# qq456cvb/VoteNet

Hardware: AMD Instinct MI355X
Metric: SUN RGB-D 20k-pt scenes/sec (fwd+bwd) (higher is better)
Workload: dtype f32

## Files before the change

votenet_amd/_lib.py:

```python
import ctypes
import os
import re
import subprocess

import torch

_HERE = os.path.dirname(os.path.abspath(__file__))
_LIB_PATH = os.path.join(_HERE, "lib", "libvotenet_hip.so")
_lib = None
SIDE_LIBS = {
    "monitors": "votenet_monitors.h",
    "guard": "votenet_step_guard.h",
    "features": "votenet_point_features.h",
    "detect": "votenet_detections.h",
    "boxpts": "votenet_box_points.h",
    "aabb": "votenet_aabb_nms.h",
    "depth": "votenet_depth_scan.h",
    "votesup": "votenet_vote_supervision.h",
    "propsup": "votenet_proposal_supervision.h",
    "votesamp": "votenet_vote_sampling.h",
    "instbox": "votenet_instance_boxes.h",
}
_side = {}


class VotenetError(RuntimeError):
    """A HIP runtime / launch / workspace error reported by libvotenet_hip.so."""


class InvalidArgumentError(ValueError):
    """Mirror of tf.errors.InvalidArgumentError raised by the reference's OP_REQUIRES checks."""


def lib_path():
    return _LIB_PATH


def build(force=False):
    if force:
        import glob
        objs = [o for d in ["obj"] + [os.path.join(name, "obj") for name in SIDE_LIBS] for o in glob.glob(os.path.join(_HERE, "csrc", d, "*.o"))]
        for f in [_LIB_PATH] + [side_path(name) for name in SIDE_LIBS] + objs:
            if os.path.exists(f):
                os.remove(f)
    out = subprocess.run(["bash", os.path.join(_HERE, "csrc", "build.sh")], capture_output=True, text=True)
    if out.returncode != 0:
        raise VotenetError("libvotenet_hip.so build failed:\n" + out.stdout + out.stderr)
    return _LIB_PATH


_SCALARS = {"int": ctypes.c_int, "long": ctypes.c_long, "float": ctypes.c_float, "double": ctypes.c_double, "unsigned": ctypes.c_uint,
            "unsigned long long": ctypes.c_ulonglong, "size_t": ctypes.c_size_t}
_POINTEES = set(_SCALARS) | {"void", "char", "unsigned char", "unsigned short", "long long"}


def _declarator(text, where):
    words = text.replace("*", " * ").split()
    if not words or not words[-1].isidentifier():
        raise ValueError("%s: cannot read the declaration '%s'" % (where, " ".join(text.split())))
    return " ".join(w for w in words[:-1] if w != "const" and w != "*"), words.count("*"), words[-1]


def _ctype(base, stars, structs, where, ret=False):
    if stars == 0 and base in _SCALARS:
        return _SCALARS[base]
    if stars == 0 and ret and base == "void":
        return None
    if stars == 1 and base in structs:
        return ctypes.POINTER(structs[base])
    if stars == 1 and ret and base == "char":
        return ctypes.c_char_p
    if stars == 1 and base in _POINTEES:
        return ctypes.c_void_p
    raise ValueError("%s: no ctypes type for the C type '%s'" % (where, base + " *" * stars))


def parse_header(text, structs):
    text = re.sub(r"/\*.*?\*/|//[^\n]*", " ", text, flags=re.S)
    text = re.sub(r"#ifdef __cplusplus.*?#endif", "", text, flags=re.S)
    text = re.sub(r"^[ \t]*#.*$", "", text, flags=re.M)

    def struct(m):
        name, fields = m.group(2), []
        for line in filter(str.strip, m.group(1).split(";")):
            decls = [_declarator(d, name) for d in line.split(",")]
            fields += [(n, _ctype(decls[0][0], stars, structs, name + "." + n)) for _, stars, n in decls]
        structs[name] = type("".join(w.capitalize() for w in name.split("_")[1:]), (ctypes.Structure,),
                             {"_fields_": fields, "__doc__": "struct %s of the C ABI." % name})
        return ""
    text = re.sub(r"typedef\s+struct\s+\w+\s*\{(.*?)\}\s*(\w+)\s*;", struct, text, flags=re.S)
    funcs = {}
    for stmt in text.split(";"):
        if not stmt.strip():
            continue
        m = re.fullmatch(r"(.*?)\((.*)\)\s*", stmt, flags=re.S)
        if not m:
            raise ValueError("not a function declaration: '%s'" % " ".join(stmt.split()))
        base, stars, name = _declarator(m.group(1), "function")
        params = [] if m.group(2).strip() == "void" else m.group(2).split(",")
        funcs[name] = (_ctype(base, stars, structs, name, ret=True),
                       [_ctype(*_declarator(p, name)[:2], structs, name) for p in params])
    return funcs


_STRUCTS = ("BnRaw", "CoefTail", "MlpInput", "RowSegment", "CopySegment")
_abi_read = None


def _abi():
    global _abi_read
    if _abi_read is None:
        structs, protos = {}, []
        for h in ("votenet_hip.h", "votenet_hip_debug.h"):
            with open(os.path.join(_HERE, os.pardir, "include", h)) as f:
                protos.append(parse_header(f.read(), structs))
        globals().update({cls.__name__: cls for cls in structs.values()})
        _abi_read = tuple(protos)
    return _abi_read


def __getattr__(name):
    if name in _STRUCTS:
        _abi()
        return globals()[name]
    raise AttributeError("module %r has no attribute %r" % (__name__, name))


class _Library(ctypes.CDLL):

    def __getattr__(self, name):
        fn = super().__getattr__(name)
        for protos in _abi():
            if name in protos:
                fn.restype, fn.argtypes = protos[name]
        if "debug" in name and name not in ("votenet_debug_enable", "votenet_debug_enabled", "votenet_debug_fps_split_timeouts"):
            self.votenet_debug_enable(1)
        return fn


def lib():
    global _lib
    if _lib is None:
        if not os.path.exists(_LIB_PATH):
            raise VotenetError(
                "libvotenet_hip.so not found at %s -- run `python -c 'import __graft_entry__ as g; g.build()'` "
                "(there is no CPU fallback)" % _LIB_PATH)
        L = _Library(_LIB_PATH)
        for name in _abi()[0]:
            getattr(L, name)
        _lib = L
    return _lib


def side_path(name):
    return os.path.join(os.path.dirname(_LIB_PATH), "libvotenet_%s.so" % name)


def side_loaded(name):
    return name in _side


def side_lib(name):
    if name not in _side:
        path = side_path(name)
        if not os.path.exists(path):
            raise VotenetError("libvotenet_%s.so not found at %s -- run `python -c 'import __graft_entry__ as g; g.build()'` "
                               "(there is no CPU fallback)" % (name, path))
        with open(os.path.join(_HERE, os.pardir, "include", SIDE_LIBS[name])) as f:
            protos = parse_header(f.read(), {})
        S = ctypes.CDLL(path)
        for fname, (restype, argtypes) in protos.items():
            fn = getattr(S, fname)
            fn.restype, fn.argtypes = restype, argtypes
        last_error, = [getattr(S, fname) for fname in protos if fname.endswith("_last_error")]
        _side[name] = (S, last_error)
    return _side[name][0]


def check(rc, side=None):
    if rc == 0:
        return
    if side is None:
        msg, who = lib().votenet_last_error().decode(), "hip"
    else:
        side_lib(side)
        msg, who = _side[side][1]().decode(), side
    if rc == 1:
        raise InvalidArgumentError(msg)
    raise VotenetError("libvotenet_%s error %d: %s" % (who, rc, msg))


_raw_stream = getattr(torch._C, "_cuda_getCurrentRawStream", None)
_cur_device = getattr(torch._C, "_cuda_getDevice", None)


def stream_ptr():
    if _raw_stream is not None and _cur_device is not None:
        return _raw_stream(_cur_device())
    return torch.cuda.current_stream().cuda_stream


class _NoGuard:
    def __enter__(self):
        return None

    def __exit__(self, *a):
        return False


_NOGUARD = _NoGuard()


def device_guard(device):
    idx = device.index
    if _cur_device is not None and (idx is None or idx == _cur_device()):
        return _NOGUARD
    return torch.cuda.device(device)


def ptr(t):
    return t.data_ptr() if t is not None else None


def dev_f32(t, name, rank=None, last=None):
    if not isinstance(t, torch.Tensor):
        raise InvalidArgumentError("%s must be a torch.Tensor" % name)
    if not t.is_cuda:
        raise VotenetError("%s must live on the GPU (no CPU fallback in votenet_amd)" % name)
    if t.dtype != torch.float32:
        raise InvalidArgumentError("%s must be float32" % name)
    if rank is not None and t.dim() != rank:
        raise InvalidArgumentError("%s expects rank %d, got shape %s" % (name, rank, tuple(t.shape)))
    if last is not None and t.shape[-1] != last:
        raise InvalidArgumentError("%s expects last dimension %d, got shape %s" % (name, last, tuple(t.shape)))
    return t.contiguous()


def pitched_rows(t):
    return t.dim() == 3 and t.stride(2) == 1 and t.stride(1) >= t.shape[2] and t.stride(0) == t.shape[1] * t.stride(1)


def dev_f32_rows(t, name):
    if isinstance(t, torch.Tensor) and t.is_cuda and t.dtype == torch.float32 and pitched_rows(t):
        return t
    return dev_f32(t, name, 3)


def dev_i32(t, name, rank=None):
    if not isinstance(t, torch.Tensor):
        raise InvalidArgumentError("%s must be a torch.Tensor" % name)
    if not t.is_cuda:
        raise VotenetError("%s must live on the GPU (no CPU fallback in votenet_amd)" % name)
    if t.dtype != torch.int32:
        raise InvalidArgumentError("%s must be int32" % name)
    if rank is not None and t.dim() != rank:
        raise InvalidArgumentError("%s expects rank %d, got shape %s" % (name, rank, tuple(t.shape)))
    return t.contiguous()
```

votenet_amd/csrc/pool_bwd.hip:

```cpp
#include "mlp_types.h"
#include <mutex>
#include <set>

namespace votenet {

bool wgrad_fast_launch(int mode, const MlpIn &d, long rows, int cin, int cout, const float *dz, const BnSrc &bs, int bsrc, float *dw,
                       hipStream_t st, float *scratch);
void wgrad_reduce(int nslice, long pstride, long e0, long e1, const float *part, float *dw, hipStream_t st);

static inline int pb_grid(long total, int block, int cap)
{
    long g = (total + block - 1) / block;
    if (g > cap) g = cap;
    return (int)(g < 1 ? 1 : g);
}

__global__ __launch_bounds__(256) void bn_bwd_reduce_zsel_kernel(long groups, int c, const float *__restrict__ gout,
                                                                 const float *__restrict__ zsel, const float *__restrict__ scale,
                                                                 const float *__restrict__ shift, const float *__restrict__ mean,
                                                                 const float *__restrict__ var, float eps, int relu,
                                                                 double *__restrict__ sums, CoefTail tail)
{
    __shared__ float sh1[4][64], sh2[4][64];
    const int cx = threadIdx.x & 63, ry = threadIdx.x >> 6;
    const int col = blockIdx.y * 64 + cx;
    float s1 = 0, s2 = 0;
    if (col < c) {
        const float sc = scale[col], sf = shift[col], mu = mean[col], inv = 1.0f / sqrtf(var[col] + eps);
        const long stride = (long)gridDim.x * 4;
        long g = (long)blockIdx.x * 4 + ry;
        for (; g + 7 * stride < groups; g += 8 * stride) {
            float zz[8], gg[8];
#pragma unroll
            for (int u = 0; u < 8; u++) {
                zz[u] = zsel[(size_t)(g + u * stride) * c + col];
                gg[u] = gout[(size_t)(g + u * stride) * c + col];
            }
#pragma unroll
            for (int u = 0; u < 8; u++) {
                if (relu && !(zz[u] * sc + sf > 0.0f)) gg[u] = 0.0f;
                s1 += gg[u];
                s2 += gg[u] * ((zz[u] - mu) * inv);
            }
        }
        for (; g < groups; g += stride) {
            const float zz = zsel[(size_t)g * c + col];
            float gg = gout[(size_t)g * c + col];
            if (relu && !(zz * sc + sf > 0.0f)) gg = 0.0f;
            s1 += gg;
            s2 += gg * ((zz - mu) * inv);
        }
    }
    sh1[ry][cx] = s1;
    sh2[ry][cx] = s2;
    __syncthreads();
    if (ry == 0 && col < c) {
        const float t1 = (sh1[0][cx] + sh1[1][cx]) + (sh1[2][cx] + sh1[3][cx]);
        const float t2 = (sh2[0][cx] + sh2[1][cx]) + (sh2[2][cx] + sh2[3][cx]);
        unsafeAtomicAdd(&sums[col], (double)t1);
        unsafeAtomicAdd(&sums[c + col], (double)t2);
    }
    coef_tail(tail, gridDim.x * gridDim.y, c, sums, scale, shift, mean, var, eps);
}

template <int COUT>
__global__ __launch_bounds__(256) void pool_dgrad_prepare_kernel(int cin, const float *__restrict__ w, const float *__restrict__ bias,
                                                                 const float *__restrict__ coef, float *__restrict__ mmat,
                                                                 float *__restrict__ cvec, unsigned *__restrict__ image,
                                                                 float *__restrict__ h2_ascale = nullptr, float *__restrict__ h2_unscale = nullptr)
{
    constexpr int LD = COUT + 4;
    __shared__ __attribute__((aligned(16))) float Wj[16][LD], Wk[16][LD];
    __shared__ float Cs[COUT], Ds[COUT];
    const int tid = threadIdx.x, tx = tid & 15, ty = tid >> 4;
    const int j0 = blockIdx.y * 16, k0 = blockIdx.x * 16;
    constexpr int Q = COUT / 4;
    for (int e = tid; e < 16 * Q; e += 256) {
        const int r = e / Q, q = e % Q;
        const float4 z4 = make_float4(0.f, 0.f, 0.f, 0.f);
        *reinterpret_cast<float4 *>(&Wj[r][q * 4]) = j0 + r < cin ? *reinterpret_cast<const float4 *>(w + (size_t)(j0 + r) * COUT + q * 4) : z4;
        *reinterpret_cast<float4 *>(&Wk[r][q * 4]) = k0 + r < cin ? *reinterpret_cast<const float4 *>(w + (size_t)(k0 + r) * COUT + q * 4) : z4;
    }
    for (int c = tid; c < COUT; c += 256) {
        const float Cc = coef[2 * COUT + c];
        Cs[c] = Cc;
        Ds[c] = coef[COUT + c] + Cc * (bias ? bias[c] : 0.0f);
    }
    __syncthreads();
    float acc = 0.0f, accv = 0.0f;
#pragma unroll 8
    for (int c = 0; c < COUT; c++) {
        const float wk = Wk[tx][c];
        acc += Wj[ty][c] * Cs[c] * wk;
        accv += Ds[c] * wk;
    }
    if (j0 + ty < cin && k0 + tx < cin) mmat[(size_t)(j0 + ty) * cin + k0 + tx] = acc;
    if (blockIdx.y == 0 && ty == 0 && k0 + tx < cin) cvec[k0 + tx] = accv;
    if (image != nullptr && h2_ascale != nullptr) {
        __shared__ float nj[16], nk[16], cmax[4];
        __syncthreads();
        {
            float pj = 0.0f, pk = 0.0f;
            for (int c = tx; c < COUT; c += 16) {
                pj += Wj[ty][c] * Wj[ty][c];
                pk += Wk[ty][c] * Wk[ty][c];
            }
#pragma unroll
            for (int o = 8; o >= 1; o >>= 1) {
                pj += __shfl_xor(pj, o);
                pk += __shfl_xor(pk, o);
            }
            if (tx == 0) {
                nj[ty] = sqrtf(pj);
                nk[ty] = sqrtf(pk);
            }
            float cm = 0.0f;
            for (int c = tid; c < COUT; c += 256) cm = fmaxf(cm, fabsf(Cs[c]));
#pragma unroll
            for (int o = 32; o >= 1; o >>= 1) cm = fmaxf(cm, __shfl_xor(cm, o));
            if ((tid & 63) == 0) cmax[tid >> 6] = cm;
        }
        __syncthreads();
        auto pow2_ge = [](float v) {
            int e = 0;
            if (v > 0.0f) (void)frexpf(v, &e);
            e = e < -100 ? -100 : (e > 100 ? 100 : e);
            return ldexpf(1.0f, e);
        };
        const float S = ldexpf(1.0f, 13) / pow2_ge(fmaxf(fmaxf(cmax[0], cmax[1]), fmaxf(cmax[2], cmax[3])));
        const float rj = pow2_ge(nj[ty]), rk = pow2_ge(nk[tx]);
        if (blockIdx.y == 0 && ty == 0 && k0 + tx < cin) {
            h2_ascale[k0 + tx] = 16.0f * rk;
            h2_unscale[k0 + tx] = rk / (16.0f * S);
        }
        float(*T)[LD] = Wj;
        __syncthreads();
        T[ty][tx] = acc * (S / (rj * rk));
        __syncthreads();
        if (tid < 32) {
            const int kh = tid >> 4, c = tid & 15;
            unsigned h[4], l[4];
#pragma unroll
            for (int i = 0; i < 4; i++) split2(T[kh * 8 + 2 * i][c], T[kh * 8 + 2 * i + 1][c], h[i], l[i]);
            uint4 *dst = reinterpret_cast<uint4 *>(image) + ((size_t)(blockIdx.y * 2) * 2 + kh) * cin + k0 + c;
            dst[0] = make_uint4(h[0], h[1], h[2], h[3]);
            dst[(size_t)2 * cin] = make_uint4(l[0], l[1], l[2], l[3]);
        }
    } else if (image != nullptr) {
        __syncthreads();
        float(*T)[LD] = Wj;
        T[ty][tx] = acc;
        __syncthreads();
        if (tid < 32) {
            const int kh = tid >> 4, c = tid & 15;
            unsigned h[4], m[4], l[4];
#pragma unroll
            for (int i = 0; i < 4; i++) split3(T[kh * 8 + 2 * i][c], T[kh * 8 + 2 * i + 1][c], h[i], m[i], l[i]);
            uint4 *dst = reinterpret_cast<uint4 *>(image) + ((size_t)(blockIdx.y * 3) * 2 + kh) * cin + k0 + c;
            dst[0] = make_uint4(h[0], h[1], h[2], h[3]);
            dst[(size_t)2 * cin] = make_uint4(m[0], m[1], m[2], m[3]);
            dst[(size_t)4 * cin] = make_uint4(l[0], l[1], l[2], l[3]);
        }
    }
}

struct PoolBelow {
    const float *z, *scale, *shift, *mean, *var;
    float eps;
    int relu;
    double *sums;
    CoefTail tail;
    int reverse;
    const int *hc;
    const float *wh;
    int G;
    const int *nh_dev;
};

template <int CIN, int COUT, int K, bool RED, int NWV = 8 >
__global__ __launch_bounds__(NWV * 64) void pool_dgrad_scatter_kernel(long groups, const float *__restrict__ gout,
                                                                 const int *__restrict__ argmax, const float *__restrict__ zsel,
                                                                 const float *__restrict__ coef, int relu, const float *__restrict__ wT,
                                                                 float *__restrict__ da, PoolBelow pb)
{
    static_assert(K == 64, "one lane per row in the prefix scan");
    constexpr bool HALF = false;
    constexpr int PL = CIN / 64;
    constexpr int RW = K / NWV;
    extern __shared__ __attribute__((aligned(16))) float pds_smem[];
    float *Wl = pds_smem;
    float *sv = Wl + COUT * CIN;
    int *lst = reinterpret_cast<int *>(sv + 2 * COUT);
    int *cnt = lst + 2 * COUT;
    int *start = cnt + 2 * K;
    const int tid = threadIdx.x, lane = tid & 63, wv = tid >> 6;
    for (int e = tid; e < COUT * CIN / 4; e += NWV * 64)
        reinterpret_cast<float4 *>(Wl)[e] = reinterpret_cast<const float4 *>(wT)[e];
    float cA = 0.f, cS = 0.f, cH = 0.f;
    const bool own = tid < COUT;
    if (own) {
        cA = coef[tid];
        cS = coef[3 * COUT + tid];
        cH = coef[4 * COUT + tid];
    }
    if (tid < 2 * K) cnt[tid] = 0;
    float bS[PL], bH[PL], bM[PL], bI[PL], s1[PL], s2[PL];
#pragma unroll
    for (int q = 0; q < PL; q++) {
        s1[q] = s2[q] = 0.0f;
        if (RED) {
            const int j = lane * PL + q;
            bS[q] = pb.scale[j];
            bH[q] = pb.shift[j];
            bM[q] = pb.mean[j];
            bI[q] = 1.0f / sqrtf(pb.var[j] + pb.eps);
        }
    }
    float n_z = 0.f, n_g = 0.f, n_w = 1.0f;
    int n_a = 0;
    auto fetch = [&](long g) {
        const long ctr = HALF ? (long)pb.hc[g] : g;
        if (HALF) n_w = pb.wh[g];
        if (own) {
            n_z = zsel[(size_t)ctr * COUT + tid];
            n_g = gout[(size_t)ctr * COUT + tid];
            n_a = argmax[(size_t)ctr * COUT + tid];
            if (HALF) {
                n_a -= g >= pb.G ? 32 : 0;
                if (n_a < 0 || n_a >= 32) n_a = -1;
            }
        }
    };
    auto grp = [&](long i) { return pb.reverse ? groups - 1 - i : i; };
    if ((long)blockIdx.x < groups) fetch(grp(blockIdx.x));
    __syncthreads();
    int par = 0;
    for (long gi = blockIdx.x; gi < groups; gi += gridDim.x, par ^= 1) {
        const long g = grp(gi);
        float *svp = sv + par * COUT;
        int *lstp = lst + par * COUT, *cntp = cnt + par * K, *startp = start + par * K;
        const float zz = n_z, w31 = n_w;
        float gg = n_g;
        const int myrow = n_a;
        const bool mine = own && (!HALF || myrow >= 0);
        float pre[RW][PL], zpre[RW][PL];
#pragma unroll
        for (int ri = 0; ri < RW; ri++)
#pragma unroll
            for (int q = 0; q < PL; q++) {
                const size_t off = ((size_t)g * K + wv + NWV * ri) * CIN + lane * PL + q;
                pre[ri][q] = da[off];
                if (RED) zpre[ri][q] = pb.z[off];
            }
        const long gn = gi + gridDim.x;
        if (gn < groups) fetch(grp(gn));
        int mypos = 0;
        if (own) {
            if (relu && !(zz * cS + cH > 0.0f)) gg = 0.0f;
            svp[tid] = cA * gg;
        }
#pragma unroll
        for (int w2 = 0; w2 < COUT / 64; w2++) {
            if (wv == w2 && (!HALF || myrow >= 0)) mypos = atomicAdd(&cntp[myrow], 1);
            __syncthreads();
        }
        if (wv == 0) {
            const int c0 = lane < K ? cntp[lane] : 0;
            int x = c0;
#pragma unroll
            for (int off = 1; off < 64; off <<= 1) {
                const int t = __shfl_up(x, off);
                if (lane >= off) x += t;
            }
            if (lane < K) startp[lane] = x - c0;
        } else if (wv == 1) {
            if (lane < K) cnt[(par ^ 1) * K + lane] = 0;
        }
        __syncthreads();
        if (mine) lstp[startp[myrow] + mypos] = tid;
        __syncthreads();
#pragma unroll
        for (int ri = 0; ri < RW; ri++) {
            const int r = wv + NWV * ri;
            const int n = cntp[r], s0 = startp[r];
            const bool scaled = HALF && r == 31 && w31 != 1.0f;
            if (!RED && n == 0 && !scaled) continue;
            float acc[PL];
#pragma unroll
            for (int q = 0; q < PL; q++) acc[q] = scaled ? pre[ri][q] * w31 : pre[ri][q];
            for (int i = 0; i < n; i += 4) {
                int c[4];
                float v[4];
#pragma unroll
                for (int u = 0; u < 4; u++) {
                    const bool ok = i + u < n;
                    c[u] = lstp[s0 + (ok ? i + u : i)];
                    v[u] = ok ? svp[c[u]] : 0.0f;
                }
#pragma unroll
                for (int u = 0; u < 4; u++)
#pragma unroll
                    for (int q = 0; q < PL; q++) acc[q] += v[u] * Wl[c[u] * CIN + lane * PL + q];
            }
            if (n != 0 || scaled) {
                float *drow = da + ((size_t)g * K + r) * CIN + lane * PL;
#pragma unroll
                for (int q = 0; q < PL; q++) drow[q] = acc[q];
            }
            if (RED) {
#pragma unroll
                for (int q = 0; q < PL; q++) {
                    const float zz2 = zpre[ri][q];
                    const float gp = (pb.relu && !(zz2 * bS[q] + bH[q] > 0.0f)) ? 0.0f : acc[q];
                    s1[q] += gp;
                    s2[q] += gp * ((zz2 - bM[q]) * bI[q]);
                }
            }
        }
    }
    if (RED) {
        __syncthreads();
        float *red = Wl;
#pragma unroll
        for (int q = 0; q < PL; q++) {
            red[(wv * 2 + 0) * CIN + lane * PL + q] = s1[q];
            red[(wv * 2 + 1) * CIN + lane * PL + q] = s2[q];
        }
        __syncthreads();
        for (int e = tid; e < 2 * CIN; e += NWV * 64) {
            float t = 0.0f;
#pragma unroll
            for (int w8 = 0; w8 < NWV; w8++) t += red[w8 * 2 * CIN + e];
            unsafeAtomicAdd(&pb.sums[e], (double)t);
        }
        coef_tail(pb.tail, gridDim.x, CIN, pb.sums, pb.scale, pb.shift, pb.mean, pb.var, pb.eps);
    }
}

template <int CIN, int COUT, int K, bool RED, int NWV>
__global__ __launch_bounds__(NWV * 64) __attribute__((amdgpu_waves_per_eu(NWV == 12 ? 3 : 4))) void pool_dgrad_scatter_wave_kernel(long groups, const float *__restrict__ gout,
                                                                           const int *__restrict__ argmax, const float *__restrict__ zsel,
                                                                           const float *__restrict__ coef, int relu,
                                                                           const float *__restrict__ wT, float *__restrict__ da, PoolBelow pb)
{
    static_assert(K == 64 || K == kPiece, "one lane per row in the prefix scan");
    constexpr bool HALF = K == kPiece;
    constexpr int PL = CIN / 64;
    constexpr int NJ = COUT / 64;
    constexpr int RB = 4;
    constexpr int NB = K / RB;
    constexpr int LCAP = COUT + 3 * K;
    constexpr int WS = LCAP * 6 + K * 4;
    static_assert(WS % 16 == 0 && (LCAP * 4) % 16 == 0, "the value lists are read 16 bytes at a time");
    extern __shared__ __attribute__((aligned(16))) float pds_smem[];
    float *Wl = pds_smem;
    const int tid = threadIdx.x, lane = tid & 63;
    const int wv = __builtin_amdgcn_readfirstlane(tid >> 6);
    unsigned char *scratch = reinterpret_cast<unsigned char *>(Wl + COUT * CIN) + (size_t)wv * WS;
    float *lv = reinterpret_cast<float *>(scratch);
    unsigned short *lc = reinterpret_cast<unsigned short *>(scratch + LCAP * 4);
    int *cnt = reinterpret_cast<int *>(scratch + LCAP * 6);
    for (int e = tid; e < COUT * CIN / 4; e += NWV * 64) reinterpret_cast<float4 *>(Wl)[e] = reinterpret_cast<const float4 *>(wT)[e];
    if (lane < K) cnt[lane] = 0;
    float cA[NJ], cS[NJ], cH[NJ];
#pragma unroll
    for (int j = 0; j < NJ; j++) {
        cA[j] = coef[j * 64 + lane];
        cS[j] = coef[3 * COUT + j * 64 + lane];
        cH[j] = coef[4 * COUT + j * 64 + lane];
    }
    float bS[PL], bH[PL], bM[PL], bI[PL], s1[PL], s2[PL];
#pragma unroll
    for (int q = 0; q < PL; q++) {
        s1[q] = s2[q] = 0.0f;
        bS[q] = bH[q] = bM[q] = bI[q] = 0.0f;
        if (RED) {
            const int j = lane * PL + q;
            bS[q] = pb.scale[j];
            bH[q] = pb.shift[j];
            bM[q] = pb.mean[j];
            bI[q] = 1.0f / sqrtf(pb.var[j] + pb.eps);
        }
    }
    __syncthreads();
    if (HALF && pb.nh_dev != nullptr) groups = pb.nh_dev[0] < groups ? pb.nh_dev[0] : groups;
    const long stride = (long)gridDim.x * NWV;
    float nz[NJ], ng[NJ], nw = 1.0f;
    int na[NJ];
    auto fetch = [&](long g) {
        const int code = HALF ? pb.hc[g] : 0;
        const long ctr = HALF ? (long)(code / kBallPieces) : g;
        if (HALF) nw = pb.wh[g];
#pragma unroll
        for (int j = 0; j < NJ; j++) {
            nz[j] = zsel[(size_t)ctr * COUT + j * 64 + lane];
            ng[j] = gout[(size_t)ctr * COUT + j * 64 + lane];
            int a = argmax[(size_t)ctr * COUT + j * 64 + lane];
            if (HALF) {
                a -= (code % kBallPieces) * kPiece;
                if (a < 0 || a >= kPiece) a = -1;
            }
            na[j] = a;
        }
    };
    struct Rows {
        float d[RB][PL], z[RB][PL];
    };
    Rows R0, R1;
    auto load_rows = [&](Rows &r, long g, int rb) {
#pragma unroll
        for (int u = 0; u < RB; u++)
#pragma unroll
            for (int q = 0; q < PL; q++) {
                const size_t off = ((size_t)g * K + rb * RB + u) * CIN + lane * PL + q;
                r.d[u][q] = da[off];
                if (RED) r.z[u][q] = pb.z[off];
            }
    };
    long gi = (long)blockIdx.x * NWV + wv;
    if (gi < groups) {
        fetch(gi);
        load_rows(R0, gi, 0);
    }
    for (; gi < groups; gi += stride) {
        const long g = gi, gn = gi + stride;
        float v[NJ];
        int row[NJ], pos[NJ];
        const float w31 = nw;
#pragma unroll
        for (int j = 0; j < NJ; j++) {
            float gg = ng[j];
            if (relu && !(nz[j] * cS[j] + cH[j] > 0.0f)) gg = 0.0f;
            v[j] = cA[j] * gg;
            row[j] = v[j] != 0.0f ? na[j] : -1;
        }
        fetch(gn < groups ? gn : g);
#pragma unroll
        for (int j = 0; j < NJ; j++) pos[j] = row[j] >= 0 ? atomicAdd(&cnt[row[j]], 1) : 0;
        const int c0 = lane < K ? cnt[lane] : 0;
        const int c4 = (c0 + 3) & ~3;
        int x = c4;
#pragma unroll
        for (int off = 1; off < 64; off <<= 1) {
            const int t = __shfl_up(x, off);
            if (lane >= off) x += t;
        }
        const int start = x - c4;
        if (lane < K) {
            cnt[lane] = 0;
            for (int t = c0; t < c4; t++) {
                lc[start + t] = 0;
                lv[start + t] = 0.0f;
            }
        }
#pragma unroll
        for (int j = 0; j < NJ; j++) {
            const int st = __shfl(start, row[j] >= 0 ? row[j] : 0);
            if (row[j] >= 0) {
                lc[st + pos[j]] = (unsigned short)(j * 64 + lane);
                lv[st + pos[j]] = v[j];
            }
        }
        auto batch = [&](const Rows &r, int rb) {
#pragma unroll
            for (int u = 0; u < RB; u++) {
                const int rr = rb * RB + u;
                const int n = __builtin_amdgcn_readlane(c4, rr), s0 = __builtin_amdgcn_readlane(start, rr);
                const bool scaled = HALF && rr == 0 && w31 != 1.0f;
                float acc[PL];
#pragma unroll
                for (int q = 0; q < PL; q++) acc[q] = scaled ? r.d[u][q] * w31 : r.d[u][q];
                for (int i = 0; i < n; i += 4) {
                    const unsigned short *pc = static_cast<const unsigned short *>(__builtin_assume_aligned(&lc[s0 + i], 8));
                    const float *pv = static_cast<const float *>(__builtin_assume_aligned(&lv[s0 + i], 16));
                    const unsigned cc[4] = {pc[0], pc[1], pc[2], pc[3]};
                    const float vv[4] = {pv[0], pv[1], pv[2], pv[3]};
                    constexpr bool kPacked = PL == 2;
                    if constexpr (kPacked) {
                        f32x2 wr[4];
#pragma unroll
                        for (int t = 0; t < 4; t++) wr[t] = *reinterpret_cast<const f32x2 *>(&Wl[cc[t] * CIN + lane * PL]);
#pragma unroll
                        for (int t = 0; t < 4; t++) {
#ifdef SCATTER_PK_SRC1
                            const f32x2 a2 = __builtin_elementwise_fma(wr[t], f32x2{vv[t], vv[t]}, f32x2{acc[0], acc[1]});
#else
                            const f32x2 a2 = __builtin_elementwise_fma(f32x2{vv[t], vv[t]}, wr[t], f32x2{acc[0], acc[1]});
#endif
                            acc[0] = a2.x;
                            acc[1] = a2.y;
                        }
                    } else {
#pragma unroll
                        for (int t = 0; t < 4; t++)
#pragma unroll
                            for (int q = 0; q < PL; q++) acc[q] = __builtin_fmaf(vv[t], Wl[cc[t] * CIN + lane * PL + q], acc[q]);
                    }
                }
                if (n != 0 || scaled) {
                    float *drow = da + ((size_t)g * K + rr) * CIN + lane * PL;
#pragma unroll
                    for (int q = 0; q < PL; q++) drow[q] = acc[q];
                }
                if (RED) {
#pragma unroll
                    for (int q = 0; q < PL; q++) {
                        const float zz2 = r.z[u][q];
                        const float gp = (pb.relu && !(zz2 * bS[q] + bH[q] > 0.0f)) ? 0.0f : acc[q];
                        s1[q] += gp;
                        s2[q] += gp * ((zz2 - bM[q]) * bI[q]);
                    }
                }
            }
        };
#pragma unroll 1
        for (int rb = 0; rb < NB; rb += 2) {
            load_rows(R1, g, rb + 1);
            batch(R0, rb);
            const bool more = rb + 2 < NB;
            load_rows(R0, more ? g : (gn < groups ? gn : g), more ? rb + 2 : 0);
            batch(R1, rb + 1);
        }
    }
    if (RED) {
        __syncthreads();
        float *red = Wl;
#pragma unroll
        for (int q = 0; q < PL; q++) {
            red[(wv * 2 + 0) * CIN + lane * PL + q] = s1[q];
            red[(wv * 2 + 1) * CIN + lane * PL + q] = s2[q];
        }
        __syncthreads();
        for (int e = tid; e < 2 * CIN; e += NWV * 64) {
            float t = 0.0f;
#pragma unroll
            for (int w8 = 0; w8 < NWV; w8++) t += red[w8 * 2 * CIN + e];
            unsafeAtomicAdd(&pb.sums[e], (double)t);
        }
        coef_tail(pb.tail, gridDim.x, CIN, pb.sums, pb.scale, pb.shift, pb.mean, pb.var, pb.eps);
    }
}

template <int CIN, int K, int TEAMS>
__global__ __launch_bounds__(256 * TEAMS) void pool_wgrad_sparse_kernel(long groups, int cout, const float *__restrict__ xz,
                                                                const float *__restrict__ in_scale, const float *__restrict__ in_shift,
                                                                int in_relu, const float *__restrict__ gout,
                                                                const int *__restrict__ argmax, const float *__restrict__ zsel,
                                                                const float *__restrict__ coef, int relu, float *__restrict__ dw,
                                                                float *__restrict__ colsum, float *__restrict__ part,
                                                                const int *__restrict__ hc, const float *__restrict__ wh, int G,
                                                                const int *__restrict__ nh_dev)
{
    constexpr bool HALF = K == kPiece;
    constexpr int LD = CIN + 4;
    constexpr int NBUF = HALF ? 2 : 1;
    if (HALF && nh_dev != nullptr) groups = nh_dev[0] < groups ? nh_dev[0] : groups;
    extern __shared__ __attribute__((aligned(16))) float sparse_smem[];
    const int team = TEAMS > 1 ? __builtin_amdgcn_readfirstlane((int)(threadIdx.x >> 8)) : 0;
    const int tid = threadIdx.x & 255;
    float(*xs)[K][LD] = reinterpret_cast<float(*)[K][LD]>(sparse_smem + (size_t)team * NBUF * K * LD);
    float acc[CIN];
#pragma unroll
    for (int i = 0; i < CIN; i++) acc[i] = 0.0f;
    float csum = 0.0f;
    const bool own = tid < cout;
    const float cA = own ? coef[tid] : 0.0f, cS = own ? coef[3 * cout + tid] : 0.0f, cH = own ? coef[4 * cout + tid] : 0.0f;
    constexpr int Q = CIN / 4;
    const int q = tid % Q;
    float4 sc = make_float4(1.f, 1.f, 1.f, 1.f), sh = make_float4(0.f, 0.f, 0.f, 0.f);
    if (in_scale) {
        sc = *reinterpret_cast<const float4 *>(in_scale + q * 4);
        sh = *reinterpret_cast<const float4 *>(in_shift + q * 4);
    }
    const float fl = (in_scale && in_relu) ? 0.0f : -__builtin_inff();
    constexpr int NL = K * Q / 256;
    constexpr int D = HALF ? 4 : 1;
    float4 nxt[D][NL];
    float n_g[D], n_z[D], n_w[D];
    int n_a[D];
    auto fetch = [&](int d, long g) {
        const float4 *src = reinterpret_cast<const float4 *>(xz + (size_t)g * K * CIN);
#pragma unroll
        for (int h = 0; h < NL; h++) nxt[d][h] = src[tid + h * 256];
        const int code = HALF ? hc[g] : 0;
        const long ctr = HALF ? (long)(code / kBallPieces) : g;
        n_w[d] = HALF ? wh[g] : 1.0f;
        n_z[d] = n_g[d] = 0.0f;
        n_a[d] = 0;
        if (own) {
            n_z[d] = zsel[(size_t)ctr * cout + tid];
            n_g[d] = gout[(size_t)ctr * cout + tid];
            n_a[d] = argmax[(size_t)ctr * cout + tid];
            if (HALF) {
                n_a[d] -= (code % kBallPieces) * kPiece;
                if (n_a[d] < 0 || n_a[d] >= kPiece) {
                    n_a[d] = 0;
                    n_g[d] = 0.0f;
                }
            }
        }
    };
    const long first = (long)blockIdx.x * TEAMS + team, stride = (long)gridDim.x * TEAMS;
#pragma unroll
    for (int d = 0; d < D; d++) {
        const long g = first + (long)d * stride;
        fetch(d, g < groups ? g : groups - 1);
    }
    int buf = 0;
    for (long g0 = (long)blockIdx.x * TEAMS; g0 < groups; g0 += (long)D * stride) {
#pragma unroll
        for (int d = 0; d < D; d++) {
            if (g0 + (long)d * stride >= groups) break;
            const long g = g0 + team + (long)d * stride;
            const bool live = g < groups;
            float(*xt)[LD] = xs[HALF ? buf : 0];
#pragma unroll
            for (int h = 0; h < NL; h++) {
                float4 v = nxt[d][h];
                v.x = fmaxf(v.x * sc.x + sh.x, fl);
                v.y = fmaxf(v.y * sc.y + sh.y, fl);
                v.z = fmaxf(v.z * sc.z + sh.z, fl);
                v.w = fmaxf(v.w * sc.w + sh.w, fl);
                *reinterpret_cast<float4 *>(&xt[(tid + h * 256) / Q][q * 4]) = v;
            }
            float gg = live ? n_g[d] : 0.0f;
            const float zz = n_z[d], w31 = n_w[d];
            const int ar = n_a[d];
            const long gn = g + (long)D * stride;
            fetch(d, gn < groups ? gn : (live ? g : groups - 1));
            __syncthreads();
            if (own) {
                if (relu && !(zz * cS + cH > 0.0f)) gg = 0.0f;
                const float v = cA * gg;
                if (v != 0.0f) {
                    const float4 *row = reinterpret_cast<const float4 *>(&xt[ar][0]);
#pragma unroll
                    for (int i0 = 0; i0 < Q; i0 += 8) {
                        float4 a[8];
#pragma unroll
                        for (int i = 0; i < 8; i++) a[i] = row[i0 + i];
                        asm volatile("" ::: "memory");
#pragma unroll
                        for (int i = 0; i < 8; i++) {
                            acc[4 * (i0 + i)] += a[i].x * v;
                            acc[4 * (i0 + i) + 1] += a[i].y * v;
                            acc[4 * (i0 + i) + 2] += a[i].z * v;
                            acc[4 * (i0 + i) + 3] += a[i].w * v;
                        }
                    }
                }
            }
            if (live && tid >= 256 - CIN) {
                const int jc = tid - (256 - CIN);
#pragma unroll 8
                for (int r = (HALF ? 1 : 0); r < K; r++) csum += xt[r][jc];
                if (HALF) csum += w31 * xt[0][jc];
            }
            if (HALF) buf ^= 1;
            else __syncthreads();
        }
    }
    if (TEAMS > 1) {
        __syncthreads();
        float *comb = sparse_smem;
        if (team == 1) {
            if (own) {
#pragma unroll
                for (int i = 0; i < CIN; i++) comb[(size_t)i * cout + tid] = acc[i];
            }
            if (tid >= 256 - CIN) comb[(size_t)CIN * cout + tid - (256 - CIN)] = csum;
        }
        __syncthreads();
        if (team == 1) return;
        if (own) {
#pragma unroll
            for (int i = 0; i < CIN; i++) acc[i] += comb[(size_t)i * cout + tid];
        }
        if (tid >= 256 - CIN) csum += comb[(size_t)CIN * cout + tid - (256 - CIN)];
    }
    if (part) {
        float *__restrict__ mine = part + (size_t)blockIdx.x * (CIN + 1) * cout;
        if (own) {
#pragma unroll
            for (int i = 0; i < CIN; i++) mine[(size_t)i * cout + tid] = acc[i];
        }
        if (tid >= 256 - CIN) mine[(size_t)CIN * cout + tid - (256 - CIN)] = csum;
        return;
    }
    if (own) {
#pragma unroll
        for (int i = 0; i < CIN; i++) unsafeAtomicAdd(&dw[(size_t)i * cout + tid], acc[i]);
    }
    if (tid >= 256 - CIN) unsafeAtomicAdd(&colsum[tid - (256 - CIN)], csum);
}

template <int CIN, int TEAMS>
__global__ __launch_bounds__(256 * TEAMS) void pool_wgrad_sparse_centre_kernel(int G, long nh, int cout, const float *__restrict__ xz,
                                                                       const float *__restrict__ in_scale, const float *__restrict__ in_shift,
                                                                       int in_relu, const float *__restrict__ gout,
                                                                       const int *__restrict__ argmax, const float *__restrict__ zsel,
                                                                       const float *__restrict__ coef, int relu, float *__restrict__ dw,
                                                                       float *__restrict__ colsum, const int *__restrict__ pos,
                                                                       const float *__restrict__ wh, const int *__restrict__ nh_dev)
{
    constexpr int K = kPiece, NP = kBallPieces;
    constexpr int LD = CIN + 4;
    if (nh_dev != nullptr) nh = nh_dev[0] < nh ? nh_dev[0] : nh;
    extern __shared__ __attribute__((aligned(16))) float sparse_smem[];
    const int team = TEAMS > 1 ? __builtin_amdgcn_readfirstlane((int)(threadIdx.x >> 8)) : 0;
    const int tid = threadIdx.x & 255;
    float(*xs)[NP][K][LD] = reinterpret_cast<float(*)[NP][K][LD]>(sparse_smem + (size_t)team * 2 * NP * K * LD);
    float acc[CIN];
#pragma unroll
    for (int i = 0; i < CIN; i++) acc[i] = 0.0f;
    float csum = 0.0f;
    const bool own = tid < cout;
    const float cA = own ? coef[tid] : 0.0f, cS = own ? coef[3 * cout + tid] : 0.0f, cH = own ? coef[4 * cout + tid] : 0.0f;
    constexpr int Q = CIN / 4;
    const int q = tid % Q;
    float4 sc = make_float4(1.f, 1.f, 1.f, 1.f), sh = make_float4(0.f, 0.f, 0.f, 0.f);
    if (in_scale) {
        sc = *reinterpret_cast<const float4 *>(in_scale + q * 4);
        sh = *reinterpret_cast<const float4 *>(in_shift + q * 4);
    }
    const float fl = (in_scale && in_relu) ? 0.0f : -__builtin_inff();
    constexpr int NL = K * Q / 256;
    constexpr int D = 2;
    float4 nxt[D][NP][NL];
    long n_row[D][NP];
    float n_g[D], n_z[D], n_w[D];
    int n_a[D];
    const __amdgpu_buffer_rsrc_t xrs = __builtin_amdgcn_make_buffer_rsrc((void *)xz, 0, (int)((size_t)nh * K * CIN * 4), 0x00020000);
    const int ch = own ? tid : 0;
    auto fetch = [&](int d, long c) {
        n_row[d][0] = c * K;
#pragma unroll
        for (int j = 1; j < NP; j++) {
            const int p = pos[(size_t)c * (NP - 1) + j - 1];
            n_row[d][j] = (p >= 0 && (long)G + p < nh) ? ((long)G + p) * K : -1;
        }
#pragma unroll
        for (int j = 0; j < NP; j++) {
            const unsigned base = n_row[d][j] < 0 ? 0x80000000u : (unsigned)(n_row[d][j] * CIN * 4);
#pragma unroll
            for (int h = 0; h < NL; h++)
                nxt[d][j][h] = __builtin_bit_cast(float4, __builtin_amdgcn_raw_buffer_load_b128(xrs, base + (unsigned)(tid + h * 256) * 16u, 0, 0));
        }
        n_w[d] = wh[c];
        n_z[d] = zsel[(size_t)c * cout + ch];
        const float gv = gout[(size_t)c * cout + ch];
        n_g[d] = own ? gv : 0.0f;
        n_a[d] = argmax[(size_t)c * cout + ch];
    };
    const long first = (long)blockIdx.x * TEAMS + team, stride = (long)gridDim.x * TEAMS;
#pragma unroll
    for (int d = 0; d < D; d++) {
        const long c = first + (long)d * stride;
        fetch(d, c < G ? c : G - 1);
    }
    int buf = 0;
    for (long c0 = (long)blockIdx.x * TEAMS; c0 < G; c0 += (long)D * stride) {
#pragma unroll
        for (int d = 0; d < D; d++) {
            if (c0 + (long)d * stride >= G) break;
            const long c = c0 + team + (long)d * stride;
            const bool live = c < G;
            float(*xt)[K][LD] = xs[buf];
            bool kept[NP];
#pragma unroll
            for (int j = 0; j < NP; j++) {
                kept[j] = n_row[d][j] >= 0;
                if (!kept[j]) continue;
#pragma unroll
                for (int h = 0; h < NL; h++) {
                    float4 v = nxt[d][j][h];
                    v.x = fmaxf(v.x * sc.x + sh.x, fl);
                    v.y = fmaxf(v.y * sc.y + sh.y, fl);
                    v.z = fmaxf(v.z * sc.z + sh.z, fl);
                    v.w = fmaxf(v.w * sc.w + sh.w, fl);
                    *reinterpret_cast<float4 *>(&xt[j][(tid + h * 256) / Q][q * 4]) = v;
                }
            }
            float gg = live ? n_g[d] : 0.0f;
            const float zz = n_z[d], w31 = n_w[d];
            const int ar = n_a[d];
            const long cn = c + (long)D * stride;
            fetch(d, cn < G ? cn : (live ? c : G - 1));
            __syncthreads();
            if (own) {
                if (relu && !(zz * cS + cH > 0.0f)) gg = 0.0f;
                const float v = cA * gg;
                const int pj = ar >> 4;
                const bool there = pj == 0 ? kept[0] : pj == 1 ? kept[1] : pj == 2 ? kept[2] : kept[3];
                if (v != 0.0f && there) {
                    const float4 *row = reinterpret_cast<const float4 *>(&xt[pj][ar & (K - 1)][0]);
#pragma unroll
                    for (int i0 = 0; i0 < Q; i0 += 8) {
                        float4 a[8];
#pragma unroll
                        for (int i = 0; i < 8; i++) a[i] = row[i0 + i];
                        asm volatile("" ::: "memory");
#pragma unroll
                        for (int i = 0; i < 8; i++) {
                            acc[4 * (i0 + i)] += a[i].x * v;
                            acc[4 * (i0 + i) + 1] += a[i].y * v;
                            acc[4 * (i0 + i) + 2] += a[i].z * v;
                            acc[4 * (i0 + i) + 3] += a[i].w * v;
                        }
                    }
                }
            }
            if (live && tid >= 256 - CIN) {
                const int jc = tid - (256 - CIN);
#pragma unroll
                for (int j = 0; j < NP; j++) {
                    if (!kept[j]) continue;
#pragma unroll 8
                    for (int r = (j == 0 ? 1 : 0); r < K; r++) csum += xt[j][r][jc];
                }
                csum += w31 * xt[0][0][jc];
            }
            buf ^= 1;
        }
    }
    if (TEAMS > 1) {
        __syncthreads();
        float *comb = sparse_smem;
        if (team == 1) {
            if (own) {
#pragma unroll
                for (int i = 0; i < CIN; i++) comb[(size_t)i * cout + tid] = acc[i];
            }
            if (tid >= 256 - CIN) comb[(size_t)CIN * cout + tid - (256 - CIN)] = csum;
        }
        __syncthreads();
        if (team == 1) return;
        if (own) {
#pragma unroll
            for (int i = 0; i < CIN; i++) acc[i] += comb[(size_t)i * cout + tid];
        }
        if (tid >= 256 - CIN) csum += comb[(size_t)CIN * cout + tid - (256 - CIN)];
    }
    if (own) {
#pragma unroll
        for (int i = 0; i < CIN; i++) unsafeAtomicAdd(&dw[(size_t)i * cout + tid], acc[i]);
    }
    if (tid >= 256 - CIN) unsafeAtomicAdd(&colsum[tid - (256 - CIN)], csum);
}

__global__ __launch_bounds__(256) void pool_wgrad_finish_kernel(int cin, int cout, const float *__restrict__ gram,
                                                                const float *__restrict__ colsum, const float *__restrict__ w,
                                                                const float *__restrict__ bias, const float *__restrict__ coef,
                                                                float *__restrict__ dw)
{
    __shared__ float Gs[16][33], Ws[32][17];
    const int tx = threadIdx.x & 15, ty = threadIdx.x >> 4;
    const int j0 = blockIdx.y * 16, c0 = blockIdx.x * 16;
    float acc = 0.0f;
    for (int i0 = 0; i0 < cin; i0 += 32) {
        for (int e = threadIdx.x; e < 16 * 32; e += 256) {
            const int r = e >> 5, ii = e & 31;
            Gs[r][ii] = (j0 + r < cin && i0 + ii < cin) ? gram[(size_t)(j0 + r) * cin + i0 + ii] : 0.0f;
            const int wr = e >> 4, wc = e & 15;
            Ws[wr][wc] = (i0 + wr < cin && c0 + wc < cout) ? w[(size_t)(i0 + wr) * cout + c0 + wc] : 0.0f;
        }
        __syncthreads();
#pragma unroll 8
        for (int ii = 0; ii < 32; ii++) acc += Gs[ty][ii] * Ws[ii][tx];
        __syncthreads();
    }
    const int j = j0 + ty, c = c0 + tx;
    if (j < cin && c < cout) {
        const float Cc = coef[2 * cout + c];
        dw[(size_t)j * cout + c] += Cc * acc + colsum[j] * (coef[cout + c] + Cc * (bias ? bias[c] : 0.0f));
    }
}

}

using namespace votenet;

extern "C" int votenet_pool_backward_supported(int cin, int cout, int k)
{
    return k == 64 && ((cin == 128 && (cout == 256 || cout == 128)) || (cin == 64 && cout == 128));
}

static int g_zsel_groups = 32, g_zsel_cap = 256;
extern "C" void votenet_debug_zsel_grid(int groups_per_wg, int cap)
{
    VN_DEBUG_GATE();
    g_zsel_groups = groups_per_wg > 0 ? groups_per_wg : 32;
    g_zsel_cap = cap > 0 ? cap : 256;
}
extern "C" int votenet_bn_backward_reduce_pool(long groups, int c, const float *gout, const float *zsel, const float *scale,
                                               const float *shift, const float *mean, const float *var, float eps, int relu,
                                               double *sums, const votenet_coef_tail *tail, void *stream)
{
    VN_REQUIRE(groups > 0 && c > 0, "bn_backward_reduce_pool expects groups > 0, c > 0");
    VN_REQUIRE(gout && zsel && scale && shift && mean && var && sums, "bn_backward_reduce_pool: null buffer");
    VN_REQUIRE(!tail || (tail->ticket && tail->gamma && tail->coef && tail->rows > 0), "bn_backward_reduce_pool: incomplete coefficient tail");
    const int ny = (c + 63) / 64;
    hipLaunchKernelGGL(bn_bwd_reduce_zsel_kernel, dim3(pb_grid(groups, g_zsel_groups, g_zsel_cap / ny), ny), dim3(256), 0, as_stream(stream), groups,
                       c, gout, zsel, scale, shift, mean, var, eps, relu, sums, to_tail(tail));
    return check_launch("bn_backward_reduce_pool");
}

static int pool_dgrad_prepare_launch(int cin, int cout, const float *w, const float *bias, const float *coef, float *mmat, float *cvec,
                                     void *image, void *stream, float *h2_ascale = nullptr, float *h2_unscale = nullptr)
{
    VN_REQUIRE(cin > 0 && w && coef && mmat && cvec, "pool_dgrad_prepare: bad arguments");
    VN_REQUIRE((cout == 128 || cout == 256) && (uintptr_t)w % 16 == 0, "pool_dgrad_prepare: cout must be 128 or 256 (got %d), w 16-byte aligned", cout);
    VN_REQUIRE(image == nullptr || (cin % 16 == 0 && (uintptr_t)image % 16 == 0), "pool_dgrad_prepare_split: cin %% 16 == 0 and a 16-byte aligned image");
    const dim3 grid((cin + 15) / 16, (cin + 15) / 16);
    unsigned *img = static_cast<unsigned *>(image);
    if (cout == 256)
        hipLaunchKernelGGL(pool_dgrad_prepare_kernel<256>, grid, dim3(256), 0, as_stream(stream), cin, w, bias, coef, mmat, cvec, img, h2_ascale, h2_unscale);
    else
        hipLaunchKernelGGL(pool_dgrad_prepare_kernel<128>, grid, dim3(256), 0, as_stream(stream), cin, w, bias, coef, mmat, cvec, img, h2_ascale, h2_unscale);
    return check_launch("pool_dgrad_prepare");
}
extern "C" int votenet_pool_dgrad_prepare(int cin, int cout, const float *w, const float *bias, const float *coef, float *mmat,
                                          float *cvec, void *stream)
{
    return pool_dgrad_prepare_launch(cin, cout, w, bias, coef, mmat, cvec, nullptr, stream);
}
extern "C" int votenet_pool_dgrad_prepare_h2(int cin, int cout, const float *w, const float *bias, const float *coef, float *mmat,
                                             float *cvec, void *image, float *ascale, float *unscale, void *stream)
{
    VN_REQUIRE(image != nullptr && ascale != nullptr && unscale != nullptr, "pool_dgrad_prepare_h2: null image / scale vectors");
    return pool_dgrad_prepare_launch(cin, cout, w, bias, coef, mmat, cvec, image, stream, ascale, unscale);
}
extern "C" int votenet_pool_dgrad_prepare_split(int cin, int cout, const float *w, const float *bias, const float *coef, float *mmat,
                                                float *cvec, void *image, void *stream)
{
    VN_REQUIRE(image != nullptr, "pool_dgrad_prepare_split: null image");
    return pool_dgrad_prepare_launch(cin, cout, w, bias, coef, mmat, cvec, image, stream);
}

static int g_scatter_reverse = 0;
extern "C" void votenet_debug_scatter_reverse(int on) { VN_DEBUG_GATE(); g_scatter_reverse = on ? 1 : 0; }
static int g_scatter_nwv = 16;
extern "C" void votenet_debug_scatter_waves(int n) { VN_DEBUG_GATE(); g_scatter_nwv = n == 12 ? 12 : 16; }
static int g_scatter_wgs = 0;
extern "C" void votenet_debug_scatter_workgroups(int n) { VN_DEBUG_GATE(); g_scatter_wgs = n > 0 ? n : 0; }
static int g_scatter_form = 1;
extern "C" void votenet_debug_scatter_form(int form) { VN_DEBUG_GATE(); g_scatter_form = form ? 1 : 0; }
static int pool_dgrad_scatter_launch(long groups, int k, int cin, int cout, const float *gout, const int *argmax, const float *zsel,
                                     const float *coef, int relu, const float *wT, float *da, const float *below_z,
                                     const float *below_scale, const float *below_shift, const float *below_mean, const float *below_var,
                                     float eps, int below_relu, double *below_sums, const votenet_coef_tail *below_tail, const int *hc,
                                     const float *wh, int G, void *stream, const int *nh_dev = nullptr);
extern "C" int votenet_pool_dgrad_scatter(long groups, int k, int cin, int cout, const float *gout, const int *argmax,
                                          const float *zsel, const float *coef, int relu, const float *wT, float *da,
                                          const float *below_z, const float *below_scale, const float *below_shift,
                                          const float *below_mean, const float *below_var, float eps, int below_relu,
                                          double *below_sums, const votenet_coef_tail *below_tail, void *stream)
{
    VN_REQUIRE(!below_tail || (below_z && below_tail->ticket && below_tail->gamma && below_tail->coef && below_tail->rows > 0),
               "pool_dgrad_scatter: incomplete coefficient tail");
    VN_REQUIRE(groups > 0 && gout && argmax && zsel && coef && wT && da, "pool_dgrad_scatter: bad arguments");
    VN_REQUIRE(votenet_pool_backward_supported(cin, cout, k), "pool_dgrad_scatter: unsupported shape cin=%d cout=%d k=%d", cin, cout, k);
    VN_REQUIRE((uintptr_t)wT % 16 == 0, "pool_dgrad_scatter: wT must be 16-byte aligned");
    VN_REQUIRE(!below_z || (below_scale && below_shift && below_mean && below_var && below_sums),
               "pool_dgrad_scatter: below_z given without the layer's BatchNorm vectors / sums");
    return pool_dgrad_scatter_launch(groups, k, cin, cout, gout, argmax, zsel, coef, relu, wT, da, below_z, below_scale, below_shift, below_mean,
                                     below_var, eps, below_relu, below_sums, below_tail, nullptr, nullptr, 0, stream);
}

extern "C" int votenet_pool_dgrad_scatter_half(long nh, int G, int cin, int cout, const float *gout, const int *argmax, const float *zsel,
                                               const float *coef, int relu, const float *wT, float *da, const int *hc, const float *wh,
                                               const float *below_z, const float *below_scale, const float *below_shift,
                                               const float *below_mean, const float *below_var, float eps, int below_relu,
                                               double *below_sums, const votenet_coef_tail *below_tail, const int *nh_dev, void *stream)
{
    VN_REQUIRE(hc && wh && G > 0 && nh >= G && nh <= (long)kBallPieces * G, "pool_dgrad_scatter_half: bad piece-layout arguments");
    VN_REQUIRE(gout && argmax && zsel && coef && wT && da && (uintptr_t)wT % 16 == 0, "pool_dgrad_scatter_half: null / unaligned buffer");
    VN_REQUIRE(votenet_pool_backward_supported(cin, cout, 64), "pool_dgrad_scatter_half: unsupported shape cin=%d cout=%d", cin, cout);
    VN_REQUIRE(!below_z || (below_scale && below_shift && below_mean && below_var && below_sums),
               "pool_dgrad_scatter_half: below_z given without the layer's BatchNorm vectors / sums");
    VN_REQUIRE(!below_tail || (below_z && below_tail->ticket && below_tail->gamma && below_tail->coef && below_tail->rows > 0),
               "pool_dgrad_scatter_half: incomplete coefficient tail");
    return pool_dgrad_scatter_launch(nh, 64, cin, cout, gout, argmax, zsel, coef, relu, wT, da, below_z, below_scale, below_shift, below_mean,
                                     below_var, eps, below_relu, below_sums, below_tail, hc, wh, G, stream, nh_dev);
}

static int pool_dgrad_scatter_launch(long groups, int k, int cin, int cout, const float *gout, const int *argmax, const float *zsel,
                                     const float *coef, int relu, const float *wT, float *da, const float *below_z,
                                     const float *below_scale, const float *below_shift, const float *below_mean, const float *below_var,
                                     float eps, int below_relu, double *below_sums, const votenet_coef_tail *below_tail, const int *hc,
                                     const float *wh, int G, void *stream, const int *nh_dev)
{
    hipStream_t st = as_stream(stream);
    const PoolBelow pb = {below_z, below_scale, below_shift, below_mean, below_var, eps, below_relu, below_sums, to_tail(below_tail), g_scatter_reverse, hc, wh, G, nh_dev};
    auto go = [&](auto kern, int ci, int co, int threads = 512) {
        const size_t smem = ((size_t)co * ci + 4 * co + 4 * k) * 4;
        const int per_cu = smem > 80 * 1024 ? 1 : (smem > 40 * 1024 ? 2 : 4);
        static std::set<const void *> raised;
        static std::mutex raised_mu;
        bool fresh;
        {
            std::lock_guard<std::mutex> lock(raised_mu);
            fresh = raised.insert(reinterpret_cast<const void *>(kern)).second;
        }
        if (fresh)
            (void)hipFuncSetAttribute(reinterpret_cast<const void *>(kern), hipFuncAttributeMaxDynamicSharedMemorySize, (int)smem);
        hipLaunchKernelGGL(kern, dim3(pb_grid(groups, 2, 256 * per_cu)), dim3(threads), smem, st, groups, gout, argmax, zsel, coef, relu,
                           wT, da, pb);
    };
    auto gow = [&](auto kern, int ci, int co, int kk, int nwv) {
        const size_t smem = (size_t)co * ci * 4 + (size_t)nwv * ((co + 3 * kk) * 6 + kk * 4);
        const int per_cu = smem > 80 * 1024 ? 1 : (smem > 40 * 1024 ? 2 : 4);
        static std::set<const void *> raised_w;
        static std::mutex raised_w_mu;
        bool fresh;
        {
            std::lock_guard<std::mutex> lock(raised_w_mu);
            fresh = raised_w.insert(reinterpret_cast<const void *>(kern)).second;
        }
        if (fresh)
            (void)hipFuncSetAttribute(reinterpret_cast<const void *>(kern), hipFuncAttributeMaxDynamicSharedMemorySize, (int)smem);
        hipLaunchKernelGGL(kern, dim3(pb_grid(groups, nwv, g_scatter_wgs > 0 ? g_scatter_wgs : 256 * per_cu)), dim3(nwv * 64), smem, st, groups, gout,
                           argmax, zsel, coef, relu, wT, da, pb);
    };
    if (g_scatter_form == 1 || hc) {
#define VN_SCATTER_WAVE(CI, CO, KK, NW)                                                            \
    do {                                                                                           \
        if (below_z) gow(pool_dgrad_scatter_wave_kernel<CI, CO, KK, true, NW>, CI, CO, KK, NW);   \
        else gow(pool_dgrad_scatter_wave_kernel<CI, CO, KK, false, NW>, CI, CO, KK, NW);          \
    } while (0)
        if (hc) {
            if (cin == 64) VN_SCATTER_WAVE(64, 128, kPiece, 8);
            else if (cout == 256) {
                if (g_scatter_nwv == 12) VN_SCATTER_WAVE(128, 256, kPiece, 12);
                else VN_SCATTER_WAVE(128, 256, kPiece, 16);
            }
            else VN_SCATTER_WAVE(128, 128, kPiece, 8);
        } else {
            if (cin == 64) VN_SCATTER_WAVE(64, 128, 64, 8);
            else if (cout == 256) VN_SCATTER_WAVE(128, 256, 64, 8);
            else VN_SCATTER_WAVE(128, 128, 64, 8);
        }
#undef VN_SCATTER_WAVE
        return check_launch("pool_dgrad_scatter");
    }
    if (below_z) {
        if (cin == 128 && cout == 256)
            go(pool_dgrad_scatter_kernel<128, 256, 64, true, 16>, 128, 256, 1024);
        else if (cin == 128)
            go(pool_dgrad_scatter_kernel<128, 128, 64, true>, 128, 128);
        else
            go(pool_dgrad_scatter_kernel<64, 128, 64, true>, 64, 128);
    } else {
        if (cin == 128 && cout == 256)
            go(pool_dgrad_scatter_kernel<128, 256, 64, false, 16>, 128, 256, 1024);
        else if (cin == 128)
            go(pool_dgrad_scatter_kernel<128, 128, 64, false>, 128, 128);
        else
            go(pool_dgrad_scatter_kernel<64, 128, 64, false>, 64, 128);
    }
    return check_launch("pool_dgrad_scatter");
}

#ifndef GRAM_ABL
#define GRAM_ABL 0
#endif
template <int C, int NP = 3>
__global__ __launch_bounds__(256) void gram_bf3_kernel(long rows, const float *__restrict__ x, const float *__restrict__ scale_shift,
                                                       int relu, float *__restrict__ gram, long rows_per_block,
                                                       const float *__restrict__ wh ,
                                                       const int *__restrict__ nh_dev )
{
    if (nh_dev != nullptr) {
        const long lim = (long)nh_dev[0] * kPiece;
        rows = lim < rows ? lim : rows;
    }
    constexpr int KPT = C / 16;
    constexpr int T = C / 64;
    constexpr int PL = C * 4 + 16;
    static_assert(NP == 2 || NP == 3, "pieces per operand");
    constexpr float kA = NP == 2 ? 16.0f : 1.0f, kUn = NP == 2 ? 1.0f / 256.0f : 1.0f;
    __shared__ __attribute__((aligned(16))) unsigned Ts[2][NP][2][PL];
    const int tid = threadIdx.x, lane = tid & 63;
    const int wv = __builtin_amdgcn_readfirstlane(tid >> 6);
    const int wi = wv >> 1, wj = wv & 1;
    const long r_begin = (long)blockIdx.x * rows_per_block;
    if (r_begin >= rows) return;
    const int nrow = (int)((r_begin + rows_per_block < rows ? r_begin + rows_per_block : rows) - r_begin);
    const int nslab = (nrow + 15) / 16;
    const int c = tid % C, rg = tid / C;
    const int kh_w = (C == 128) ? rg : (rg >> 1), d_w = (C == 128) ? 0 : (rg & 1) * 2;
    const float sc = scale_shift[c] * kA, sh = scale_shift[C + c] * kA;
    const float floor_ = relu ? 0.0f : -__builtin_inff();
    const float *xb = x + (size_t)r_begin * C + c;
    float R[2][KPT];
    static_assert(kPiece == 16, "one slab = one piece");
    const bool first_rg = rg == 0;
    const float *whb = wh ? wh + r_begin / kPiece : nullptr;
    const float *whp = whb ? whb : scale_shift;
    float Wq[2] = {1.0f, 1.0f};
    bool abl_prologue = true;
    auto load = [&](float (&r)[KPT], int s, float &wq) {
        if ((GRAM_ABL & 4) && !abl_prologue) return;
#pragma unroll
        for (int i = 0; i < KPT; i++) {
            int lr = s * 16 + rg * KPT + i;
            lr = lr < nrow ? lr : nrow - 1;
            r[i] = xb[(size_t)lr * C];
        }
        const int sw = (whb != nullptr && s * 16 < nrow) ? s : 0;
        wq = whp[sw];
    };
    auto store = [&](int buf, const float (&r)[KPT], int s, float wq) {
        if ((GRAM_ABL & 8) && !abl_prologue) return;
        float v[KPT];
#pragma unroll
        for (int i = 0; i < KPT; i++) {
            v[i] = fmaxf(r[i] * sc + sh, floor_);
            if (s * 16 + rg * KPT + i >= nrow) v[i] = 0.0f;
        }
        if (whb != nullptr && first_rg && s * 16 < nrow) v[0] *= sqrtf(wq);
        if constexpr (NP == 2) {
            unsigned h[KPT / 2], l[KPT / 2];
#pragma unroll
            for (int i = 0; i < KPT / 2; i++) split2(v[2 * i], v[2 * i + 1], h[i], l[i]);
            if constexpr (C == 128) {
                *reinterpret_cast<uint4 *>(&Ts[buf][0][kh_w][c * 4]) = make_uint4(h[0], h[1], h[2], h[3]);
                *reinterpret_cast<uint4 *>(&Ts[buf][1][kh_w][c * 4]) = make_uint4(l[0], l[1], l[2], l[3]);
            } else {
                *reinterpret_cast<uint2 *>(&Ts[buf][0][kh_w][c * 4 + d_w]) = make_uint2(h[0], h[1]);
                *reinterpret_cast<uint2 *>(&Ts[buf][1][kh_w][c * 4 + d_w]) = make_uint2(l[0], l[1]);
            }
            return;
        }
        unsigned h[KPT / 2], m[KPT / 2], l[KPT / 2];
#pragma unroll
        for (int i = 0; i < KPT / 2; i++) split3(v[2 * i], v[2 * i + 1], h[i], m[i], l[i]);
        if constexpr (C == 128) {
            *reinterpret_cast<uint4 *>(&Ts[buf][0][kh_w][c * 4]) = make_uint4(h[0], h[1], h[2], h[3]);
            *reinterpret_cast<uint4 *>(&Ts[buf][1][kh_w][c * 4]) = make_uint4(m[0], m[1], m[2], m[3]);
            *reinterpret_cast<uint4 *>(&Ts[buf][NP - 1][kh_w][c * 4]) = make_uint4(l[0], l[1], l[2], l[3]);
        } else {
            *reinterpret_cast<uint2 *>(&Ts[buf][0][kh_w][c * 4 + d_w]) = make_uint2(h[0], h[1]);
            *reinterpret_cast<uint2 *>(&Ts[buf][1][kh_w][c * 4 + d_w]) = make_uint2(m[0], m[1]);
            *reinterpret_cast<uint2 *>(&Ts[buf][NP - 1][kh_w][c * 4 + d_w]) = make_uint2(l[0], l[1]);
        }
    };
    f32x16 acc[T][T];
#pragma unroll
    for (int a = 0; a < T; a++)
#pragma unroll
        for (int b = 0; b < T; b++)
#pragma unroll
            for (int e = 0; e < 16; e++) acc[a][b][e] = 0.0f;
    load(R[0], 0, Wq[0]);
    store(0, R[0], 0, Wq[0]);
    load(R[1], 1, Wq[1]);
    __builtin_amdgcn_sched_barrier(0);
    load(R[0], 2, Wq[0]);
    __syncthreads();
    const int kh = lane >> 5, l31 = lane & 31;
    int buf = 0;
    abl_prologue = false;
    const int nslab2 = (nslab + 1) & ~1;
    for (int s = 0; s < nslab2; s += 2) {
#pragma unroll
        for (int par = 0; par < 2; par++) {
            uint4 fa[NP][T], fb[NP][T];
#pragma unroll
            for (int p = 0; p < NP; p++) {
#pragma unroll
                for (int t = 0; t < T; t++) {
                    fa[p][t] = *reinterpret_cast<const uint4 *>(&Ts[buf][p][kh][((wi * T + t) * 32 + l31) * 4]);
                    fb[p][t] = *reinterpret_cast<const uint4 *>(&Ts[buf][p][kh][((wj * T + t) * 32 + l31) * 4]);
                }
            }
            auto mm = [&](int pa, int pb) {
                if (GRAM_ABL & 1) {
                    acc[0][0][0] += __uint_as_float(fa[pa][0].x ^ fb[pb][0].y);
                    return;
                }
#pragma unroll
                for (int a = 0; a < T; a++)
#pragma unroll
                    for (int b = 0; b < T; b++) {
                        if constexpr (NP == 2)
                            acc[a][b] = __builtin_amdgcn_mfma_f32_32x32x16_f16(__builtin_bit_cast(f16x8, fa[pa][a]),
                                                                               __builtin_bit_cast(f16x8, fb[pb][b]), acc[a][b], 0, 0, 0);
                        else
                            acc[a][b] = __builtin_amdgcn_mfma_f32_32x32x16_bf16(__builtin_bit_cast(bf16x8, fa[pa][a]),
                                                                                __builtin_bit_cast(bf16x8, fb[pb][b]), acc[a][b], 0, 0, 0);
                    }
            };
            if constexpr (NP == 2) {
                mm(1, 0);
                mm(0, 1);
                store(buf ^ 1, R[par ^ 1], s + par + 1, Wq[par ^ 1]);
                load(R[par ^ 1], s + par + 3, Wq[par ^ 1]);
                mm(0, 0);
            } else {
                mm(2, 0);
                mm(0, 2);
                mm(1, 1);
                store(buf ^ 1, R[par ^ 1], s + par + 1, Wq[par ^ 1]);
                load(R[par ^ 1], s + par + 3, Wq[par ^ 1]);
                mm(1, 0);
                mm(0, 1);
                mm(0, 0);
            }
            lds_barrier();
            buf ^= 1;
        }
    }
    if (GRAM_ABL & 2) {
        float t_ = 0.0f;
#pragma unroll
        for (int a = 0; a < T; a++)
#pragma unroll
            for (int b = 0; b < T; b++)
#pragma unroll
                for (int e = 0; e < 16; e++) t_ += acc[a][b][e];
        if (t_ == 12345.678f) gram[0] = t_;
        return;
    }
#pragma unroll
    for (int a = 0; a < T; a++)
#pragma unroll
        for (int b = 0; b < T; b++) {
            const int j = (wj * T + b) * 32 + l31;
#pragma unroll
            for (int e = 0; e < 16; e++) {
                const int i = (wi * T + a) * 32 + (e & 3) + 8 * (e >> 2) + 4 * kh;
                unsafeAtomicAdd(&gram[(size_t)i * C + j], acc[a][b][e] * kUn);
            }
        }
}

int g_gram_bf3 = 1;
static int g_gram_wgs = 384;
template <int C>
static void gram_bf3_launch(long rows, const float *z, const float *scale_shift, int relu, float *gram, hipStream_t st, const float *wh = nullptr,
                            const int *nh_dev = nullptr)
{
    long rpb = (rows + g_gram_wgs - 1) / g_gram_wgs;
    rpb = (rpb + 31) / 32 * 32;
    if (rpb < 128) rpb = 128;
    const unsigned gx = (unsigned)((rows + rpb - 1) / rpb);
    if (g_gram_bf3 != 3) hipLaunchKernelGGL((gram_bf3_kernel<C, 2>), dim3(gx), dim3(256), 0, st, rows, z, scale_shift, relu, gram, rpb, wh, nh_dev);
    else hipLaunchKernelGGL((gram_bf3_kernel<C, 3>), dim3(gx), dim3(256), 0, st, rows, z, scale_shift, relu, gram, rpb, wh, nh_dev);
}
extern "C" void votenet_debug_gram_bf3(int on) { VN_DEBUG_GATE(); g_gram_bf3 = on; }
extern "C" void votenet_debug_gram_workgroups(int n) { VN_DEBUG_GATE(); g_gram_wgs = n > 0 ? n : 384; }

extern "C" int votenet_mlp_gram(long rows, int c, const float *z, const float *scale_shift, int relu, float *gram, float *scratch,
                                void *stream)
{
    if (g_gram_bf3 && scratch == nullptr && (c == 64 || c == 128) && rows > 0 && rows < (1L << 31) / c && z && scale_shift && gram &&
        (uintptr_t)z % 16 == 0) {
        if (c == 128) gram_bf3_launch<128>(rows, z, scale_shift, relu, gram, as_stream(stream));
        else gram_bf3_launch<64>(rows, z, scale_shift, relu, gram, as_stream(stream));
        return check_launch("mlp_gram");
    }
    VN_REQUIRE(rows > 0 && c > 0 && z && scale_shift && gram, "mlp_gram: bad arguments");
    MlpIn d = {};
    d.x = z;
    d.in_scale = scale_shift;
    d.in_shift = scale_shift + c;
    d.in_relu = relu;
    BnSrc bs = {};
    bs.z = z;
    bs.coef = scale_shift;
    bs.relu = relu;
    VN_REQUIRE(wgrad_fast_launch(0, d, rows, c, c, nullptr, bs, 3, gram, as_stream(stream), scratch),
               "mlp_gram: shape not served (c %% 64 == 0, 16-byte aligned operands), got c = %d", c);
    return check_launch("mlp_gram");
}

static int g_sparse_wgs = 384, g_sparse_wgs2 = 256, g_sparse_teams = 2;
extern "C" void votenet_debug_sparse_workgroups(int n) { VN_DEBUG_GATE(); g_sparse_wgs = n > 0 ? n : 384; }
extern "C" void votenet_debug_sparse_teams(int teams, int wgs)
{
    VN_DEBUG_GATE();
    g_sparse_teams = teams == 1 ? 1 : 2;
    if (wgs > 0) g_sparse_wgs2 = wgs;
}
static int pool_wgrad_sparse_launch(long groups, int cin, int cout, const float *xz, const float *in_scale, const float *in_shift, int in_relu,
                                    const float *gout, const int *argmax, const float *zsel, const float *coef, int relu, float *dw,
                                    float *colsum, float *scratch, const int *hc, const float *wh, int G, void *stream, const int *nh_dev = nullptr);
extern "C" int votenet_pool_wgrad_sparse(long groups, int k, int cin, int cout, const float *xz, const float *in_scale,
                                         const float *in_shift, int in_relu, const float *gout, const int *argmax, const float *zsel,
                                         const float *coef, int relu, float *dw, float *colsum, float *scratch, void *stream)
{
    VN_REQUIRE(groups > 0 && xz && gout && argmax && zsel && coef && dw && colsum, "pool_wgrad_sparse: bad arguments");
    VN_REQUIRE(cin <= cout, "pool_wgrad_sparse expects cin <= cout");
    VN_REQUIRE(votenet_pool_backward_supported(cin, cout, k), "pool_wgrad_sparse: unsupported shape cin=%d cout=%d k=%d", cin, cout, k);
    VN_REQUIRE((in_scale == nullptr) == (in_shift == nullptr), "pool_wgrad_sparse: in_scale and in_shift go together");
    VN_REQUIRE((uintptr_t)xz % 16 == 0 && (!in_scale || ((uintptr_t)in_scale % 16 == 0 && (uintptr_t)in_shift % 16 == 0)),
               "pool_wgrad_sparse: operands must be 16-byte aligned");
    return pool_wgrad_sparse_launch(groups, cin, cout, xz, in_scale, in_shift, in_relu, gout, argmax, zsel, coef, relu, dw, colsum, scratch,
                                    nullptr, nullptr, 0, stream);
}

extern "C" int votenet_mlp_gram_half(long rows, int c, const float *z, const float *scale_shift, int relu, const float *wh, float *gram,
                                     const int *nh_dev, void *stream)
{
    VN_REQUIRE(rows > 0 && rows % kPiece == 0 && rows < (1L << 31) / c && (c == 128 || c == 64), "mlp_gram_half expects rows %% 16 == 0 and c in {64, 128}");
    VN_REQUIRE(z && scale_shift && wh && gram && (uintptr_t)z % 16 == 0, "mlp_gram_half: null / unaligned buffer");
    if (c == 128) gram_bf3_launch<128>(rows, z, scale_shift, relu, gram, as_stream(stream), wh, nh_dev);
    else gram_bf3_launch<64>(rows, z, scale_shift, relu, gram, as_stream(stream), wh, nh_dev);
    return check_launch("mlp_gram_half");
}

extern "C" int votenet_pool_wgrad_sparse_half(long nh, int G, int cin, int cout, const float *xz, const float *in_scale, const float *in_shift,
                                              int in_relu, const float *gout, const int *argmax, const float *zsel, const float *coef, int relu,
                                              float *dw, float *colsum, const int *hc, const float *wh, const int *nh_dev, void *stream)
{
    VN_REQUIRE(nh > 0 && G > 0 && nh >= G && nh <= (long)kBallPieces * G && hc && wh, "pool_wgrad_sparse_half: bad piece-layout arguments");
    VN_REQUIRE(xz && gout && argmax && zsel && coef && dw && colsum, "pool_wgrad_sparse_half: bad arguments");
    VN_REQUIRE(votenet_pool_backward_supported(cin, cout, 64), "pool_wgrad_sparse_half: unsupported shape cin=%d cout=%d", cin, cout);
    VN_REQUIRE((in_scale == nullptr) == (in_shift == nullptr), "pool_wgrad_sparse_half: in_scale and in_shift go together");
    VN_REQUIRE((uintptr_t)xz % 16 == 0 && (!in_scale || ((uintptr_t)in_scale % 16 == 0 && (uintptr_t)in_shift % 16 == 0)),
               "pool_wgrad_sparse_half: operands must be 16-byte aligned");
    return pool_wgrad_sparse_launch(nh, cin, cout, xz, in_scale, in_shift, in_relu, gout, argmax, zsel, coef, relu, dw, colsum, nullptr, hc, wh,
                                    G, stream, nh_dev);
}

static int g_sparse_centre_wgs = 192, g_sparse_centre_teams = 2;
extern "C" void votenet_debug_sparse_centre_workgroups(int n) { VN_DEBUG_GATE(); g_sparse_centre_wgs = n > 0 ? n : 192; }
extern "C" void votenet_debug_sparse_centre_teams(int t) { VN_DEBUG_GATE(); g_sparse_centre_teams = t == 1 ? 1 : 2; }
extern "C" int votenet_pool_wgrad_sparse_half_centres(long nh, int G, int cin, int cout, const float *xz, const float *in_scale,
                                                      const float *in_shift, int in_relu, const float *gout, const int *argmax,
                                                      const float *zsel, const float *coef, int relu, float *dw, float *colsum,
                                                      const int *pos, const float *wh, const int *nh_dev, void *stream)
{
    VN_REQUIRE(nh > 0 && G > 0 && nh >= G && nh <= (long)kBallPieces * G && pos && wh, "pool_wgrad_sparse_half_centres: bad piece-layout arguments");
    VN_REQUIRE(xz && gout && argmax && zsel && coef && dw && colsum, "pool_wgrad_sparse_half_centres: bad arguments");
    VN_REQUIRE(votenet_pool_backward_supported(cin, cout, 64), "pool_wgrad_sparse_half_centres: unsupported shape cin=%d cout=%d", cin, cout);
    VN_REQUIRE((in_scale == nullptr) == (in_shift == nullptr), "pool_wgrad_sparse_half_centres: in_scale and in_shift go together");
    VN_REQUIRE((size_t)nh * kPiece * (size_t)cin * 4 < ((size_t)1 << 31),
               "pool_wgrad_sparse_half_centres: nh*16*cin*4 = %zu bytes exceeds the 2 GiB the centre-walking kernel addresses; "
               "use votenet_pool_wgrad_sparse_half", (size_t)nh * kPiece * (size_t)cin * 4);
    VN_REQUIRE((uintptr_t)xz % 16 == 0 && (!in_scale || ((uintptr_t)in_scale % 16 == 0 && (uintptr_t)in_shift % 16 == 0)),
               "pool_wgrad_sparse_half_centres: operands must be 16-byte aligned");
    hipStream_t st = as_stream(stream);
    const int teams = g_sparse_centre_teams;
    auto go = [&](auto kern, int ci) {
        const size_t tiles = (size_t)teams * 2 * kBallPieces * kPiece * (ci + 4) * 4;
        const size_t comb = teams > 1 ? (size_t)(ci + 1) * cout * 4 : 0;
        const size_t smem = tiles > comb ? tiles : comb;
        static std::set<const void *> raised_c;
        static std::mutex raised_c_mu;
        bool fresh;
        {
            std::lock_guard<std::mutex> lock(raised_c_mu);
            fresh = raised_c.insert(reinterpret_cast<const void *>(kern)).second;
        }
        if (fresh) (void)hipFuncSetAttribute(reinterpret_cast<const void *>(kern), hipFuncAttributeMaxDynamicSharedMemorySize, (int)smem);
        const int grid = pb_grid(G, 8 * teams, g_sparse_centre_wgs * 2 / teams);
        hipLaunchKernelGGL(kern, dim3(grid), dim3(256 * teams), smem, st, G, nh, cout, xz, in_scale, in_shift, in_relu, gout, argmax, zsel, coef, relu, dw,
                           colsum, pos, wh, nh_dev);
    };
    if (teams == 1) {
        if (cin == 64) go(pool_wgrad_sparse_centre_kernel<64, 1>, 64);
        else go(pool_wgrad_sparse_centre_kernel<128, 1>, 128);
    } else if (cin == 64) go(pool_wgrad_sparse_centre_kernel<64, 2>, 64);
    else go(pool_wgrad_sparse_centre_kernel<128, 2>, 128);
    return check_launch("pool_wgrad_sparse_half_centres");
}

static int pool_wgrad_sparse_launch(long groups, int cin, int cout, const float *xz, const float *in_scale, const float *in_shift, int in_relu,
                                    const float *gout, const int *argmax, const float *zsel, const float *coef, int relu, float *dw,
                                    float *colsum, float *scratch, const int *hc, const float *wh, int G, void *stream, const int *nh_dev)
{
    hipStream_t st = as_stream(stream);
    int grid;
    auto go = [&](auto kern, int ci, int kk, int teams, int cap) {
        const size_t tiles = (size_t)teams * (kk == kPiece ? 2 : 1) * kk * (ci + 4) * 4;
        const size_t comb = teams > 1 ? (size_t)(ci + 1) * cout * 4 : 0;
        const size_t smem = tiles > comb ? tiles : comb;
        static std::set<const void *> raised_s;
        static std::mutex raised_s_mu;
        bool fresh;
        {
            std::lock_guard<std::mutex> lock(raised_s_mu);
            fresh = raised_s.insert(reinterpret_cast<const void *>(kern)).second;
        }
        if (fresh) (void)hipFuncSetAttribute(reinterpret_cast<const void *>(kern), hipFuncAttributeMaxDynamicSharedMemorySize, (int)smem);
        grid = pb_grid(groups, (kk == kPiece ? 32 : 8) * teams, cap);
        hipLaunchKernelGGL(kern, dim3(grid), dim3(256 * teams), smem, st, groups, cout, xz, in_scale, in_shift, in_relu, gout, argmax, zsel, coef,
                           relu, dw, colsum, scratch, hc, wh, G, nh_dev);
    };
    if (hc && g_sparse_teams == 2 && !scratch) {
        if (cin == 64) go(pool_wgrad_sparse_kernel<64, kPiece, 2>, 64, kPiece, 2, g_sparse_wgs2);
        else go(pool_wgrad_sparse_kernel<128, kPiece, 2>, 128, kPiece, 2, g_sparse_wgs2);
    } else if (hc) {
        if (cin == 64) go(pool_wgrad_sparse_kernel<64, kPiece, 1>, 64, kPiece, 1, g_sparse_wgs);
        else go(pool_wgrad_sparse_kernel<128, kPiece, 1>, 128, kPiece, 1, g_sparse_wgs);
    } else if (cin == 128) {
        go(pool_wgrad_sparse_kernel<128, 64, 1>, 128, 64, 1, g_sparse_wgs);
    } else {
        go(pool_wgrad_sparse_kernel<64, 64, 1>, 64, 64, 1, g_sparse_wgs);
    }
    if (scratch) {
        const long ps = (long)(cin + 1) * cout;
        wgrad_reduce(grid, ps, 0, (long)cin * cout, scratch, dw, st);
        wgrad_reduce(grid, ps, (long)cin * cout, (long)cin * cout + cin, scratch, colsum - (long)cin * cout, st);
    }
    return check_launch("pool_wgrad_sparse");
}

extern "C" size_t votenet_pool_wgrad_scratch_floats(long groups, int cin, int cout)
{
    if (groups <= 0) return 0;
    return (size_t)pb_grid(groups, 8, g_sparse_wgs) * (size_t)(cin + 1) * cout;
}

extern "C" int votenet_pool_wgrad_finish(int cin, int cout, const float *gram, const float *colsum, const float *w, const float *bias,
                                         const float *coef, float *dw, void *stream)
{
    VN_REQUIRE(cin > 0 && cout > 0 && gram && colsum && w && coef && dw, "pool_wgrad_finish: bad arguments");
    hipLaunchKernelGGL(pool_wgrad_finish_kernel, dim3((cout + 15) / 16, (cin + 15) / 16), dim3(256), 0, as_stream(stream), cin, cout,
                       gram, colsum, w, bias, coef, dw);
    return check_launch("pool_wgrad_finish");
}
```

votenet_amd/mlp.py:

```python
import ctypes

import torch

from . import _lib as L

PROFILE_EVENTS = None
PROFILE_SHAPES = None


class _Timed:
    def __init__(self, kind, flops, shape=None, limit=None):
        self.kind, self.flops, self.shape = kind, flops, shape
        if limit is not None and getattr(limit, "nh_limit", None) is not None:
            self.flops = (flops, limit.nh_dev, BALL_PIECES * limit.G)

    def __enter__(self):
        if PROFILE_EVENTS is not None:
            self.e0, self.e1 = torch.cuda.Event(enable_timing=True), torch.cuda.Event(enable_timing=True)
            self.e0.record()

    def __exit__(self, *a):
        if PROFILE_EVENTS is not None:
            self.e1.record()
            PROFILE_EVENTS.append((self.e0, self.e1, self.kind, self.flops) if PROFILE_SHAPES is None else (self.e0, self.e1, self.kind, self.flops, self.shape))


def resolve_event(ev):
    if isinstance(ev[3], tuple):
        fl, nh, bound = ev[3]
        ev = ev[:3] + (fl * float(nh.item()) / bound,) + tuple(ev[4:])
    return ev


class _StatsArena:
    buf = None
    nd = 0
    off = 0
    cap32 = 0
    off32 = 0
    want32 = 0
    zeroed32 = 0
    depth = 0
    active = False
    whole_step = False


def arena_begin(device, ndoubles=1 << 17, whole_step=False):
    a = _StatsArena
    if a.active and a.buf is not None and a.buf.device == device:
        a.depth += 1
        return
    need32 = (a.want32 + 1023) // 1024 * 1024
    if a.buf is None or a.buf.device != device or a.nd < ndoubles or a.cap32 < need32:
        a.nd, a.cap32 = ndoubles, max(need32, a.cap32)
        a.buf = torch.empty(a.nd + a.cap32 // 2, dtype=torch.float64, device=device)
    used32 = min(a.cap32, need32)
    a.buf[:a.nd + used32 // 2].zero_()
    a.zeroed32 = used32
    a.off = a.off32 = a.want32 = 0
    a.depth = 1
    a.active = True
    a.whole_step = bool(whole_step)


def arena_end():
    a = _StatsArena
    a.depth -= 1
    if a.depth <= 0:
        a.active = False
        a.depth = 0
        a.whole_step = False


def _zeros_f64(n, device):
    a = _StatsArena
    if a.active and a.buf.device == device and a.off + n <= a.nd:
        v = a.buf[a.off:a.off + n]
        a.off += (n + 1) & ~1
        return v
    return torch.zeros(n, dtype=torch.float64, device=device)


def _zeros_i64(shape, device):
    n = 1
    for d in shape:
        n *= int(d)
    a = _StatsArena
    if a.active and a.buf.device == device and a.off + n <= a.nd:
        v = a.buf[a.off:a.off + n].view(torch.int64).view(shape)
        a.off += (n + 1) & ~1
        return v
    return torch.zeros(shape, dtype=torch.int64, device=device)


def _zeros_f32(shape, device):
    n = 1
    for d in shape:
        n *= int(d)
    a = _StatsArena
    if a.active and a.buf.device == device:
        n4 = (n + 3) & ~3
        a.want32 += n4
        if a.off32 + n4 <= a.zeroed32:
            v = a.buf[a.nd:].view(torch.float32)[a.off32:a.off32 + n].view(shape)
            a.off32 += n4
            return v
    return torch.zeros(shape, dtype=torch.float32, device=device)


DETERMINISTIC = False
CONFIG_EPOCH = 0


def debug_switch(name, *args):
    global CONFIG_EPOCH
    CONFIG_EPOCH += 1
    return getattr(L.lib(), "votenet_debug_" + name)(*args)


def set_deterministic(on=True):
    global DETERMINISTIC
    prev, DETERMINISTIC = DETERMINISTIC, bool(on)
    return prev


COEF_TAIL = True
_tickets = {}


def _coef_tail(tail, c, device):
    if tail is None or not COEF_TAIL:
        return None, None
    rows, gamma, dgamma, dbeta = tail
    tk = _tickets.get(device)
    if tk is None:
        tk = _tickets[device] = [torch.zeros(64, dtype=torch.int32, device=device), 0]
    tk[1] = (tk[1] + 1) % 64
    coef = torch.empty(5 * c, dtype=torch.float32, device=device)
    t = L.CoefTail()
    t.ticket = tk[0].data_ptr() + 4 * tk[1]
    t.rows = rows
    t.gamma, t.coef = gamma.data_ptr(), coef.data_ptr()
    t.dgamma = dgamma.data_ptr() if dgamma is not None else None
    t.dbeta = dbeta.data_ptr() if dbeta is not None else None
    return t, coef


def _coef_after(tail, bn, sums, eps):
    rows, gamma, dgamma, dbeta = tail
    return bn_backward_coef(rows, bn[0], bn[1], bn[2], bn[3], gamma, sums, dgamma, dbeta, eps)


def _wgrad_scratch(desc, rows, cin, cout, device):
    if not DETERMINISTIC:
        return None
    nf = L.lib().votenet_mlp_wgrad_scratch_floats(ctypes.byref(desc) if desc is not None else None, rows, cin, cout)
    return torch.empty(nf, dtype=torch.float32, device=device) if nf else None


def inverse_index(idx, n):
    b = idx.shape[0]
    slots = idx.numel()
    if idx.is_cuda and idx.dtype == torch.int32 and idx.is_contiguous() and 0 < n <= 8192 and b > 0 and slots // b <= 8 * n:
        order = torch.empty(slots, dtype=torch.int32, device=idx.device)
        offsets = torch.empty(b * n + 1, dtype=torch.int32, device=idx.device)
        with L.device_guard(idx.device):
            L.check(L.lib().votenet_inverse_index(b, slots // b, n, L.ptr(idx), L.ptr(order), L.ptr(offsets), L.stream_ptr()))
        return order, offsets
    flat = (idx.reshape(b, -1).to(torch.int64) + (torch.arange(b, device=idx.device, dtype=torch.int64) * n)[:, None]).reshape(-1)
    keys, _ = torch.sort(flat * slots + torch.arange(slots, device=idx.device, dtype=torch.int64))
    pts = torch.div(keys, slots, rounding_mode="floor")
    order = (keys - pts * slots).to(torch.int32)
    offsets = torch.searchsorted(pts, torch.arange(b * n + 1, device=idx.device, dtype=torch.int64)).to(torch.int32)
    return order, offsets


def attach_inverse(idx, n, always=False):
    if (DETERMINISTIC or always) and getattr(idx, "_inv", None) is None:
        idx._inv = inverse_index(idx, n)
    return idx


def _inverse_of(idx, n):
    inv = getattr(idx, "_inv", None)
    if inv is None or inv[1].numel() != idx.shape[0] * n + 1:
        inv = inverse_index(idx, n)
        idx._inv = inv
    return inv


def csr_gather_sum(src2d, inv, npts, weight=None, div=1):
    c = src2d.shape[1]
    out = torch.empty((npts, c), dtype=torch.float32, device=src2d.device)
    with L.device_guard(src2d.device):
        if src2d.is_contiguous():
            L.check(L.lib().votenet_csr_gather_sum(npts, c, L.ptr(src2d), L.ptr(inv[0]), L.ptr(inv[1]), L.ptr(weight), div, L.ptr(out),
                                                   L.stream_ptr()))
        else:
            if src2d.stride(1) != 1 or src2d.stride(0) < c:
                raise L.InvalidArgumentError("csr_gather_sum expects rows with unit column stride")
            L.check(L.lib().votenet_csr_gather_sum_pitched(npts, c, L.ptr(src2d), src2d.stride(0), L.ptr(inv[0]), L.ptr(inv[1]), L.ptr(weight),
                                                           div, L.ptr(out), L.stream_ptr()))
    return out


BN_EPS = 1e-5


class PendingBN:

    def __init__(self, stats, gamma, beta, rows, eps=None, out=None):
        self.stats, self.gamma, self.beta, self.rows = stats, gamma, beta, rows
        self.eps = BN_EPS if eps is None else eps
        self.out = out if out is not None else torch.empty((4, gamma.shape[0]), dtype=torch.float32, device=gamma.device)
        self.done = False

    scale = property(lambda self: self.out[0])
    shift = property(lambda self: self.out[1])
    mean = property(lambda self: self.out[2])
    var = property(lambda self: self.out[3])

    def raw(self):
        r = L.BnRaw()
        r.stats, r.gamma, r.beta = self.stats.data_ptr(), self.gamma.data_ptr(), self.beta.data_ptr()
        r.rows, r.eps, r.out = self.rows, self.eps, self.out.data_ptr()
        self.done = True
        return r

    def finalize(self):
        if not self.done:
            c = self.gamma.shape[0]
            with L.device_guard(self.gamma.device):
                L.check(L.lib().votenet_bn_finalize(self.rows, c, L.ptr(self.stats), L.ptr(self.gamma), L.ptr(self.beta), float(self.eps),
                                                    L.ptr(self.out[0]), L.ptr(self.out[1]), L.ptr(self.out[2]), L.ptr(self.out[3]),
                                                    L.stream_ptr()))
            self.done = True
        return self.out[0], self.out[1]


class FrozenBN:
    done = True

    def __init__(self, out):
        self.out = out

    scale = property(lambda self: self.out[0])
    shift = property(lambda self: self.out[1])

    def finalize(self):
        return self.out[0], self.out[1]


def _desc_dense(x, scale=None, shift=None, relu=True, in_bn=None):
    d = L.MlpInput()
    if in_bn is not None:
        if in_bn.done:
            scale, shift = in_bn.scale, in_bn.shift
        else:
            d._raw = in_bn.raw()
            d.in_bn = ctypes.pointer(d._raw)
    d.x = x.data_ptr()
    d.in_scale = scale.data_ptr() if scale is not None else None
    d.in_shift = shift.data_ptr() if shift is not None else None
    d.in_relu = 1 if (relu and (scale is not None or bool(d.in_bn))) else 0
    return d


def _desc_gather(xyz, new_xyz, feat, idx):
    d = L.MlpInput()
    d.x = None
    d.xyz = xyz.data_ptr()
    d.new_xyz = new_xyz.data_ptr()
    d.feat = feat.data_ptr() if feat is not None else None
    d.idx = idx.data_ptr()
    d.b, d.n = xyz.shape[0], xyz.shape[1]
    d.m, d.nsample = idx.shape[1], idx.shape[2]
    d.c = feat.shape[2] if feat is not None else 0
    return d


SPLIT_ADHOC = False
SPLIT_ADHOC_ROWS = 65536
ADHOC_H2 = True


def split_eligible(cin, cout):
    return cin % 32 == 0 and cin <= 512 and cout % 64 == 0


class SplitImages:

    def __init__(self, mats, pieces=3):
        mats = [w for w in mats if w.dim() == 2 and w.is_contiguous() and split_eligible(*w.shape)]
        self.mats = mats
        self.nseg = len(mats)
        self.pieces = int(pieces)
        assert self.pieces in (2, 3)
        if not mats:
            return
        dev = mats[0].device
        total, offs = 0, []
        for w in mats:
            offs.append(total)
            total += w.shape[0] * w.shape[1] * 2 * self.pieces
            total = (total + 15) // 16 * 16
        self.buf = torch.empty(total, dtype=torch.uint8, device=dev)
        base = self.buf.data_ptr()
        table = []
        for w, o in zip(mats, offs):
            table += [w.data_ptr(), base + o, w.shape[0], w.shape[1]]
        self.table = torch.tensor(table, dtype=torch.int64, device=dev)
        self._reg = [(w.data_ptr(), w.shape[0], w.shape[1], base + o) for w, o in zip(mats, offs)]
        for wp, cin, cout, ip in self._reg:
            L.check(L.lib().votenet_register_split_weights_pieces(ctypes.c_void_p(wp), cin, cout, ctypes.c_void_p(ip), self.pieces))

    def refresh(self):
        if self.nseg:
            with L.device_guard(self.buf.device):
                fn = L.lib().votenet_split_weights_h2 if self.pieces == 2 else L.lib().votenet_split_weights
                L.check(fn(self.nseg, L.ptr(self.table), L.stream_ptr()))

    def close(self):
        for wp, cin, cout, _ in getattr(self, "_reg", []):
            L.lib().votenet_register_split_weights(ctypes.c_void_p(wp), cin, cout, None)
        self._reg = []

    def __del__(self):
        try:
            self.close()
        except Exception:
            pass


FORWARD_H2 = True
SPLIT_K = False
_SK_TICKETS = {}


class _SplitK:
    __slots__ = ("ws",)

    def __init__(self, rows, cin, cout, device):
        self.ws = None
        if not SPLIT_K or rows <= 0 or rows > 16384:
            return
        if device not in _SK_TICKETS:
            if torch.cuda.is_current_stream_capturing():
                return
            t = torch.zeros(1 << 16, dtype=torch.int32, device=device)
            torch.cuda.current_stream(device).synchronize()
            L.check(L.lib().votenet_mlp_split_k_tickets(L.ptr(t), t.numel()))
            _SK_TICKETS[device] = t
        n = L.lib().votenet_mlp_split_k_floats(rows, cin, cout)
        if n > 0:
            self.ws = torch.empty(n, dtype=torch.float32, device=device)

    def __enter__(self):
        if self.ws is not None:
            L.lib().votenet_mlp_split_k_arm(L.ptr(self.ws), self.ws.numel())
        return self

    def __exit__(self, *exc):
        if self.ws is not None:
            L.lib().votenet_mlp_split_k_arm(None, 0)
        return False


def linear_dense(x, w, bias=None, in_scale=None, in_shift=None, in_relu=True, want_stats=True, in_bn=None):
    x = L.dev_f32(x, "mlp_linear x", 2)
    w = L.dev_f32(w, "mlp_linear w", 2)
    rows, cin = x.shape
    if w.shape[0] != cin:
        raise L.InvalidArgumentError("mlp_linear: w has %d rows, input has %d channels" % (w.shape[0], cin))
    cout = w.shape[1]
    z = torch.empty((rows, cout), dtype=torch.float32, device=x.device)
    stats = _zeros_f64(2 * cout, x.device) if want_stats else None
    d = _desc_dense(x, in_scale, in_shift, in_relu, in_bn)
    with L.device_guard(x.device), _SplitK(rows, cin, cout, x.device), \
            _Timed("linear_dense", 2.0 * rows * cin * cout, (rows, cin, cout, "fwd" + ("+bn" if (in_scale is not None or in_bn is not None) else ""))):
        L.check(L.lib().votenet_mlp_linear(ctypes.byref(d), rows, cin, cout, L.ptr(w), L.ptr(bias), L.ptr(z), L.ptr(stats),
                                           L.stream_ptr()))
    return z, stats


def linear_gather(xyz, new_xyz, feat, idx, w, bias=None, want_stats=True):
    xyz = L.dev_f32(xyz, "mlp_linear xyz", 3, 3)
    new_xyz = L.dev_f32(new_xyz, "mlp_linear new_xyz", 3, 3)
    idx = L.dev_i32(idx, "mlp_linear idx", 3)
    feat = L.dev_f32(feat, "mlp_linear feat", 3) if feat is not None else None
    w = L.dev_f32(w, "mlp_linear w", 2)
    b, m, k = idx.shape
    c = feat.shape[2] if feat is not None else 0
    cin, cout = 3 + c, w.shape[1]
    if w.shape[0] != cin:
        raise L.InvalidArgumentError("mlp_linear: w has %d rows, grouped input has %d channels" % (w.shape[0], cin))
    rows = b * m * k
    z = torch.empty((rows, cout), dtype=torch.float32, device=xyz.device)
    stats = _zeros_f64(2 * cout, xyz.device) if want_stats else None
    d = _desc_gather(xyz, new_xyz, feat, idx)
    with L.device_guard(xyz.device), _Timed("linear_gather", 2.0 * rows * cin * cout, (rows, cin, cout, "gather")):
        L.check(L.lib().votenet_mlp_linear(ctypes.byref(d), rows, cin, cout, L.ptr(w), L.ptr(bias), L.ptr(z), L.ptr(stats),
                                           L.stream_ptr()))
    return z, stats


def assembled_supported(rows, c0, c1):
    return rows > 0 and rows % 128 == 0 and rows < 2 ** 31 and c0 % 64 == 0 and c0 <= 512 and c1 % 64 == 0


def assemble_rows(xyz, new_xyz, idx, want_sums=True, pts_cnt=None, in_pass=False):
    b, m, k = idx.shape
    n = xyz.shape[1]
    geo = torch.empty((b * m * k, 4), dtype=torch.float32, device=xyz.device)
    cntv = (_zeros_i64((b * n, 4), xyz.device) if in_pass else torch.zeros((b * n, 4), dtype=torch.int64, device=xyz.device)) if want_sums else None
    mom = (_zeros_f64(10, xyz.device)[:9] if in_pass else torch.zeros(9, dtype=torch.float64, device=xyz.device)) if want_sums else None
    with L.device_guard(xyz.device):
        L.check(L.lib().votenet_assemble_rows(b, n, m, k, L.ptr(xyz), L.ptr(new_xyz), L.ptr(idx), L.ptr(pts_cnt), L.ptr(geo), L.ptr(cntv), L.ptr(mom),
                                              L.stream_ptr()))
    return geo, cntv, mom


PIECE = 16
BALL_PIECES = 64 // PIECE
_nh_ring = None
_nh_turn = 0


_slot_source = None


class layout_slots:

    def __init__(self, pinned):
        self.pinned, self.turn = pinned, 0

    def _next(self):
        if self.turn >= self.pinned.numel():
            raise L.VotenetError("layout_slots: more piece layouts than slots (%d)" % self.pinned.numel())
        self.turn += 1
        return self.pinned[self.turn - 1:self.turn]

    def __enter__(self):
        global _slot_source
        self._saved, _slot_source = _slot_source, self._next
        return self

    def __exit__(self, *exc):
        global _slot_source
        _slot_source = self._saved


class HalfLayout:

    @staticmethod
    def host_slot():
        global _nh_ring, _nh_turn
        if _slot_source is not None:
            return _slot_source()
        if _nh_ring is None:
            if L.lib().votenet_half_piece_rows() != PIECE:
                raise L.VotenetError("libvotenet_hip.so was built for pieces of %d rows, the host code for %d" % (L.lib().votenet_half_piece_rows(), PIECE))
            _nh_ring = torch.zeros(256, dtype=torch.int32).pin_memory()
        slot = _nh_ring[_nh_turn:_nh_turn + 1]
        _nh_turn = (_nh_turn + 1) % 256
        return slot

    def __init__(self, G, pos, hc, wh, nh_dev, device_count=False, slot=None):
        global _nh_ring, _nh_turn
        self.G, self.pos, self._hc, self._wh, self.nh_dev = G, pos, hc, wh, nh_dev
        self._geo = self._u8 = None
        self._order = None
        self.nh_limit = nh_dev if device_count else None
        if device_count:
            self.nh = None
            self._ev = None
            return
        self._slot = slot
        if torch.cuda.is_current_stream_capturing():
            self._ev = None
        else:
            self._ev = torch.cuda.Event()
            self._ev.record()
        self.nh = None

    def rearm(self, ev):
        self.nh = None
        self._ev = ev

    def tensors(self):
        return [t for t in (self.pos, self._hc, self._wh, self.nh_dev, self._geo, self._u8, self._order) if t is not None]

    def resolve(self):
        if self.nh is None and self.nh_limit is not None:
            self.nh = BALL_PIECES * self.G
            self.hc, self.wh, self.geo, self.u8, self.order = self._hc, self._wh, self._geo, self._u8, self._order
        if self.nh is None:
            self._ev.synchronize()
            self.nh = int(self._slot.item())
            if not (self.G <= self.nh <= BALL_PIECES * self.G and self.nh % (128 // PIECE) == 0):
                raise L.VotenetError("piece layout: bad count %d for %d centres" % (self.nh, self.G))
            self.hc, self.wh = self._hc[:self.nh], self._wh[:self.nh]
            self.geo = self._geo[:self.nh * PIECE] if self._geo is not None else None
            self.u8 = self._u8[:self.nh * PIECE] if self._u8 is not None else None
            self.order = self._order[:self.nh * PIECE] if self._order is not None else None
        return self

    @property
    def rows(self):
        return self.resolve().nh * PIECE

    def true_count(self):
        return int(self.nh_dev.item()) if self.nh_limit is not None else self.resolve().nh

    def full_index(self):
        self.resolve()
        G, dev = self.G, self.pos.device
        c = torch.arange(G, device=dev)[:, None]
        s = torch.arange(64, device=dev)[None, :]
        j = s // PIECE
        posx = torch.cat([torch.zeros(G, 1, dtype=torch.long, device=dev), self.pos.view(G, BALL_PIECES - 1).long()], 1)
        p = torch.gather(posx, 1, j.expand(G, 64))
        src = torch.where(j == 0, c * PIECE + s, torch.where(p >= 0, (G + p) * PIECE + s % PIECE, c * PIECE))
        return src.reshape(-1)

    def full_rows(self, t):
        return t[self.full_index()]

    def row_weights(self):
        self.resolve()
        w = torch.ones(self.nh, PIECE, device=self.wh.device)
        w[:, 0] = self.wh
        return w.reshape(-1)


def half_groups(pts_cnt, device_count=False):
    G = pts_cnt.numel()
    dev = pts_cnt.device
    ints = torch.empty((BALL_PIECES - 1) * G + BALL_PIECES * G + 1, dtype=torch.int32, device=dev)
    pos, hc, nh = ints[:(BALL_PIECES - 1) * G], ints[(BALL_PIECES - 1) * G:-1], ints[-1:]
    wh = torch.empty(BALL_PIECES * G, dtype=torch.float32, device=dev)
    slot = None if device_count else HalfLayout.host_slot()
    with L.device_guard(dev):
        L.check(L.lib().votenet_half_groups(G, L.ptr(pts_cnt), L.ptr(pos), L.ptr(hc), L.ptr(wh), L.ptr(nh), L.ptr(slot), L.stream_ptr()))
        return HalfLayout(G, pos, hc, wh, nh, device_count, slot)


def assemble_rows_half(xyz, new_xyz, idx, pts_cnt, half):
    b, m, k = idx.shape
    n = xyz.shape[1]
    if k != 64:
        raise L.InvalidArgumentError("assemble_rows_half expects nsample == 64")
    geo = torch.empty((b * m * 64, 4), dtype=torch.float32, device=xyz.device)
    npts = b * n
    nz = npts * 4 + 16 + (npts + 1) // 2
    if half.nh_limit is not None and _StatsArena.active and _StatsArena.whole_step:
        zero = _zeros_i64((nz,), xyz.device)
    else:
        zero = torch.zeros(nz, dtype=torch.int64, device=xyz.device)
    cntv = zero[:npts * 4].view(npts, 4)
    mom = zero[npts * 4:npts * 4 + 9].view(torch.float64)
    work = zero[npts * 4 + 16:].view(torch.int32)[:npts]
    with L.device_guard(xyz.device):
        L.check(L.lib().votenet_assemble_rows_half(b, n, m, L.ptr(half.nh_dev), L.ptr(xyz), L.ptr(new_xyz), L.ptr(idx), L.ptr(pts_cnt),
                                                   L.ptr(half._hc), L.ptr(geo), L.ptr(cntv), L.ptr(mom), L.ptr(work), L.stream_ptr()))
    half._geo, half._work = geo, work
    return geo, cntv, mom


def narrow_rows_half(xyz, new_xyz, feat, idx, pts_cnt, half):
    b, m, k = idx.shape
    n = xyz.shape[1]
    c = feat.shape[2] if feat is not None else 0
    if k != 64:
        raise L.InvalidArgumentError("narrow_rows_half expects nsample == 64")
    u8 = torch.empty((b * m * 64, 8), dtype=torch.float32, device=xyz.device)
    mom = torch.zeros(72, dtype=torch.float64, device=xyz.device)
    with L.device_guard(xyz.device):
        L.check(L.lib().votenet_narrow_rows_half(b, n, m, c, L.ptr(half.nh_dev), L.ptr(xyz), L.ptr(new_xyz), L.ptr(feat), L.ptr(idx),
                                                 L.ptr(pts_cnt), L.ptr(half._hc), L.ptr(u8), L.ptr(mom), L.stream_ptr()))
    half._u8 = u8
    return u8, mom


def half_sort_rows(half, npts):
    dev = half._geo.device
    work, half._work = getattr(half, "_work", None), None
    counted = work is not None
    if not counted:
        work = torch.empty(npts, dtype=torch.int32, device=dev)
    order = torch.empty(half.G * 64, dtype=torch.int32, device=dev)
    with L.device_guard(dev):
        L.check(L.lib().votenet_half_sort_rows(npts, half.G, L.ptr(half.nh_dev), L.ptr(half._geo), L.ptr(work), 1 if counted else 0, L.ptr(order),
                                               L.stream_ptr()))
    half._order = order
    if half.nh is not None:
        half.order = order[:half.nh * PIECE]
    return order


def group_linear_backward_half(half, b, n, P, wx, da, coef, relu, dw_xyz):
    cout = P.shape[1]
    if getattr(half, "order", None) is None:
        half_sort_rows(half, b * n)
    S = _zeros_f32((b, n, cout), P.device)
    with L.device_guard(P.device):
        L.check(L.lib().votenet_group_linear_backward_sorted(half.nh, cout, L.ptr(half.order), L.ptr(half.geo), L.ptr(half.wh), L.ptr(P),
                                                             L.ptr(wx), L.ptr(da), L.ptr(coef), 1 if relu else 0, L.ptr(S), L.ptr(dw_xyz),
                                                             L.ptr(half.nh_limit), L.stream_ptr()))
    return S


_masked_slots = None


def dgrad_bn_half(z, coef, relu, wT, da, half):
    rows, c = z.shape
    cout = wT.shape[1]
    out = torch.empty((rows, cout), dtype=torch.float32, device=z.device)
    with L.device_guard(z.device), _Timed("linear_dense", 2.0 * rows * c * cout, (rows, c, cout, "dgrad_bn half"), limit=half):
        L.check(L.lib().votenet_mlp_dgrad_bn_half(rows, c, cout, L.ptr(da), L.ptr(z), L.ptr(coef), 1 if relu else 0, L.ptr(wT), L.ptr(out),
                                                  L.ptr(half.wh), L.ptr(half.nh_limit), L.stream_ptr()))
    return out


def group_linear_backward_decomposed(half, b, n, P, wx, da, bn, relu, tail, cntv, mom, dw_xyz, eps=BN_EPS, defer=None):
    cout = P.shape[1]
    dev = P.device
    if getattr(half, "order", None) is None:
        half_sort_rows(half, b * n)
    sc, sh, me, va = bn
    global _masked_slots, COEF_TAIL
    if _masked_slots is None:
        _masked_slots = int(L.lib().votenet_group_linear_backward_masked_slots())
    nparts = _masked_slots
    S = _zeros_f32((b, n, cout), dev)
    small = _zeros_f32((3 + 3 * nparts, cout), dev)
    ug, vp = small[:3], small[3:]
    zeros = _zeros_f64(2 * cout + _masked_slots * 5 * cout, dev)
    sums, part = zeros[:2 * cout], zeros[2 * cout:]
    prev_ct, COEF_TAIL = COEF_TAIL, True
    try:
        t, coef = _coef_tail(tail, cout, dev)
    finally:
        COEF_TAIL = prev_ct
    with L.device_guard(dev):
        L.check(L.lib().votenet_group_linear_backward_masked(half.nh, cout, L.ptr(half.order), L.ptr(half.geo), L.ptr(P), L.ptr(wx), L.ptr(da),
                                                             L.ptr(sc), L.ptr(sh), L.ptr(me), L.ptr(va), eps, 1 if relu else 0, L.ptr(S),
                                                             L.ptr(ug), L.ptr(sums), L.ptr(part), ctypes.byref(t), L.ptr(half.nh_limit),
                                                             L.stream_ptr()))
        L.check(L.lib().votenet_assembled_point_grad(b * n, cout, L.ptr(P), L.ptr(cntv), L.ptr(wx), L.ptr(coef), L.ptr(S), L.ptr(vp),
                                                     L.stream_ptr()))

    def finish():
        with L.device_guard(dev):
            L.check(L.lib().votenet_assembled_wx_finish(cout, L.ptr(coef), L.ptr(ug), L.ptr(vp), nparts, L.ptr(mom), L.ptr(wx), L.ptr(dw_xyz),
                                                        L.stream_ptr()))
    if defer is not None:
        defer(finish, coef, small, mom)
    else:
        finish()
    return S, coef


def half_centre_sums(half, P, wx, da, coef, relu):
    cout = P.shape[1]
    T = torch.empty((half.G, cout), dtype=torch.float32, device=P.device)
    with L.device_guard(P.device):
        L.check(L.lib().votenet_half_centre_sums(half.G, cout, L.ptr(half.pos), L.ptr(half.geo), L.ptr(half.wh), L.ptr(P), L.ptr(wx), L.ptr(da),
                                                 L.ptr(coef), 1 if relu else 0, L.ptr(T), L.stream_ptr()))
    return T


def assemble_stats(P, cntv, wx, mom):
    npts, c0 = P.shape
    stats = _zeros_f64(2 * c0, P.device)
    with L.device_guard(P.device):
        L.check(L.lib().votenet_assemble_stats(npts, c0, L.ptr(P), L.ptr(cntv), L.ptr(wx), L.ptr(mom), L.ptr(stats), L.stream_ptr()))
    return stats


def assemble_z0(geo, P, wx):
    z0 = torch.empty((geo.shape[0], P.shape[1]), dtype=torch.float32, device=P.device)
    with L.device_guard(P.device):
        L.check(L.lib().votenet_assemble_z0(geo.shape[0], P.shape[1], L.ptr(geo), L.ptr(P), L.ptr(wx), L.ptr(z0), L.stream_ptr()))
    return z0


def assembled_linear(geo, P, wx, w, bias, in_bn, in_relu=True, want_stats=True, half=None):
    rows, c0, cout = geo.shape[0], P.shape[1], w.shape[1]
    z = torch.empty((rows, cout), dtype=torch.float32, device=P.device)
    stats = _zeros_f64(2 * cout, P.device) if want_stats else None
    scale = shift = raw = None
    if in_bn.done:
        scale, shift = in_bn.scale, in_bn.shift
    else:
        raw = in_bn.raw()
    if half is not None:
        with L.device_guard(P.device), _Timed("linear_dense", 2.0 * rows * c0 * cout, (rows, c0, cout, "fwd+bn assembled half"), limit=half):
            L.check(L.lib().votenet_assembled_linear_half(rows, c0, cout, L.ptr(geo), L.ptr(P), L.ptr(wx), L.ptr(scale), L.ptr(shift),
                                                          ctypes.byref(raw) if raw is not None else None, 1 if in_relu else 0, L.ptr(w),
                                                          L.ptr(bias), L.ptr(z), L.ptr(stats), L.ptr(half.wh), L.ptr(half.nh_limit), L.stream_ptr()))
        return z, stats
    with L.device_guard(P.device), _Timed("linear_dense", 2.0 * rows * c0 * cout, (rows, c0, cout, "fwd+bn assembled")):
        L.check(L.lib().votenet_assembled_linear(rows, c0, cout, L.ptr(geo), L.ptr(P), L.ptr(wx), L.ptr(scale), L.ptr(shift),
                                                 ctypes.byref(raw) if raw is not None else None, 1 if in_relu else 0, L.ptr(w),
                                                 L.ptr(bias), L.ptr(z), L.ptr(stats), L.stream_ptr()))
    return z, stats


def assembled_wgrad_bn(geo, P, wx, in_scale, in_shift, in_relu, z, coef, relu, da, dw, half=None):
    rows, c0, cout = geo.shape[0], P.shape[1], z.shape[1]
    if half is not None:
        with L.device_guard(P.device), _Timed("wgrad_dense", 2.0 * rows * c0 * cout, (rows, c0, cout, "wgrad_bn assembled half"), limit=half):
            L.check(L.lib().votenet_assembled_wgrad_bn_half(rows, c0, cout, L.ptr(geo), L.ptr(P), L.ptr(wx), L.ptr(in_scale), L.ptr(in_shift),
                                                            1 if in_relu else 0, L.ptr(da), L.ptr(z), L.ptr(coef), 1 if relu else 0,
                                                            L.ptr(half.wh), L.ptr(dw), L.ptr(half.nh_limit), L.stream_ptr()))
        return
    scr = _wgrad_scratch(None, rows, c0, cout, P.device)
    with L.device_guard(P.device), _Timed("wgrad_dense", 2.0 * rows * c0 * cout, (rows, c0, cout, "wgrad_bn assembled")):
        L.check(L.lib().votenet_assembled_wgrad_bn(rows, c0, cout, L.ptr(geo), L.ptr(P), L.ptr(wx), L.ptr(in_scale), L.ptr(in_shift),
                                                   1 if in_relu else 0, L.ptr(da), L.ptr(z), L.ptr(coef), 1 if relu else 0, L.ptr(dw),
                                                   L.ptr(scr), L.stream_ptr()))


def assembled_dgrad_bn_reduce(z, coef, relu, wT, da, geo, P, wx, below, eps=BN_EPS, below_tail=None, half=None):
    rows, c = z.shape
    cout = wT.shape[1]
    bsc, bsh, bme, bva, brelu = below
    out = torch.empty((rows, cout), dtype=torch.float32, device=z.device)
    sums = _zeros_f64(2 * cout, z.device)
    t, coef_b = _coef_tail(below_tail, cout, z.device)
    if half is not None:
        with L.device_guard(z.device), _Timed("linear_dense", 2.0 * rows * c * cout, (rows, c, cout, "dgrad_bn_reduce assembled half"), limit=half):
            L.check(L.lib().votenet_assembled_dgrad_bn_reduce_half(rows, c, cout, L.ptr(da), L.ptr(z), L.ptr(coef), 1 if relu else 0, L.ptr(wT),
                                                                   L.ptr(out), L.ptr(geo), L.ptr(P), L.ptr(wx), L.ptr(bsc), L.ptr(bsh),
                                                                   L.ptr(bme), L.ptr(bva), eps, 1 if brelu else 0, L.ptr(sums),
                                                                   ctypes.byref(t) if t is not None else None, L.ptr(half.wh), L.ptr(half.nh_limit),
                                                                   L.stream_ptr()))
    else:
        with L.device_guard(z.device), _Timed("linear_dense", 2.0 * rows * c * cout, (rows, c, cout, "dgrad_bn_reduce assembled")):
            L.check(L.lib().votenet_assembled_dgrad_bn_reduce(rows, c, cout, L.ptr(da), L.ptr(z), L.ptr(coef), 1 if relu else 0, L.ptr(wT),
                                                              L.ptr(out), L.ptr(geo), L.ptr(P), L.ptr(wx), L.ptr(bsc), L.ptr(bsh), L.ptr(bme),
                                                              L.ptr(bva), eps, 1 if brelu else 0, L.ptr(sums),
                                                              ctypes.byref(t) if t is not None else None, L.stream_ptr()))
    if below_tail is None:
        return out, sums
    return out, (coef_b if coef_b is not None else _coef_after(below_tail, (bsc, bsh, bme, bva), sums, eps))


def group_linear_backward_assembled(xyz, new_xyz, idx, pts_cnt, P, wx, da, coef, relu, dw_xyz, want_dz=False):
    b, m, k = idx.shape
    n, cout = xyz.shape[1], P.shape[1]
    dz = torch.empty((b * m * k, cout), dtype=torch.float32, device=P.device) if want_dz else None
    S = _zeros_f32((b, n, cout), P.device)
    with L.device_guard(P.device):
        L.check(L.lib().votenet_group_linear_backward_assembled(b, n, m, k, cout, L.ptr(xyz), L.ptr(new_xyz), L.ptr(idx), L.ptr(pts_cnt),
                                                                L.ptr(P), L.ptr(wx), L.ptr(da), L.ptr(coef), 1 if relu else 0, L.ptr(S),
                                                                L.ptr(dw_xyz), L.ptr(dz), L.stream_ptr()))
    return S, dz


def narrow_supported(rows, k0, c0, c1):
    return 3 <= k0 <= 8 and rows > 0 and rows % 128 == 0 and rows < 2 ** 31 and c0 % 64 == 0 and c0 <= 128 and (c1 % 64 == 0)


def narrow_rows(xyz, new_xyz, feat, idx, want_moments=True):
    b, m, k = idx.shape
    n = xyz.shape[1]
    c = feat.shape[2] if feat is not None else 0
    u8 = torch.empty((b * m * k, 8), dtype=torch.float32, device=xyz.device)
    mom = torch.zeros(72, dtype=torch.float64, device=xyz.device) if want_moments else None
    with L.device_guard(xyz.device):
        L.check(L.lib().votenet_narrow_rows(b, n, m, k, c, L.ptr(xyz), L.ptr(new_xyz), L.ptr(feat), L.ptr(idx), L.ptr(u8), L.ptr(mom),
                                            L.stream_ptr()))
    return u8, mom


def narrow_z0(u8, w0, b0):
    k0, c0 = w0.shape
    z0 = torch.empty((u8.shape[0], c0), dtype=torch.float32, device=u8.device)
    with L.device_guard(u8.device):
        L.check(L.lib().votenet_narrow_z0(u8.shape[0], k0, c0, L.ptr(u8), L.ptr(w0), L.ptr(b0), L.ptr(z0), L.stream_ptr()))
    return z0


def narrow_stats(rows, mom, w0, b0):
    k0, c0 = w0.shape
    stats = torch.empty(2 * c0, dtype=torch.float64, device=w0.device)
    with L.device_guard(w0.device):
        L.check(L.lib().votenet_narrow_stats(rows, k0, c0, L.ptr(mom), L.ptr(w0), L.ptr(b0), L.ptr(stats), L.stream_ptr()))
    return stats


NARROW_MASK = True


def narrow_mask_supported(rows, c0):
    return rows % 128 == 0 and c0 % 64 == 0


def narrow_linear(u8, w0, b0, w, bias, in_bn, in_relu=True, want_stats=True, half=None, want_mask=False):
    rows = u8.shape[0]
    k0, c0 = w0.shape
    cout = w.shape[1]
    z = torch.empty((rows, cout), dtype=torch.float32, device=u8.device)
    stats = _zeros_f64(2 * cout, u8.device) if want_stats else None
    scale = shift = raw = None
    if in_bn.done:
        scale, shift = in_bn.scale, in_bn.shift
    else:
        raw = in_bn.raw()
    if want_mask:
        if not narrow_mask_supported(rows, c0):
            raise L.InvalidArgumentError("narrow_linear: the mask needs rows %% 128 == 0 and c0 %% 64 == 0")
        mask = torch.empty((rows, c0 // 16), dtype=torch.int16, device=u8.device)
        with L.device_guard(u8.device), _Timed("linear_dense", 2.0 * rows * c0 * cout, (rows, c0, cout, "fwd+bn narrow" + (" half" if half else ""))):
            L.check(L.lib().votenet_narrow_linear_masked(rows, k0, c0, cout, L.ptr(u8), L.ptr(w0), L.ptr(b0), L.ptr(scale), L.ptr(shift),
                                                         ctypes.byref(raw) if raw is not None else None, 1 if in_relu else 0, L.ptr(w),
                                                         L.ptr(bias), L.ptr(z), L.ptr(stats), L.ptr(half.wh) if half is not None else None,
                                                         L.ptr(mask), L.stream_ptr()))
        return z, stats, mask
    if half is not None:
        with L.device_guard(u8.device), _Timed("linear_dense", 2.0 * rows * c0 * cout, (rows, c0, cout, "fwd+bn narrow half")):
            L.check(L.lib().votenet_narrow_linear_half(rows, k0, c0, cout, L.ptr(u8), L.ptr(w0), L.ptr(b0), L.ptr(scale), L.ptr(shift),
                                                       ctypes.byref(raw) if raw is not None else None, 1 if in_relu else 0, L.ptr(w),
                                                       L.ptr(bias), L.ptr(z), L.ptr(stats), L.ptr(half.wh), L.stream_ptr()))
        return z, stats
    with L.device_guard(u8.device), _Timed("linear_dense", 2.0 * rows * c0 * cout, (rows, c0, cout, "fwd+bn narrow")):
        L.check(L.lib().votenet_narrow_linear(rows, k0, c0, cout, L.ptr(u8), L.ptr(w0), L.ptr(b0), L.ptr(scale), L.ptr(shift),
                                              ctypes.byref(raw) if raw is not None else None, 1 if in_relu else 0, L.ptr(w),
                                              L.ptr(bias), L.ptr(z), L.ptr(stats), L.stream_ptr()))
    return z, stats


def narrow_wgrad_bn(u8, w0, b0, in_scale, in_shift, in_relu, z, coef, relu, da, dw, half=None):
    rows = u8.shape[0]
    k0, c0 = w0.shape
    cout = z.shape[1]
    if half is not None:
        with L.device_guard(u8.device), _Timed("wgrad_dense", 2.0 * rows * c0 * cout, (rows, c0, cout, "wgrad_bn narrow half")):
            L.check(L.lib().votenet_narrow_wgrad_bn_half(rows, k0, c0, cout, L.ptr(u8), L.ptr(w0), L.ptr(b0), L.ptr(in_scale), L.ptr(in_shift),
                                                         1 if in_relu else 0, L.ptr(da), L.ptr(z), L.ptr(coef), 1 if relu else 0,
                                                         L.ptr(half.wh), L.ptr(dw), L.stream_ptr()))
        return
    scr = _wgrad_scratch(None, rows, c0, cout, u8.device)
    with L.device_guard(u8.device), _Timed("wgrad_dense", 2.0 * rows * c0 * cout, (rows, c0, cout, "wgrad_bn narrow")):
        L.check(L.lib().votenet_narrow_wgrad_bn(rows, k0, c0, cout, L.ptr(u8), L.ptr(w0), L.ptr(b0), L.ptr(in_scale), L.ptr(in_shift),
                                                1 if in_relu else 0, L.ptr(da), L.ptr(z), L.ptr(coef), 1 if relu else 0, L.ptr(dw),
                                                L.ptr(scr), L.stream_ptr()))


def narrow_dgrad_bn_reduce(z, coef, relu, wT, da, u8, w0, b0, below, eps=BN_EPS, tail=None, half=None, mask=None):
    rows, c = z.shape
    k0, c0 = w0.shape
    bsc, bsh, bme, bva, brelu = below
    out = _zeros_f64(10 * c0, z.device)
    sums, ug = out[:2 * c0], out[2 * c0:]
    t, coef0 = _coef_tail(tail, c0, z.device)
    if mask is not None and t is not None and half is not None:
        with L.device_guard(z.device), _Timed("linear_dense", 2.0 * rows * c * c0, (rows, c, c0, "dgrad_bn_reduce narrow half")):
            L.check(L.lib().votenet_narrow_dgrad_bn_reduce_masked(rows, c, c0, k0, L.ptr(da), L.ptr(z), L.ptr(coef), 1 if relu else 0, L.ptr(wT),
                                                                  L.ptr(u8), L.ptr(w0), L.ptr(b0), L.ptr(bsc), L.ptr(bsh), L.ptr(bme), L.ptr(bva),
                                                                  eps, 1 if brelu else 0, L.ptr(sums), L.ptr(ug), ctypes.byref(t), L.ptr(half.wh),
                                                                  L.ptr(mask), L.stream_ptr()))
        return coef0, ug.view(8, c0)
    with L.device_guard(z.device), _Timed("linear_dense", 2.0 * rows * c * c0, (rows, c, c0, "dgrad_bn_reduce narrow" + (" half" if half else ""))):
        args = (rows, c, c0, k0, L.ptr(da), L.ptr(z), L.ptr(coef), 1 if relu else 0, L.ptr(wT), L.ptr(u8), L.ptr(w0), L.ptr(b0), L.ptr(bsc),
                L.ptr(bsh), L.ptr(bme), L.ptr(bva), eps, 1 if brelu else 0, L.ptr(sums), L.ptr(ug), ctypes.byref(t) if t is not None else None)
        if half is not None:
            L.check(L.lib().votenet_narrow_dgrad_bn_reduce_half(*args, L.ptr(half.wh), L.stream_ptr()))
        else:
            L.check(L.lib().votenet_narrow_dgrad_bn_reduce(*args, L.stream_ptr()))
    if tail is None:
        return sums, ug.view(8, c0)
    return (coef0 if coef0 is not None else _coef_after(tail, (bsc, bsh, bme, bva), sums, eps)), ug.view(8, c0)


def narrow_wgrad_first(mom, ug, coef, w0, b0, dw0):
    k0, c0 = w0.shape
    with L.device_guard(w0.device):
        L.check(L.lib().votenet_narrow_wgrad_first(k0, c0, L.ptr(mom), L.ptr(ug), L.ptr(coef), L.ptr(w0), L.ptr(b0), L.ptr(dw0),
                                                   L.stream_ptr()))


def linear_pool_supported(rows, cin, cout, k):
    return k == 64 and rows > 0 and rows % 128 == 0 and cin % 32 == 0 and cin <= 512 and cout % 128 == 0


def linear_dense_pool(x, w, k, bias=None, in_scale=None, in_shift=None, in_relu=True, keep_z=True, in_bn=None, half=None, gamma=None):
    rows, cin = x.shape
    cout = w.shape[1]
    z = torch.empty((rows, cout), dtype=torch.float32, device=x.device) if keep_z else None
    stats = _zeros_f64(2 * cout, x.device)
    d = _desc_dense(x, in_scale, in_shift, in_relu, in_bn)
    if half is not None:
        if gamma is None:
            raise L.InvalidArgumentError("linear_dense_pool(half=...): the layer's gamma decides which extreme a piece keeps")
        zbest = torch.empty((half.nh, cout), dtype=torch.float32, device=x.device)
        abest = torch.empty((half.nh, cout), dtype=torch.int32, device=x.device)
        with L.device_guard(x.device), _Timed("linear_dense", 2.0 * rows * cin * cout, (rows, cin, cout, "fwd+pool half"), limit=half):
            L.check(L.lib().votenet_mlp_linear_pool_half(ctypes.byref(d), rows, cin, cout, L.ptr(w), L.ptr(bias), L.ptr(z), L.ptr(stats),
                                                         L.ptr(half.wh), L.ptr(gamma), L.ptr(zbest), L.ptr(abest), L.ptr(half.nh_limit), L.stream_ptr()))
        return z, stats, (zbest, abest)
    g = rows // k
    vals = torch.empty((2, g, cout), dtype=torch.float32, device=x.device)
    args = torch.empty((2, g, cout), dtype=torch.int32, device=x.device)
    with L.device_guard(x.device), _Timed("linear_dense", 2.0 * rows * cin * cout, (rows, cin, cout, "fwd+pool")):
        L.check(L.lib().votenet_mlp_linear_pool(ctypes.byref(d), rows, cin, cout, L.ptr(w), L.ptr(bias), L.ptr(z), L.ptr(stats), k,
                                                L.ptr(vals[0]), L.ptr(vals[1]), L.ptr(args[0]), L.ptr(args[1]), L.stream_ptr()))
    return z, stats, (vals[0], vals[1], args[0], args[1])


def bn_pool_finalize(pool, scale, shift, relu=True, want_argmax=False, bn=None, want_zsel=False, half=None):
    zmax = pool[0]
    raw = None
    if bn is not None:
        if bn.done:
            scale, shift = bn.scale, bn.shift
        else:
            raw = bn.raw()
    g, c = zmax.shape
    if half is not None:
        g = half.G
    out = torch.empty((g, c), dtype=torch.float32, device=zmax.device)
    arg = torch.empty((g, c), dtype=torch.int32, device=zmax.device) if want_argmax else None
    zsel = torch.empty((g, c), dtype=torch.float32, device=zmax.device) if want_zsel else None
    if half is not None:
        with L.device_guard(zmax.device):
            L.check(L.lib().votenet_bn_pool_finalize_half(g, c, L.ptr(pool[0]), L.ptr(pool[1]), L.ptr(half.pos), L.ptr(scale), L.ptr(shift),
                                                          ctypes.byref(raw) if raw is not None else None, 1 if relu else 0, L.ptr(out),
                                                          L.ptr(arg), L.ptr(zsel), L.stream_ptr()))
        return (out, arg, zsel) if want_zsel else (out, arg)
    zmax, zmin, amax, amin = pool
    with L.device_guard(zmax.device):
        L.check(L.lib().votenet_bn_pool_finalize(g, c, L.ptr(zmax), L.ptr(zmin), L.ptr(amax), L.ptr(amin), L.ptr(scale), L.ptr(shift),
                                                 ctypes.byref(raw) if raw is not None else None, 1 if relu else 0, L.ptr(out),
                                                 L.ptr(arg), L.ptr(zsel), L.stream_ptr()))
    return (out, arg, zsel) if want_zsel else (out, arg)


def pool_backward_supported(cin, cout, k):
    return bool(L.lib().votenet_pool_backward_supported(cin, cout, k))


def bn_backward_reduce_pool(gout, zsel, scale, shift, mean, var, relu, eps=BN_EPS, tail=None):
    g, c = gout.shape
    sums = _zeros_f64(2 * c, gout.device)
    t, coef = _coef_tail(tail, c, gout.device)
    with L.device_guard(gout.device):
        L.check(L.lib().votenet_bn_backward_reduce_pool(g, c, L.ptr(gout), L.ptr(zsel), L.ptr(scale), L.ptr(shift), L.ptr(mean),
                                                        L.ptr(var), float(eps), 1 if relu else 0, L.ptr(sums),
                                                        ctypes.byref(t) if t is not None else None, L.stream_ptr()))
    if tail is None:
        return sums
    return coef if coef is not None else _coef_after(tail, (scale, shift, mean, var), sums, eps)


def pool_dgrad_prepare(w, bias, coef, rows=None):
    cin, cout = w.shape
    mm = torch.empty((cin + 1, cin), dtype=torch.float32, device=w.device)
    want_img = SPLIT_ADHOC and split_eligible(cin, cin) and (rows is None or rows >= SPLIT_ADHOC_ROWS)
    with L.device_guard(w.device):
        if ADHOC_H2 and FORWARD_H2 and split_eligible(cin, cin):
            img = torch.empty(cin * cin * 4, dtype=torch.uint8, device=w.device)
            sv = torch.empty((2, cin), dtype=torch.float32, device=w.device)
            L.check(L.lib().votenet_pool_dgrad_prepare_h2(cin, cout, L.ptr(w), L.ptr(bias), L.ptr(coef), L.ptr(mm), L.ptr(mm[cin]),
                                                          L.ptr(img), L.ptr(sv[0]), L.ptr(sv[1]), L.stream_ptr()))
            mm._img, mm._h2 = img, sv
        elif want_img:
            img = torch.empty(cin * cin * 6, dtype=torch.uint8, device=w.device)
            L.check(L.lib().votenet_pool_dgrad_prepare_split(cin, cout, L.ptr(w), L.ptr(bias), L.ptr(coef), L.ptr(mm), L.ptr(mm[cin]),
                                                             L.ptr(img), L.stream_ptr()))
            mm._img = img
        else:
            L.check(L.lib().votenet_pool_dgrad_prepare(cin, cout, L.ptr(w), L.ptr(bias), L.ptr(coef), L.ptr(mm), L.ptr(mm[cin]), L.stream_ptr()))
    return mm


def pool_dgrad(xz, in_scale, in_shift, in_relu, w, bias, wT, coef, relu, gout, argmax, zsel, k, below=None, eps=BN_EPS, mm=None,
               below_tail=None, half=None):
    rows, cin = xz.shape
    cout = w.shape[1]
    if mm is None:
        mm = pool_dgrad_prepare(w, bias, coef, rows)
    img = getattr(mm, "_img", None)
    h2 = getattr(mm, "_h2", None)

    def register():
        if h2 is not None:
            L.check(L.lib().votenet_register_split_weights_scaled(L.ptr(mm), cin, cin, L.ptr(img), L.ptr(h2[0]), L.ptr(h2[1])))
        else:
            L.check(L.lib().votenet_register_split_weights(L.ptr(mm), cin, cin, L.ptr(img)))
    if half is not None and half.nh_limit is not None:
        da = torch.empty((rows, cin), dtype=torch.float32, device=xz.device)
        if h2 is not None:
            register()
        try:
            with L.device_guard(xz.device), _Timed("linear_dense", 2.0 * rows * cin * cin, (rows, cin, cin, "gram-form dense dgrad half"), limit=half):
                L.check(L.lib().votenet_mlp_linear_half(L.ptr(xz), L.ptr(in_scale), L.ptr(in_shift), 1 if in_relu else 0, rows, cin, cin, L.ptr(mm),
                                                        L.ptr(mm[cin]), L.ptr(da), L.ptr(half.nh_limit), L.stream_ptr()))
        finally:
            if h2 is not None:
                L.lib().votenet_register_split_weights(L.ptr(mm), cin, cin, None)
    elif img is not None:
        register()
        try:
            da, _ = linear_dense(xz, mm[:cin], mm[cin], in_scale, in_shift, in_relu, want_stats=False)
        finally:
            L.lib().votenet_register_split_weights(L.ptr(mm), cin, cin, None)
    else:
        da, _ = linear_dense(xz, mm[:cin], mm[cin], in_scale, in_shift, in_relu, want_stats=False)
    sums = _zeros_f64(2 * cin, xz.device) if below is not None else None
    bsc, bsh, bme, bva, brelu = below if below is not None else (None, None, None, None, False)
    t, coef_b = _coef_tail(below_tail if below is not None else None, cin, xz.device)
    if half is not None:
        with L.device_guard(xz.device):
            L.check(L.lib().votenet_pool_dgrad_scatter_half(half.nh, half.G, cin, cout, L.ptr(gout), L.ptr(argmax), L.ptr(zsel), L.ptr(coef),
                                                            1 if relu else 0, L.ptr(wT), L.ptr(da), L.ptr(half.hc), L.ptr(half.wh),
                                                            L.ptr(xz if below is not None else None), L.ptr(bsc), L.ptr(bsh), L.ptr(bme),
                                                            L.ptr(bva), float(eps), 1 if brelu else 0, L.ptr(sums),
                                                            ctypes.byref(t) if t is not None else None, L.ptr(half.nh_limit), L.stream_ptr()))
    else:
        with L.device_guard(xz.device):
            L.check(L.lib().votenet_pool_dgrad_scatter(rows // k, k, cin, cout, L.ptr(gout), L.ptr(argmax), L.ptr(zsel), L.ptr(coef),
                                                       1 if relu else 0, L.ptr(wT), L.ptr(da), L.ptr(xz if below is not None else None),
                                                       L.ptr(bsc), L.ptr(bsh), L.ptr(bme), L.ptr(bva), float(eps), 1 if brelu else 0,
                                                       L.ptr(sums), ctypes.byref(t) if t is not None else None, L.stream_ptr()))
    if below is None:
        return da
    if below_tail is None:
        return da, sums
    return da, (coef_b if coef_b is not None else _coef_after(below_tail, (bsc, bsh, bme, bva), sums, eps))


def gram(xz, scale_shift, relu, half=None):
    rows, c = xz.shape
    g = _zeros_f32((c + 1, c), xz.device)
    if half is not None:
        with L.device_guard(xz.device), _Timed("wgrad_dense", 2.0 * rows * c * c, (rows, c, c, "gram half"), limit=half):
            L.check(L.lib().votenet_mlp_gram_half(rows, c, L.ptr(xz), L.ptr(scale_shift), 1 if relu else 0, L.ptr(half.wh), L.ptr(g),
                                                  L.ptr(half.nh_limit), L.stream_ptr()))
        return g
    scr = _wgrad_scratch(None, rows, c, c, xz.device)
    with L.device_guard(xz.device), _Timed("wgrad_dense", 2.0 * rows * c * c, (rows, c, c, "gram")):
        L.check(L.lib().votenet_mlp_gram(rows, c, L.ptr(xz), L.ptr(scale_shift), 1 if relu else 0, L.ptr(g), L.ptr(scr), L.stream_ptr()))
    return g


POOL_WGRAD_CENTRES = True


def pool_wgrad(xz, in_scale, in_shift, in_relu, gram_buf, w, bias, coef, relu, gout, argmax, zsel, k, dw, half=None):
    rows, cin = xz.shape
    cout = w.shape[1]
    if half is not None and POOL_WGRAD_CENTRES and half.nh * 16 * cin * 4 < 2 ** 31:
        with L.device_guard(xz.device):
            L.check(L.lib().votenet_pool_wgrad_sparse_half_centres(half.nh, half.G, cin, cout, L.ptr(xz), L.ptr(in_scale), L.ptr(in_shift),
                                                                   1 if in_relu else 0, L.ptr(gout), L.ptr(argmax), L.ptr(zsel), L.ptr(coef),
                                                                   1 if relu else 0, L.ptr(dw), L.ptr(gram_buf[cin]), L.ptr(half.pos), L.ptr(half.wh),
                                                                   L.ptr(half.nh_limit), L.stream_ptr()))
            L.check(L.lib().votenet_pool_wgrad_finish(cin, cout, L.ptr(gram_buf), L.ptr(gram_buf[cin]), L.ptr(w), L.ptr(bias), L.ptr(coef),
                                                      L.ptr(dw), L.stream_ptr()))
        return
    if half is not None:
        with L.device_guard(xz.device):
            L.check(L.lib().votenet_pool_wgrad_sparse_half(half.nh, half.G, cin, cout, L.ptr(xz), L.ptr(in_scale), L.ptr(in_shift),
                                                           1 if in_relu else 0, L.ptr(gout), L.ptr(argmax), L.ptr(zsel), L.ptr(coef),
                                                           1 if relu else 0, L.ptr(dw), L.ptr(gram_buf[cin]), L.ptr(half.hc), L.ptr(half.wh),
                                                           L.ptr(half.nh_limit), L.stream_ptr()))
            L.check(L.lib().votenet_pool_wgrad_finish(cin, cout, L.ptr(gram_buf), L.ptr(gram_buf[cin]), L.ptr(w), L.ptr(bias), L.ptr(coef),
                                                      L.ptr(dw), L.stream_ptr()))
        return
    scr = None
    if DETERMINISTIC:
        scr = torch.empty(L.lib().votenet_pool_wgrad_scratch_floats(rows // k, cin, cout), dtype=torch.float32, device=xz.device)
    with L.device_guard(xz.device):
        L.check(L.lib().votenet_pool_wgrad_sparse(rows // k, k, cin, cout, L.ptr(xz), L.ptr(in_scale), L.ptr(in_shift), 1 if in_relu else 0,
                                                  L.ptr(gout), L.ptr(argmax), L.ptr(zsel), L.ptr(coef), 1 if relu else 0, L.ptr(dw),
                                                  L.ptr(gram_buf[cin]), L.ptr(scr), L.stream_ptr()))
        L.check(L.lib().votenet_pool_wgrad_finish(cin, cout, L.ptr(gram_buf), L.ptr(gram_buf[cin]), L.ptr(w), L.ptr(bias), L.ptr(coef),
                                                  L.ptr(dw), L.stream_ptr()))


def group_linear(xyz, new_xyz, idx, P, w_xyz, bias=None, want_stats=True):
    b, m, k = idx.shape
    n, cout = xyz.shape[1], w_xyz.shape[1]
    rows = b * m * k
    z = torch.empty((rows, cout), dtype=torch.float32, device=xyz.device)
    stats = _zeros_f64(2 * cout, xyz.device) if want_stats else None
    with L.device_guard(xyz.device):
        L.check(L.lib().votenet_group_linear(b, n, m, k, cout, L.ptr(xyz), L.ptr(new_xyz), L.ptr(idx), L.ptr(P), L.ptr(w_xyz),
                                             L.ptr(bias), L.ptr(z), L.ptr(stats), L.stream_ptr()))
    return z, stats


def group_linear_backward_supported(cout, nsample):
    return cout in (32, 64, 128, 256) and nsample <= 128


def group_linear_backward(xyz, new_xyz, idx, pts_cnt, z, da, coef, relu, dw_xyz, want_dz=False):
    b, m, k = idx.shape
    n, cout = xyz.shape[1], z.shape[1]
    dz = torch.empty_like(z) if want_dz else None
    if DETERMINISTIC:
        inv = _inverse_of(idx, n)
        S = torch.empty((b, n, cout), dtype=torch.float32, device=z.device)
        scr = torch.empty(L.lib().votenet_group_linear_backward_scratch_floats(b, n, cout), dtype=torch.float32, device=z.device)
        with L.device_guard(z.device):
            L.check(L.lib().votenet_group_linear_backward_csr(b, n, m, k, cout, L.ptr(xyz), L.ptr(new_xyz), L.ptr(inv[0]), L.ptr(inv[1]),
                                                              L.ptr(inv[2]) if len(inv) > 2 else None, L.ptr(z), L.ptr(da), L.ptr(coef), 1 if relu else 0, L.ptr(S), L.ptr(dw_xyz),
                                                              L.ptr(dz), L.ptr(scr), L.stream_ptr()))
        return S, dz
    S = _zeros_f32((b, n, cout), z.device)
    with L.device_guard(z.device):
        L.check(L.lib().votenet_group_linear_backward(b, n, m, k, cout, L.ptr(xyz), L.ptr(new_xyz), L.ptr(idx), L.ptr(pts_cnt),
                                                      L.ptr(z), L.ptr(da), L.ptr(coef), 1 if relu else 0, L.ptr(S), L.ptr(dw_xyz),
                                                      L.ptr(dz), L.stream_ptr()))
    return S, dz


def bn_finalize(rows, stats, gamma, beta, eps=BN_EPS):
    c = gamma.shape[0]
    out = torch.empty((4, c), dtype=torch.float32, device=gamma.device)
    with L.device_guard(gamma.device):
        L.check(L.lib().votenet_bn_finalize(rows, c, L.ptr(stats), L.ptr(gamma), L.ptr(beta), float(eps), L.ptr(out[0]),
                                            L.ptr(out[1]), L.ptr(out[2]), L.ptr(out[3]), L.stream_ptr()))
    return out[0], out[1], out[2], out[3]


def bn_relu_max(z, k, scale, shift, relu=True, want_argmax=False):
    rows, c = z.shape
    groups = rows // k
    out = torch.empty((groups, c), dtype=torch.float32, device=z.device)
    arg = torch.empty((groups, c), dtype=torch.int32, device=z.device) if want_argmax else None
    with L.device_guard(z.device):
        L.check(L.lib().votenet_bn_relu_max(groups, k, c, L.ptr(z), L.ptr(scale), L.ptr(shift), 1 if relu else 0, L.ptr(out),
                                            L.ptr(arg), L.stream_ptr()))
    return out, arg


POOL_MODES = {"max": 0, "avg": 1, "weighted_avg": 2, "max_and_avg": 3}


def bn_relu_pool(z, k, scale, shift, relu=True, mode="max", w=None, want_argmax=False):
    rows, c = z.shape
    groups = rows // k
    m = POOL_MODES[mode]
    out = torch.empty((groups, 2 * c if mode == "max_and_avg" else c), dtype=torch.float32, device=z.device)
    arg = torch.empty((groups, c), dtype=torch.int32, device=z.device) if want_argmax and mode in ("max", "max_and_avg") else None
    nwork = L.lib().votenet_bn_relu_pool_workspace_floats(groups, k, c)
    work = torch.empty(nwork, dtype=torch.float32, device=z.device) if nwork else None
    with L.device_guard(z.device):
        L.check(L.lib().votenet_bn_relu_pool(groups, k, c, L.ptr(z), L.ptr(scale), L.ptr(shift), 1 if relu else 0, m, L.ptr(w),
                                             L.ptr(out), L.ptr(arg), L.ptr(work), L.stream_ptr()))
    return out, arg


def sa_pool_weights(xyz, new_xyz=None, idx=None):
    b, n = xyz.shape[:2]
    m, k = (idx.shape[1], idx.shape[2]) if idx is not None else (1, n)
    w = torch.empty(b * m * k, dtype=torch.float32, device=xyz.device)
    with L.device_guard(xyz.device):
        L.check(L.lib().votenet_sa_pool_weights(b, n, m, k, L.ptr(xyz), L.ptr(new_xyz), L.ptr(idx), L.ptr(w), L.stream_ptr()))
    return w


def sa_pool_grad(gout, k, c, mode, w=None, argmax=None):
    groups = gout.shape[0]
    da = torch.empty((groups * k, c), dtype=torch.float32, device=gout.device)
    with L.device_guard(gout.device):
        L.check(L.lib().votenet_sa_pool_grad(groups, k, c, POOL_MODES[mode], L.ptr(gout), L.ptr(w), L.ptr(argmax), L.ptr(da),
                                             L.stream_ptr()))
    return da


def sa_pool_weights_grad(xyz, new_xyz, idx, z, scale, shift, relu, gout, w):
    b, n = xyz.shape[:2]
    m, k = (idx.shape[1], idx.shape[2]) if idx is not None else (1, n)
    c = z.shape[1]
    gw = torch.empty(b * m * k, dtype=torch.float32, device=z.device)
    dv = torch.empty((b * m * k, 3), dtype=torch.float32, device=z.device)
    with L.device_guard(z.device):
        L.check(L.lib().votenet_sa_pool_weights_grad(b, n, m, k, c, L.ptr(xyz), L.ptr(new_xyz), L.ptr(idx), L.ptr(z), L.ptr(scale),
                                                     L.ptr(shift), 1 if relu else 0, L.ptr(gout), L.ptr(w), L.ptr(gw), L.ptr(dv),
                                                     L.stream_ptr()))
    return dv


def bn_relu(z, scale, shift, relu=True, bn=None):
    rows, c = z.shape
    y = torch.empty_like(z)
    raw = None
    if bn is not None:
        if bn.done:
            scale, shift = bn.scale, bn.shift
        else:
            raw = bn.raw()
    with L.device_guard(z.device):
        L.check(L.lib().votenet_bn_relu(rows, c, L.ptr(z), L.ptr(scale), L.ptr(shift), ctypes.byref(raw) if raw is not None else None,
                                        1 if relu else 0, L.ptr(y), L.stream_ptr()))
    return y


def bn_backward(z, scale, shift, mean, var, gamma, relu, da, dgamma, dbeta, argmax=None, k=0, eps=BN_EPS):
    sums = bn_backward_reduce(z, scale, shift, mean, var, relu, da, argmax, k, eps)
    coef = bn_backward_coef(z.shape[0], scale, shift, mean, var, gamma, sums, dgamma, dbeta, eps)
    return bn_backward_apply(z, coef, relu, da, argmax, k)


def bn_backward_apply(z, coef, relu, da, argmax=None, k=0):
    rows, c = z.shape
    dz = torch.empty_like(z)
    with L.device_guard(z.device):
        L.check(L.lib().votenet_bn_backward_apply(rows, c, k, L.ptr(da), L.ptr(argmax), L.ptr(z), L.ptr(coef), 1 if relu else 0,
                                                  L.ptr(dz), L.stream_ptr()))
    return dz


def bn_backward_reduce(z, scale, shift, mean, var, relu, da, argmax=None, k=0, eps=BN_EPS, tail=None):
    rows, c = z.shape
    sums = _zeros_f64(2 * c, z.device)
    t, coef = _coef_tail(tail, c, z.device)
    with L.device_guard(z.device):
        L.check(L.lib().votenet_bn_backward_reduce(rows, c, k, L.ptr(da), L.ptr(argmax), L.ptr(z), L.ptr(scale), L.ptr(shift),
                                                   L.ptr(mean), L.ptr(var), float(eps), 1 if relu else 0, L.ptr(sums),
                                                   ctypes.byref(t) if t is not None else None, L.stream_ptr()))
    if tail is None:
        return sums
    return coef if coef is not None else _coef_after(tail, (scale, shift, mean, var), sums, eps)


def bn_backward_coef(rows, scale, shift, mean, var, gamma, sums, dgamma, dbeta, eps=BN_EPS):
    c = gamma.shape[0]
    coef = torch.empty(5 * c, dtype=torch.float32, device=gamma.device)
    with L.device_guard(gamma.device):
        L.check(L.lib().votenet_bn_backward_coef(rows, c, L.ptr(scale), L.ptr(shift), L.ptr(mean), L.ptr(var), float(eps),
                                                 L.ptr(gamma), L.ptr(sums), L.ptr(coef), L.ptr(dgamma), L.ptr(dbeta),
                                                 L.stream_ptr()))
    return coef


def dgrad_bn_supported(rows, c, cout):
    return rows > 0 and rows % 128 == 0 and c % 32 == 0 and c <= 512 and cout % 64 == 0


def wgrad_dense_bn(x, z, coef, relu, dw, da=None, gout=None, argmax=None, k=0, in_scale=None, in_shift=None, in_relu=True):
    rows, cin = x.shape
    cout = z.shape[1]
    d = _desc_dense(x, in_scale, in_shift, in_relu)
    scr = _wgrad_scratch(d, rows, cin, cout, x.device)
    with L.device_guard(x.device), _Timed("wgrad_dense", 2.0 * rows * cin * cout, (rows, cin, cout, "wgrad_bn")):
        L.check(L.lib().votenet_mlp_wgrad_bn(ctypes.byref(d), rows, cin, cout, L.ptr(da), L.ptr(gout), L.ptr(argmax), k, L.ptr(z),
                                             L.ptr(coef), 1 if relu else 0, L.ptr(dw), L.ptr(scr), L.stream_ptr()))


def dgrad_bn(z, coef, relu, wT, da=None, gout=None, argmax=None, k=0, below=None, eps=BN_EPS, below_tail=None):
    rows, c = z.shape
    cout = wT.shape[1]
    out = torch.empty((rows, cout), dtype=torch.float32, device=z.device)
    if below is not None:
        zp, bsc, bsh, bme, bva, brelu = below
        sums = _zeros_f64(2 * cout, z.device)
        t, coef_b = _coef_tail(below_tail, cout, z.device)
        with L.device_guard(z.device), _SplitK(rows, c, cout, z.device), _Timed("linear_dense", 2.0 * rows * c * cout, (rows, c, cout, "dgrad_bn_reduce")):
            L.check(L.lib().votenet_mlp_dgrad_bn_reduce(rows, c, cout, L.ptr(da), L.ptr(z), L.ptr(coef), 1 if relu else 0, L.ptr(wT),
                                                        L.ptr(out), L.ptr(zp), L.ptr(bsc), L.ptr(bsh), L.ptr(bme), L.ptr(bva), eps,
                                                        1 if brelu else 0, L.ptr(sums), ctypes.byref(t) if t is not None else None,
                                                        L.stream_ptr()))
        if below_tail is None:
            return out, sums
        return out, (coef_b if coef_b is not None else _coef_after(below_tail, (bsc, bsh, bme, bva), sums, eps))
    with L.device_guard(z.device), _SplitK(rows if da is not None else 0, c, cout, z.device), _Timed("linear_dense", 2.0 * rows * c * cout, (rows, c, cout, "dgrad_bn")):
        L.check(L.lib().votenet_mlp_dgrad_bn(rows, c, cout, L.ptr(da), L.ptr(gout), L.ptr(argmax), k, L.ptr(z), L.ptr(coef),
                                             1 if relu else 0, L.ptr(wT), L.ptr(out), L.stream_ptr()))
    return out


def bias_grad(dz, dbias):
    rows, c = dz.shape
    pitch = dz.stride(0) if rows > 1 else c
    if dz.stride(1) != 1:
        dz, pitch = dz.contiguous(), c
    with L.device_guard(dz.device):
        L.check(L.lib().votenet_bias_grad_strided(rows, c, L.ptr(dz), pitch, L.ptr(_zeros_f64(c, dz.device)), L.ptr(dbias), L.stream_ptr()))


def wgrad_dense(x, dz, dw, in_scale=None, in_shift=None, in_relu=True):
    rows, cin = x.shape
    cout = dz.shape[1]
    d = _desc_dense(x, in_scale, in_shift, in_relu)
    scr = _wgrad_scratch(d, rows, cin, cout, x.device)
    with L.device_guard(x.device), _Timed("wgrad_dense", 2.0 * rows * cin * cout, (rows, cin, cout, "wgrad")):
        L.check(L.lib().votenet_mlp_wgrad(ctypes.byref(d), rows, cin, cout, L.ptr(dz), L.ptr(dw), L.ptr(scr), L.stream_ptr()))


def wgrad_gather(xyz, new_xyz, feat, idx, dz, dw):
    b, m, k = idx.shape
    c = feat.shape[2] if feat is not None else 0
    d = _desc_gather(xyz, new_xyz, feat, idx)
    scr = _wgrad_scratch(d, b * m * k, 3 + c, dz.shape[1], xyz.device)
    with L.device_guard(xyz.device), _Timed("wgrad_gather", 2.0 * b * m * k * (3 + c) * dz.shape[1], (b * m * k, 3 + c, dz.shape[1], "wgrad_gather")):
        L.check(L.lib().votenet_mlp_wgrad(ctypes.byref(d), b * m * k, 3 + c, dz.shape[1], L.ptr(dz), L.ptr(dw), L.ptr(scr), L.stream_ptr()))


def rows_dot3(dz, w3):
    rows, c = dz.shape
    out = torch.empty((rows, 3), dtype=torch.float32, device=dz.device)
    with L.device_guard(dz.device):
        L.check(L.lib().votenet_rows_dot3(rows, c, L.ptr(dz), L.ptr(w3), L.ptr(out), L.stream_ptr()))
    return out


def group_concat_grad(d_rows_feat, d_rows_xyz, idx, pts_cnt, n, c):
    b, m, k = idx.shape
    dev = idx.device
    if DETERMINISTIC and (d_rows_feat is None or d_rows_feat.shape[1] <= 256):
        inv = _inverse_of(idx, n)
        d_feat = csr_gather_sum(d_rows_feat, inv, b * n).view(b, n, c) if d_rows_feat is not None else None
        d_xyz = d_new = None
        if d_rows_xyz is not None:
            d_xyz = csr_gather_sum(d_rows_xyz, inv, b * n).view(b, n, 3)
            d_new = -d_rows_xyz.view(b, m, k, 3).sum(2)
        return d_feat, d_xyz, d_new
    d_feat = _zeros_f32((b, n, c), dev) if d_rows_feat is not None else None
    d_xyz = _zeros_f32((b, n, 3), dev) if d_rows_xyz is not None else None
    d_new = _zeros_f32((b, m, 3), dev) if d_rows_xyz is not None else None
    with L.device_guard(dev):
        L.check(L.lib().votenet_group_concat_grad(b, n, c, m, k, L.ptr(d_rows_feat), L.ptr(d_rows_xyz), L.ptr(idx), L.ptr(pts_cnt),
                                                  L.ptr(d_feat), L.ptr(d_xyz), L.ptr(d_new), L.stream_ptr()))
    return d_feat, d_xyz, d_new


def _rows2d(t):
    if t.dim() != 2 or (t.shape[1] > 1 and t.stride(1) != 1):
        raise L.InvalidArgumentError("row_segments: operands are 2-D row-major views with unit column stride")
    return t, (t.stride(0) if t.shape[0] > 1 else max(t.shape[1], t.stride(0)))


def row_segments(rows, segs):
    arr = (L.RowSegment * len(segs))()
    dev = None
    for i, (dst, a, b) in enumerate(segs):
        d, dp = _rows2d(dst)
        dev = d.device
        w = d.shape[1]
        arr[i].dst, arr[i].dst_pitch, arr[i].dst_off, arr[i].width = d.data_ptr(), dp, 0, w
        for name, t in (("a", a), ("b", b)):
            if t is None:
                setattr(arr[i], name, None)
                setattr(arr[i], name + "_pitch", w)
                setattr(arr[i], name + "_off", 0)
                continue
            tt, tp = _rows2d(t)
            if tt.shape[0] != rows or tt.shape[1] != w or d.shape[0] != rows:
                raise L.InvalidArgumentError("row_segments: segment %d: shapes %s / %s do not match (%d rows)" % (i, tuple(d.shape), tuple(tt.shape), rows))
            setattr(arr[i], name, tt.data_ptr())
            setattr(arr[i], name + "_pitch", tp)
            setattr(arr[i], name + "_off", 0)
    with L.device_guard(dev):
        L.check(L.lib().votenet_row_segments(rows, len(segs), arr, L.stream_ptr()))


def copy_segments(pairs):
    arr = (L.CopySegment * len(pairs))()
    dev = None
    for i, (dst, src) in enumerate(pairs):
        nb = dst.numel() * dst.element_size()
        if not (dst.is_contiguous() and src.is_contiguous() and nb == src.numel() * src.element_size() and dst.device == src.device):
            raise L.InvalidArgumentError("copy_segments: pair %d: tensors must be contiguous, on one device and of equal byte size (%s <- %s)"
                                         % (i, tuple(dst.shape), tuple(src.shape)))
        arr[i].dst, arr[i].src, arr[i].bytes = dst.data_ptr(), src.data_ptr(), nb
        dev = dst.device
    if not pairs:
        return
    with L.device_guard(dev):
        L.check(L.lib().votenet_copy_segments(len(pairs), arr, L.stream_ptr()))


SUMSQ_SLICES = 32


def clip_adam(seg, sumsq, p, g, m, v, lr, step, grad_scale=1.0, clip=0.5, beta1=0.9, beta2=0.999, eps=1e-8):
    if sumsq.numel() < SUMSQ_SLICES * (seg.numel() // 2):
        raise L.InvalidArgumentError("clip_adam: the scratch holds %d floats, %d tensors need %d" % (sumsq.numel(), seg.numel() // 2, SUMSQ_SLICES * (seg.numel() // 2)))
    with L.device_guard(p.device):
        L.check(L.lib().votenet_clip_adam(seg.numel() // 2, L.ptr(seg), L.ptr(sumsq), L.ptr(p), L.ptr(g), L.ptr(m), L.ptr(v),
                                          float(lr), float(beta1), float(beta2), float(eps), int(step), float(grad_scale),
                                          float(clip), L.stream_ptr()))


def clip_adam_guarded(seg, sumsq, p, g, m, v, lr, step, guard_state, ema=None, ema_snapshot=None, grad_scale=1.0, clip=0.5, beta1=0.9,
                      beta2=0.999, eps=1e-8):
    nt = seg.numel() // 2
    if sumsq.numel() < SUMSQ_SLICES * nt:
        raise L.InvalidArgumentError("clip_adam_guarded: the scratch holds %d floats, %d tensors need %d" % (sumsq.numel(), nt, SUMSQ_SLICES * nt))
    G = L.side_lib("guard")
    want = G.votenet_step_guard_state_ints()
    if guard_state.dtype != torch.int32 or guard_state.numel() != want or not guard_state.is_contiguous():
        raise L.InvalidArgumentError("clip_adam_guarded: guard_state must be %d contiguous int32, got %d %s"
                                     % (want, guard_state.numel(), guard_state.dtype))
    if (ema is None) != (ema_snapshot is None):
        raise L.InvalidArgumentError("clip_adam_guarded: ema and ema_snapshot go together")
    n_ema = 0
    if ema is not None:
        n_ema = ema.numel()
        if ema_snapshot.numel() != n_ema or ema.dtype != torch.float32 or ema_snapshot.dtype != torch.float32 \
                or not (ema.is_contiguous() and ema_snapshot.is_contiguous()):
            raise L.InvalidArgumentError("clip_adam_guarded: ema and ema_snapshot must be contiguous float32 of one size (%d, %d)"
                                         % (n_ema, ema_snapshot.numel()))
    if not p.is_cuda:
        raise L.VotenetError("clip_adam_guarded: the buffers must live on the GPU (no CPU fallback in votenet_amd)")
    with L.device_guard(p.device):
        L.check(G.votenet_clip_adam_guarded(nt, L.ptr(seg), L.ptr(sumsq), L.ptr(p), L.ptr(g), L.ptr(m), L.ptr(v), float(lr),
                                            float(beta1), float(beta2), float(eps), int(step), float(grad_scale), float(clip),
                                            L.ptr(ema) if n_ema else None, L.ptr(ema_snapshot) if n_ema else None, n_ema,
                                            L.ptr(guard_state), L.stream_ptr()), side="guard")
```

Baseline: 2298.

## Fuse column sums into half-gram kernel and compute only upper-triangle gram tiles

The half-precision gram kernel now also accumulates per-column sums and computes only the upper-triangular (diagonal and off-diagonal) MFMA tiles. The finish kernel mirrors the missing lower half from the upper half as it reads it. The sparse pool wgrad kernels get a CSUM=false variant that skips their column-sum accumulation, because the colsum now comes from the gram pass. This is meant to cut redundant MFMA work and the colsum reduction inside the sparse pass. It adds a new side library, and the finish step now writes the lower half of the gram buffer.

```diff
diff --git a/include/votenet_pool_once.h b/include/votenet_pool_once.h
--- /dev/null
+++ b/include/votenet_pool_once.h
@@ -0,0 +1,22 @@
+#ifndef VOTENET_POOL_ONCE_H
+#define VOTENET_POOL_ONCE_H
+
+#ifdef __cplusplus
+extern "C" {
+#endif
+
+const char *votenet_pool_once_last_error(void);
+
+int votenet_mlp_gram_colsum_half(long rows, int c, const float *z, const float *scale_shift, int relu, const float *wh, float *gram,
+                                 float *colsum, const int *nh_dev, void *stream);
+
+int votenet_pool_wgrad_finish_upper(int cin, int cout, float *gram, const float *colsum, const float *w, const float *bias,
+                                    const float *coef, float *dw, void *stream);
+
+int votenet_pool_once_pieces(int pieces);
+
+#ifdef __cplusplus
+}
+#endif
+
+#endif
diff --git a/votenet_amd/_lib.py b/votenet_amd/_lib.py
--- a/votenet_amd/_lib.py
+++ b/votenet_amd/_lib.py
@@ -20,6 +20,7 @@
     "propsup": "votenet_proposal_supervision.h",
     "votesamp": "votenet_vote_sampling.h",
     "instbox": "votenet_instance_boxes.h",
+    "poolonce": "votenet_pool_once.h",
 }
 _side = {}
 
diff --git a/votenet_amd/csrc/gram_bf3.h b/votenet_amd/csrc/gram_bf3.h
--- /dev/null
+++ b/votenet_amd/csrc/gram_bf3.h
@@ -0,0 +1,274 @@
+#pragma once
+#include "mlp_types.h"
+#include <type_traits>
+
+namespace votenet {
+
+template <bool UPPER>
+__global__ __launch_bounds__(256) void pool_wgrad_finish_kernel(int cin, int cout, float *gram,
+                                                                const float *__restrict__ colsum, const float *__restrict__ w,
+                                                                const float *__restrict__ bias, const float *__restrict__ coef,
+                                                                float *__restrict__ dw)
+{
+    __shared__ float Gs[16][33], Ws[32][17];
+    const int tx = threadIdx.x & 15, ty = threadIdx.x >> 4;
+    const int j0 = blockIdx.y * 16, c0 = blockIdx.x * 16;
+    float acc = 0.0f;
+    for (int i0 = 0; i0 < cin; i0 += 32) {
+        for (int e = threadIdx.x; e < 16 * 32; e += 256) {
+            const int r = e >> 5, ii = e & 31;
+            const int gj = j0 + r, gi = i0 + ii;
+            const bool in = gj < cin && gi < cin, low = UPPER && gj > gi;
+            const float gv = in ? gram[low ? (size_t)gi * cin + gj : (size_t)gj * cin + gi] : 0.0f;
+            Gs[r][ii] = gv;
+            if (UPPER && blockIdx.x == 0 && in && low) gram[(size_t)gj * cin + gi] = gv;
+            const int wr = e >> 4, wc = e & 15;
+            Ws[wr][wc] = (i0 + wr < cin && c0 + wc < cout) ? w[(size_t)(i0 + wr) * cout + c0 + wc] : 0.0f;
+        }
+        __syncthreads();
+#pragma unroll 8
+        for (int ii = 0; ii < 32; ii++) acc += Gs[ty][ii] * Ws[ii][tx];
+        __syncthreads();
+    }
+    const int j = j0 + ty, c = c0 + tx;
+    if (j < cin && c < cout) {
+        const float Cc = coef[2 * cout + c];
+        dw[(size_t)j * cout + c] += Cc * acc + colsum[j] * (coef[cout + c] + Cc * (bias ? bias[c] : 0.0f));
+    }
+}
+
+
+#ifndef GRAM_ABL
+#define GRAM_ABL 0
+#endif
+enum { kGramFull, kGramDiag, kGramOff, kGramNone };
+__host__ __device__ constexpr int gram_px(int form, int T, int t) { return form == kGramFull ? t / T : form == kGramDiag ? (t == 2 ? 1 : 0) : 0; }
+__host__ __device__ constexpr int gram_py(int form, int T, int t) { return form == kGramFull ? T + t % T : form == kGramDiag ? (t == 0 ? 0 : 1) : 1 + t; }
+template <int C, int NP = 3, bool CS = false, bool UP = false>
+__global__ __launch_bounds__(256) void gram_bf3_kernel(long rows, const float *__restrict__ x, const float *__restrict__ scale_shift,
+                                                       int relu, float *__restrict__ gram, long rows_per_block,
+                                                       const float *__restrict__ wh ,
+                                                       const int *__restrict__ nh_dev ,
+                                                       float *__restrict__ colsum = nullptr )
+{
+    if (nh_dev != nullptr) {
+        const long lim = (long)nh_dev[0] * kPiece;
+        rows = lim < rows ? lim : rows;
+    }
+    constexpr int KPT = 8;
+    constexpr int KS = 128 / C;
+    constexpr int RS = 16 * KS;
+    constexpr int T = C / 64;
+    constexpr int PL = C * 4 + 16;
+    static_assert(NP == 2 || NP == 3, "pieces per operand");
+    constexpr float kA = NP == 2 ? 16.0f : 1.0f, kUn = NP == 2 ? 1.0f / 256.0f : 1.0f;
+    __shared__ __attribute__((aligned(16))) unsigned Ts[2][NP][KS][2][PL];
+    const int tid = threadIdx.x, lane = tid & 63;
+    const int wv = __builtin_amdgcn_readfirstlane(tid >> 6);
+    const int wi = wv >> 1, wj = wv & 1;
+    const long r_begin = (long)blockIdx.x * rows_per_block;
+    if (r_begin >= rows) return;
+    const int nrow = (int)((r_begin + rows_per_block < rows ? r_begin + rows_per_block : rows) - r_begin);
+    const int nslab = (nrow + RS - 1) / RS;
+    const int c = tid % C, rg = tid / C;
+    const int ks_w = rg >> 1, kh_w = rg & 1;
+    const int row_w = ks_w * 16 + kh_w * KPT;
+    const float sc = scale_shift[c] * kA, sh = scale_shift[C + c] * kA;
+    const float floor_ = relu ? 0.0f : -__builtin_inff();
+    const float *xb = x + (size_t)r_begin * C + c;
+    float R[2][KPT];
+    static_assert(kPiece == 16, "one k-step = one piece");
+    const bool first_rg = kh_w == 0;
+    const float *whb = wh ? wh + r_begin / kPiece : nullptr;
+    const float *whp = whb ? whb : scale_shift;
+    float Wq[2] = {1.0f, 1.0f};
+    bool abl_prologue = true;
+    float csum = 0.0f;
+    auto load = [&](float (&r)[KPT], int s, float &wq) {
+        if ((GRAM_ABL & 4) && !abl_prologue) return;
+#pragma unroll
+        for (int i = 0; i < KPT; i++) {
+            int lr = s * RS + row_w + i;
+            lr = lr < nrow ? lr : nrow - 1;
+            r[i] = xb[(size_t)lr * C];
+        }
+        const int sw = (whb != nullptr && s * RS + ks_w * 16 < nrow) ? s * KS + ks_w : 0;
+        wq = whp[sw];
+    };
+    auto store = [&](int buf, const float (&r)[KPT], int s, float wq) {
+        if ((GRAM_ABL & 8) && !abl_prologue) return;
+        float v[KPT];
+#pragma unroll
+        for (int i = 0; i < KPT; i++) {
+            v[i] = fmaxf(r[i] * sc + sh, floor_);
+            if (s * RS + row_w + i >= nrow) v[i] = 0.0f;
+        }
+        const bool head = whb != nullptr && first_rg && s * RS + ks_w * 16 < nrow;
+        if constexpr (CS) {
+            float t[KPT];
+            t[0] = head ? v[0] * wq : v[0];
+#pragma unroll
+            for (int i = 1; i < KPT; i++) t[i] = v[i];
+#pragma unroll
+            for (int w2 = 1; w2 < KPT; w2 *= 2)
+#pragma unroll
+                for (int i = 0; i < KPT; i += 2 * w2) t[i] += t[i + w2];
+            csum += t[0];
+        }
+        if (head) v[0] *= sqrtf(wq);
+        if constexpr (NP == 2) {
+            unsigned h[KPT / 2], l[KPT / 2];
+#pragma unroll
+            for (int i = 0; i < KPT / 2; i++) split2(v[2 * i], v[2 * i + 1], h[i], l[i]);
+            *reinterpret_cast<uint4 *>(&Ts[buf][0][ks_w][kh_w][c * 4]) = make_uint4(h[0], h[1], h[2], h[3]);
+            *reinterpret_cast<uint4 *>(&Ts[buf][1][ks_w][kh_w][c * 4]) = make_uint4(l[0], l[1], l[2], l[3]);
+            return;
+        }
+        unsigned h[KPT / 2], m[KPT / 2], l[KPT / 2];
+#pragma unroll
+        for (int i = 0; i < KPT / 2; i++) split3(v[2 * i], v[2 * i + 1], h[i], m[i], l[i]);
+        *reinterpret_cast<uint4 *>(&Ts[buf][0][ks_w][kh_w][c * 4]) = make_uint4(h[0], h[1], h[2], h[3]);
+        *reinterpret_cast<uint4 *>(&Ts[buf][1][ks_w][kh_w][c * 4]) = make_uint4(m[0], m[1], m[2], m[3]);
+        *reinterpret_cast<uint4 *>(&Ts[buf][NP - 1][ks_w][kh_w][c * 4]) = make_uint4(l[0], l[1], l[2], l[3]);
+    };
+    load(R[0], 0, Wq[0]);
+    store(0, R[0], 0, Wq[0]);
+    load(R[1], 1, Wq[1]);
+    __builtin_amdgcn_sched_barrier(0);
+    load(R[0], 2, Wq[0]);
+    __syncthreads();
+    const int kh = lane >> 5, l31 = lane & 31;
+    auto run = [&](auto form_c) {
+        constexpr int FORM = decltype(form_c)::value;
+        constexpr int NF = FORM == kGramFull ? 2 * T : FORM == kGramDiag ? 2 : FORM == kGramOff ? 3 : 1;
+        constexpr int NT = FORM == kGramFull ? T * T : FORM == kGramDiag ? 3 : FORM == kGramOff ? 2 : 0;
+        auto blk = [&](int f) {
+            if constexpr (FORM == kGramFull) return f < T ? wi * T + f : wj * T + (f - T);
+            else if constexpr (FORM == kGramDiag) return 2 * wv + f;
+            else return f == 0 ? wv - 2 : f + 1;
+        };
+        f32x16 acc[NT > 0 ? NT : 1];
+#pragma unroll
+        for (int t = 0; t < (NT > 0 ? NT : 1); t++)
+#pragma unroll
+            for (int e = 0; e < 16; e++) acc[t][e] = 0.0f;
+        int buf = 0;
+        abl_prologue = false;
+        const int nslab2 = (nslab + 1) & ~1;
+        for (int s = 0; s < nslab2; s += 2) {
+#pragma unroll
+            for (int par = 0; par < 2; par++) {
+                uint4 fr[KS][NP][NF];
+                if constexpr (NT > 0) {
+#pragma unroll
+                    for (int k = 0; k < KS; k++)
+#pragma unroll
+                        for (int p = 0; p < NP; p++)
+#pragma unroll
+                            for (int f = 0; f < NF; f++) fr[k][p][f] = *reinterpret_cast<const uint4 *>(&Ts[buf][p][k][kh][(blk(f) * 32 + l31) * 4]);
+                }
+                auto mmk = [&](int k, int pa, int pb) {
+                    if constexpr (NT > 0) {
+                        if (GRAM_ABL & 1) {
+                            acc[0][0] += __uint_as_float(fr[k][pa][0].x ^ fr[k][pb][NF - 1].y);
+                            return;
+                        }
+#pragma unroll
+                        for (int t = 0; t < NT; t++) {
+                            const uint4 fa = fr[k][pa][gram_px(FORM, T, t)], fb = fr[k][pb][gram_py(FORM, T, t)];
+                            if constexpr (NP == 2)
+                                acc[t] = __builtin_amdgcn_mfma_f32_32x32x16_f16(__builtin_bit_cast(f16x8, fa), __builtin_bit_cast(f16x8, fb), acc[t], 0, 0, 0);
+                            else
+                                acc[t] = __builtin_amdgcn_mfma_f32_32x32x16_bf16(__builtin_bit_cast(bf16x8, fa), __builtin_bit_cast(bf16x8, fb), acc[t], 0, 0, 0);
+                        }
+                    }
+                };
+                auto mm = [&](int pa, int pb) { mmk(0, pa, pb); };
+                auto rest = [&]() {
+#pragma unroll
+                    for (int k = 1; k < KS; k++) {
+                        if constexpr (NP == 3) {
+                            mmk(k, 2, 0);
+                            mmk(k, 0, 2);
+                            mmk(k, 1, 1);
+                        }
+                        mmk(k, 1, 0);
+                        mmk(k, 0, 1);
+                        mmk(k, 0, 0);
+                    }
+                };
+                if constexpr (NP == 2) {
+                    mm(1, 0);
+                    mm(0, 1);
+                    store(buf ^ 1, R[par ^ 1], s + par + 1, Wq[par ^ 1]);
+                    load(R[par ^ 1], s + par + 3, Wq[par ^ 1]);
+                    mm(0, 0);
+                } else {
+                    mm(2, 0);
+                    mm(0, 2);
+                    mm(1, 1);
+                    store(buf ^ 1, R[par ^ 1], s + par + 1, Wq[par ^ 1]);
+                    load(R[par ^ 1], s + par + 3, Wq[par ^ 1]);
+                    mm(1, 0);
+                    mm(0, 1);
+                    mm(0, 0);
+                }
+                rest();
+                lds_barrier();
+                buf ^= 1;
+            }
+        }
+        if (GRAM_ABL & 2) {
+            float t_ = 0.0f;
+#pragma unroll
+            for (int t = 0; t < NT; t++)
+#pragma unroll
+                for (int e = 0; e < 16; e++) t_ += acc[t][e];
+            if (t_ == 12345.678f) gram[0] = t_;
+            return;
+        }
+#pragma unroll
+        for (int t = 0; t < NT; t++) {
+            const int i0 = blk(gram_px(FORM, T, t)) * 32 + 4 * kh, j = blk(gram_py(FORM, T, t)) * 32 + l31;
+#pragma unroll
+            for (int e = 0; e < 16; e++) unsafeAtomicAdd(&gram[(size_t)(i0 + (e & 3) + 8 * (e >> 2)) * C + j], acc[t][e] * kUn);
+        }
+    };
+    if constexpr (!UP) run(std::integral_constant<int, kGramFull>{});
+    else if constexpr (C == 128) {
+        if (wv < 2) run(std::integral_constant<int, kGramDiag>{});
+        else run(std::integral_constant<int, kGramOff>{});
+    } else {
+        if (wv == 2) run(std::integral_constant<int, kGramNone>{});
+        else run(std::integral_constant<int, kGramFull>{});
+    }
+    if constexpr (CS) {
+        float *cl = reinterpret_cast<float *>(&Ts[0][0][0][0][0]);
+        cl[tid] = csum;
+        __syncthreads();
+        if (tid < C) {
+            float t = cl[tid] + cl[C + tid];
+            if constexpr (C == 64) t = t + (cl[2 * C + tid] + cl[3 * C + tid]);
+            unsafeAtomicAdd(&colsum[tid], t * (1.0f / kA));
+        }
+    }
+}
+
+template <int C, bool ONCE = false>
+static void gram_bf3_launch(int pieces , int wgs, long rows, const float *z, const float *scale_shift, int relu, float *gram, hipStream_t st, const float *wh = nullptr,
+                            const int *nh_dev = nullptr, float *colsum = nullptr)
+{
+    long rpb = (rows + wgs - 1) / wgs;
+    rpb = (rpb + 31) / 32 * 32;
+    if (rpb < 128) rpb = 128;
+    const unsigned gx = (unsigned)((rows + rpb - 1) / rpb);
+    if constexpr (ONCE) {
+        if (pieces != 3) hipLaunchKernelGGL((gram_bf3_kernel<C, 2, true, true>), dim3(gx), dim3(256), 0, st, rows, z, scale_shift, relu, gram, rpb, wh, nh_dev, colsum);
+        else hipLaunchKernelGGL((gram_bf3_kernel<C, 3, true, true>), dim3(gx), dim3(256), 0, st, rows, z, scale_shift, relu, gram, rpb, wh, nh_dev, colsum);
+        return;
+    }
+    if (pieces != 3) hipLaunchKernelGGL((gram_bf3_kernel<C, 2>), dim3(gx), dim3(256), 0, st, rows, z, scale_shift, relu, gram, rpb, wh, nh_dev, colsum);
+    else hipLaunchKernelGGL((gram_bf3_kernel<C, 3>), dim3(gx), dim3(256), 0, st, rows, z, scale_shift, relu, gram, rpb, wh, nh_dev, colsum);
+}
+
+}
diff --git a/votenet_amd/csrc/pool_bwd.hip b/votenet_amd/csrc/pool_bwd.hip
--- a/votenet_amd/csrc/pool_bwd.hip
+++ b/votenet_amd/csrc/pool_bwd.hip
@@ -1,4 +1,5 @@
 #include "mlp_types.h"
+#include "gram_bf3.h"
 #include <mutex>
 #include <set>
 
@@ -541,7 +542,7 @@
     }
 }
 
-template <int CIN, int K, int TEAMS>
+template <int CIN, int K, int TEAMS, bool CSUM = true>
 __global__ __launch_bounds__(256 * TEAMS) void pool_wgrad_sparse_kernel(long groups, int cout, const float *__restrict__ xz,
                                                                 const float *__restrict__ in_scale, const float *__restrict__ in_shift,
                                                                 int in_relu, const float *__restrict__ gout,
@@ -650,7 +651,7 @@
                     }
                 }
             }
-            if (live && tid >= 256 - CIN) {
+            if (CSUM && live && tid >= 256 - CIN) {
                 const int jc = tid - (256 - CIN);
 #pragma unroll 8
                 for (int r = (HALF ? 1 : 0); r < K; r++) csum += xt[r][jc];
@@ -668,7 +669,7 @@
 #pragma unroll
                 for (int i = 0; i < CIN; i++) comb[(size_t)i * cout + tid] = acc[i];
             }
-            if (tid >= 256 - CIN) comb[(size_t)CIN * cout + tid - (256 - CIN)] = csum;
+            if (CSUM && tid >= 256 - CIN) comb[(size_t)CIN * cout + tid - (256 - CIN)] = csum;
         }
         __syncthreads();
         if (team == 1) return;
@@ -676,7 +677,7 @@
 #pragma unroll
             for (int i = 0; i < CIN; i++) acc[i] += comb[(size_t)i * cout + tid];
         }
-        if (tid >= 256 - CIN) csum += comb[(size_t)CIN * cout + tid - (256 - CIN)];
+        if (CSUM && tid >= 256 - CIN) csum += comb[(size_t)CIN * cout + tid - (256 - CIN)];
     }
     if (part) {
         float *__restrict__ mine = part + (size_t)blockIdx.x * (CIN + 1) * cout;
@@ -684,17 +685,17 @@
 #pragma unroll
             for (int i = 0; i < CIN; i++) mine[(size_t)i * cout + tid] = acc[i];
         }
-        if (tid >= 256 - CIN) mine[(size_t)CIN * cout + tid - (256 - CIN)] = csum;
+        if (CSUM && tid >= 256 - CIN) mine[(size_t)CIN * cout + tid - (256 - CIN)] = csum;
         return;
     }
     if (own) {
 #pragma unroll
         for (int i = 0; i < CIN; i++) unsafeAtomicAdd(&dw[(size_t)i * cout + tid], acc[i]);
     }
-    if (tid >= 256 - CIN) unsafeAtomicAdd(&colsum[tid - (256 - CIN)], csum);
-}
-
-template <int CIN, int TEAMS>
+    if (CSUM && tid >= 256 - CIN) unsafeAtomicAdd(&colsum[tid - (256 - CIN)], csum);
+}
+
+template <int CIN, int TEAMS, bool CSUM = true>
 __global__ __launch_bounds__(256 * TEAMS) void pool_wgrad_sparse_centre_kernel(int G, long nh, int cout, const float *__restrict__ xz,
                                                                        const float *__restrict__ in_scale, const float *__restrict__ in_shift,
                                                                        int in_relu, const float *__restrict__ gout,
@@ -810,7 +811,7 @@
                     }
                 }
             }
-            if (live && tid >= 256 - CIN) {
+            if (CSUM && live && tid >= 256 - CIN) {
                 const int jc = tid - (256 - CIN);
 #pragma unroll
                 for (int j = 0; j < NP; j++) {
@@ -831,7 +832,7 @@
 #pragma unroll
                 for (int i = 0; i < CIN; i++) comb[(size_t)i * cout + tid] = acc[i];
             }
-            if (tid >= 256 - CIN) comb[(size_t)CIN * cout + tid - (256 - CIN)] = csum;
+            if (CSUM && tid >= 256 - CIN) comb[(size_t)CIN * cout + tid - (256 - CIN)] = csum;
         }
         __syncthreads();
         if (team == 1) return;
@@ -839,41 +840,13 @@
 #pragma unroll
             for (int i = 0; i < CIN; i++) acc[i] += comb[(size_t)i * cout + tid];
         }
-        if (tid >= 256 - CIN) csum += comb[(size_t)CIN * cout + tid - (256 - CIN)];
+        if (CSUM && tid >= 256 - CIN) csum += comb[(size_t)CIN * cout + tid - (256 - CIN)];
     }
     if (own) {
 #pragma unroll
         for (int i = 0; i < CIN; i++) unsafeAtomicAdd(&dw[(size_t)i * cout + tid], acc[i]);
     }
-    if (tid >= 256 - CIN) unsafeAtomicAdd(&colsum[tid - (256 - CIN)], csum);
-}
-
-__global__ __launch_bounds__(256) void pool_wgrad_finish_kernel(int cin, int cout, const float *__restrict__ gram,
-                                                                const float *__restrict__ colsum, const float *__restrict__ w,
-                                                                const float *__restrict__ bias, const float *__restrict__ coef,
-                                                                float *__restrict__ dw)
-{
-    __shared__ float Gs[16][33], Ws[32][17];
-    const int tx = threadIdx.x & 15, ty = threadIdx.x >> 4;
-    const int j0 = blockIdx.y * 16, c0 = blockIdx.x * 16;
-    float acc = 0.0f;
-    for (int i0 = 0; i0 < cin; i0 += 32) {
-        for (int e = threadIdx.x; e < 16 * 32; e += 256) {
-            const int r = e >> 5, ii = e & 31;
-            Gs[r][ii] = (j0 + r < cin && i0 + ii < cin) ? gram[(size_t)(j0 + r) * cin + i0 + ii] : 0.0f;
-            const int wr = e >> 4, wc = e & 15;
-            Ws[wr][wc] = (i0 + wr < cin && c0 + wc < cout) ? w[(size_t)(i0 + wr) * cout + c0 + wc] : 0.0f;
-        }
-        __syncthreads();
-#pragma unroll 8
-        for (int ii = 0; ii < 32; ii++) acc += Gs[ty][ii] * Ws[ii][tx];
-        __syncthreads();
-    }
-    const int j = j0 + ty, c = c0 + tx;
-    if (j < cin && c < cout) {
-        const float Cc = coef[2 * cout + c];
-        dw[(size_t)j * cout + c] += Cc * acc + colsum[j] * (coef[cout + c] + Cc * (bias ? bias[c] : 0.0f));
-    }
+    if (CSUM && tid >= 256 - CIN) unsafeAtomicAdd(&colsum[tid - (256 - CIN)], csum);
 }
 
 }
@@ -1061,193 +1034,8 @@
     return check_launch("pool_dgrad_scatter");
 }
 
-#ifndef GRAM_ABL
-#define GRAM_ABL 0
-#endif
-template <int C, int NP = 3>
-__global__ __launch_bounds__(256) void gram_bf3_kernel(long rows, const float *__restrict__ x, const float *__restrict__ scale_shift,
-                                                       int relu, float *__restrict__ gram, long rows_per_block,
-                                                       const float *__restrict__ wh ,
-                                                       const int *__restrict__ nh_dev )
-{
-    if (nh_dev != nullptr) {
-        const long lim = (long)nh_dev[0] * kPiece;
-        rows = lim < rows ? lim : rows;
-    }
-    constexpr int KPT = C / 16;
-    constexpr int T = C / 64;
-    constexpr int PL = C * 4 + 16;
-    static_assert(NP == 2 || NP == 3, "pieces per operand");
-    constexpr float kA = NP == 2 ? 16.0f : 1.0f, kUn = NP == 2 ? 1.0f / 256.0f : 1.0f;
-    __shared__ __attribute__((aligned(16))) unsigned Ts[2][NP][2][PL];
-    const int tid = threadIdx.x, lane = tid & 63;
-    const int wv = __builtin_amdgcn_readfirstlane(tid >> 6);
-    const int wi = wv >> 1, wj = wv & 1;
-    const long r_begin = (long)blockIdx.x * rows_per_block;
-    if (r_begin >= rows) return;
-    const int nrow = (int)((r_begin + rows_per_block < rows ? r_begin + rows_per_block : rows) - r_begin);
-    const int nslab = (nrow + 15) / 16;
-    const int c = tid % C, rg = tid / C;
-    const int kh_w = (C == 128) ? rg : (rg >> 1), d_w = (C == 128) ? 0 : (rg & 1) * 2;
-    const float sc = scale_shift[c] * kA, sh = scale_shift[C + c] * kA;
-    const float floor_ = relu ? 0.0f : -__builtin_inff();
-    const float *xb = x + (size_t)r_begin * C + c;
-    float R[2][KPT];
-    static_assert(kPiece == 16, "one slab = one piece");
-    const bool first_rg = rg == 0;
-    const float *whb = wh ? wh + r_begin / kPiece : nullptr;
-    const float *whp = whb ? whb : scale_shift;
-    float Wq[2] = {1.0f, 1.0f};
-    bool abl_prologue = true;
-    auto load = [&](float (&r)[KPT], int s, float &wq) {
-        if ((GRAM_ABL & 4) && !abl_prologue) return;
-#pragma unroll
-        for (int i = 0; i < KPT; i++) {
-            int lr = s * 16 + rg * KPT + i;
-            lr = lr < nrow ? lr : nrow - 1;
-            r[i] = xb[(size_t)lr * C];
-        }
-        const int sw = (whb != nullptr && s * 16 < nrow) ? s : 0;
-        wq = whp[sw];
-    };
-    auto store = [&](int buf, const float (&r)[KPT], int s, float wq) {
-        if ((GRAM_ABL & 8) && !abl_prologue) return;
-        float v[KPT];
-#pragma unroll
-        for (int i = 0; i < KPT; i++) {
-            v[i] = fmaxf(r[i] * sc + sh, floor_);
-            if (s * 16 + rg * KPT + i >= nrow) v[i] = 0.0f;
-        }
-        if (whb != nullptr && first_rg && s * 16 < nrow) v[0] *= sqrtf(wq);
-        if constexpr (NP == 2) {
-            unsigned h[KPT / 2], l[KPT / 2];
-#pragma unroll
-            for (int i = 0; i < KPT / 2; i++) split2(v[2 * i], v[2 * i + 1], h[i], l[i]);
-            if constexpr (C == 128) {
-                *reinterpret_cast<uint4 *>(&Ts[buf][0][kh_w][c * 4]) = make_uint4(h[0], h[1], h[2], h[3]);
-                *reinterpret_cast<uint4 *>(&Ts[buf][1][kh_w][c * 4]) = make_uint4(l[0], l[1], l[2], l[3]);
-            } else {
-                *reinterpret_cast<uint2 *>(&Ts[buf][0][kh_w][c * 4 + d_w]) = make_uint2(h[0], h[1]);
-                *reinterpret_cast<uint2 *>(&Ts[buf][1][kh_w][c * 4 + d_w]) = make_uint2(l[0], l[1]);
-            }
-            return;
-        }
-        unsigned h[KPT / 2], m[KPT / 2], l[KPT / 2];
-#pragma unroll
-        for (int i = 0; i < KPT / 2; i++) split3(v[2 * i], v[2 * i + 1], h[i], m[i], l[i]);
-        if constexpr (C == 128) {
-            *reinterpret_cast<uint4 *>(&Ts[buf][0][kh_w][c * 4]) = make_uint4(h[0], h[1], h[2], h[3]);
-            *reinterpret_cast<uint4 *>(&Ts[buf][1][kh_w][c * 4]) = make_uint4(m[0], m[1], m[2], m[3]);
-            *reinterpret_cast<uint4 *>(&Ts[buf][NP - 1][kh_w][c * 4]) = make_uint4(l[0], l[1], l[2], l[3]);
-        } else {
-            *reinterpret_cast<uint2 *>(&Ts[buf][0][kh_w][c * 4 + d_w]) = make_uint2(h[0], h[1]);
-            *reinterpret_cast<uint2 *>(&Ts[buf][1][kh_w][c * 4 + d_w]) = make_uint2(m[0], m[1]);
-            *reinterpret_cast<uint2 *>(&Ts[buf][NP - 1][kh_w][c * 4 + d_w]) = make_uint2(l[0], l[1]);
-        }
-    };
-    f32x16 acc[T][T];
-#pragma unroll
-    for (int a = 0; a < T; a++)
-#pragma unroll
-        for (int b = 0; b < T; b++)
-#pragma unroll
-            for (int e = 0; e < 16; e++) acc[a][b][e] = 0.0f;
-    load(R[0], 0, Wq[0]);
-    store(0, R[0], 0, Wq[0]);
-    load(R[1], 1, Wq[1]);
-    __builtin_amdgcn_sched_barrier(0);
-    load(R[0], 2, Wq[0]);
-    __syncthreads();
-    const int kh = lane >> 5, l31 = lane & 31;
-    int buf = 0;
-    abl_prologue = false;
-    const int nslab2 = (nslab + 1) & ~1;
-    for (int s = 0; s < nslab2; s += 2) {
-#pragma unroll
-        for (int par = 0; par < 2; par++) {
-            uint4 fa[NP][T], fb[NP][T];
-#pragma unroll
-            for (int p = 0; p < NP; p++) {
-#pragma unroll
-                for (int t = 0; t < T; t++) {
-                    fa[p][t] = *reinterpret_cast<const uint4 *>(&Ts[buf][p][kh][((wi * T + t) * 32 + l31) * 4]);
-                    fb[p][t] = *reinterpret_cast<const uint4 *>(&Ts[buf][p][kh][((wj * T + t) * 32 + l31) * 4]);
-                }
-            }
-            auto mm = [&](int pa, int pb) {
-                if (GRAM_ABL & 1) {
-                    acc[0][0][0] += __uint_as_float(fa[pa][0].x ^ fb[pb][0].y);
-                    return;
-                }
-#pragma unroll
-                for (int a = 0; a < T; a++)
-#pragma unroll
-                    for (int b = 0; b < T; b++) {
-                        if constexpr (NP == 2)
-                            acc[a][b] = __builtin_amdgcn_mfma_f32_32x32x16_f16(__builtin_bit_cast(f16x8, fa[pa][a]),
-                                                                               __builtin_bit_cast(f16x8, fb[pb][b]), acc[a][b], 0, 0, 0);
-                        else
-                            acc[a][b] = __builtin_amdgcn_mfma_f32_32x32x16_bf16(__builtin_bit_cast(bf16x8, fa[pa][a]),
-                                                                                __builtin_bit_cast(bf16x8, fb[pb][b]), acc[a][b], 0, 0, 0);
-                    }
-            };
-            if constexpr (NP == 2) {
-                mm(1, 0);
-                mm(0, 1);
-                store(buf ^ 1, R[par ^ 1], s + par + 1, Wq[par ^ 1]);
-                load(R[par ^ 1], s + par + 3, Wq[par ^ 1]);
-                mm(0, 0);
-            } else {
-                mm(2, 0);
-                mm(0, 2);
-                mm(1, 1);
-                store(buf ^ 1, R[par ^ 1], s + par + 1, Wq[par ^ 1]);
-                load(R[par ^ 1], s + par + 3, Wq[par ^ 1]);
-                mm(1, 0);
-                mm(0, 1);
-                mm(0, 0);
-            }
-            lds_barrier();
-            buf ^= 1;
-        }
-    }
-    if (GRAM_ABL & 2) {
-        float t_ = 0.0f;
-#pragma unroll
-        for (int a = 0; a < T; a++)
-#pragma unroll
-            for (int b = 0; b < T; b++)
-#pragma unroll
-                for (int e = 0; e < 16; e++) t_ += acc[a][b][e];
-        if (t_ == 12345.678f) gram[0] = t_;
-        return;
-    }
-#pragma unroll
-    for (int a = 0; a < T; a++)
-#pragma unroll
-        for (int b = 0; b < T; b++) {
-            const int j = (wj * T + b) * 32 + l31;
-#pragma unroll
-            for (int e = 0; e < 16; e++) {
-                const int i = (wi * T + a) * 32 + (e & 3) + 8 * (e >> 2) + 4 * kh;
-                unsafeAtomicAdd(&gram[(size_t)i * C + j], acc[a][b][e] * kUn);
-            }
-        }
-}
-
 int g_gram_bf3 = 1;
 static int g_gram_wgs = 384;
-template <int C>
-static void gram_bf3_launch(long rows, const float *z, const float *scale_shift, int relu, float *gram, hipStream_t st, const float *wh = nullptr,
-                            const int *nh_dev = nullptr)
-{
-    long rpb = (rows + g_gram_wgs - 1) / g_gram_wgs;
-    rpb = (rpb + 31) / 32 * 32;
-    if (rpb < 128) rpb = 128;
-    const unsigned gx = (unsigned)((rows + rpb - 1) / rpb);
-    if (g_gram_bf3 != 3) hipLaunchKernelGGL((gram_bf3_kernel<C, 2>), dim3(gx), dim3(256), 0, st, rows, z, scale_shift, relu, gram, rpb, wh, nh_dev);
-    else hipLaunchKernelGGL((gram_bf3_kernel<C, 3>), dim3(gx), dim3(256), 0, st, rows, z, scale_shift, relu, gram, rpb, wh, nh_dev);
-}
 extern "C" void votenet_debug_gram_bf3(int on) { VN_DEBUG_GATE(); g_gram_bf3 = on; }
 extern "C" void votenet_debug_gram_workgroups(int n) { VN_DEBUG_GATE(); g_gram_wgs = n > 0 ? n : 384; }
 
@@ -1256,8 +1044,8 @@
 {
     if (g_gram_bf3 && scratch == nullptr && (c == 64 || c == 128) && rows > 0 && rows < (1L << 31) / c && z && scale_shift && gram &&
         (uintptr_t)z % 16 == 0) {
-        if (c == 128) gram_bf3_launch<128>(rows, z, scale_shift, relu, gram, as_stream(stream));
-        else gram_bf3_launch<64>(rows, z, scale_shift, relu, gram, as_stream(stream));
+        if (c == 128) gram_bf3_launch<128>(g_gram_bf3, g_gram_wgs, rows, z, scale_shift, relu, gram, as_stream(stream));
+        else gram_bf3_launch<64>(g_gram_bf3, g_gram_wgs, rows, z, scale_shift, relu, gram, as_stream(stream));
         return check_launch("mlp_gram");
     }
     VN_REQUIRE(rows > 0 && c > 0 && z && scale_shift && gram, "mlp_gram: bad arguments");
@@ -1305,8 +1093,8 @@
 {
     VN_REQUIRE(rows > 0 && rows % kPiece == 0 && rows < (1L << 31) / c && (c == 128 || c == 64), "mlp_gram_half expects rows %% 16 == 0 and c in {64, 128}");
     VN_REQUIRE(z && scale_shift && wh && gram && (uintptr_t)z % 16 == 0, "mlp_gram_half: null / unaligned buffer");
-    if (c == 128) gram_bf3_launch<128>(rows, z, scale_shift, relu, gram, as_stream(stream), wh, nh_dev);
-    else gram_bf3_launch<64>(rows, z, scale_shift, relu, gram, as_stream(stream), wh, nh_dev);
+    if (c == 128) gram_bf3_launch<128>(g_gram_bf3, g_gram_wgs, rows, z, scale_shift, relu, gram, as_stream(stream), wh, nh_dev);
+    else gram_bf3_launch<64>(g_gram_bf3, g_gram_wgs, rows, z, scale_shift, relu, gram, as_stream(stream), wh, nh_dev);
     return check_launch("mlp_gram_half");
 }
 
@@ -1315,7 +1103,7 @@
                                               float *dw, float *colsum, const int *hc, const float *wh, const int *nh_dev, void *stream)
 {
     VN_REQUIRE(nh > 0 && G > 0 && nh >= G && nh <= (long)kBallPieces * G && hc && wh, "pool_wgrad_sparse_half: bad piece-layout arguments");
-    VN_REQUIRE(xz && gout && argmax && zsel && coef && dw && colsum, "pool_wgrad_sparse_half: bad arguments");
+    VN_REQUIRE(xz && gout && argmax && zsel && coef && dw, "pool_wgrad_sparse_half: bad arguments");
     VN_REQUIRE(votenet_pool_backward_supported(cin, cout, 64), "pool_wgrad_sparse_half: unsupported shape cin=%d cout=%d", cin, cout);
     VN_REQUIRE((in_scale == nullptr) == (in_shift == nullptr), "pool_wgrad_sparse_half: in_scale and in_shift go together");
     VN_REQUIRE((uintptr_t)xz % 16 == 0 && (!in_scale || ((uintptr_t)in_scale % 16 == 0 && (uintptr_t)in_shift % 16 == 0)),
@@ -1333,7 +1121,7 @@
                                                       const int *pos, const float *wh, const int *nh_dev, void *stream)
 {
     VN_REQUIRE(nh > 0 && G > 0 && nh >= G && nh <= (long)kBallPieces * G && pos && wh, "pool_wgrad_sparse_half_centres: bad piece-layout arguments");
-    VN_REQUIRE(xz && gout && argmax && zsel && coef && dw && colsum, "pool_wgrad_sparse_half_centres: bad arguments");
+    VN_REQUIRE(xz && gout && argmax && zsel && coef && dw, "pool_wgrad_sparse_half_centres: bad arguments");
     VN_REQUIRE(votenet_pool_backward_supported(cin, cout, 64), "pool_wgrad_sparse_half_centres: unsupported shape cin=%d cout=%d", cin, cout);
     VN_REQUIRE((in_scale == nullptr) == (in_shift == nullptr), "pool_wgrad_sparse_half_centres: in_scale and in_shift go together");
     VN_REQUIRE((size_t)nh * kPiece * (size_t)cin * 4 < ((size_t)1 << 31),
@@ -1359,7 +1147,13 @@
         hipLaunchKernelGGL(kern, dim3(grid), dim3(256 * teams), smem, st, G, nh, cout, xz, in_scale, in_shift, in_relu, gout, argmax, zsel, coef, relu, dw,
                            colsum, pos, wh, nh_dev);
     };
-    if (teams == 1) {
+    if (colsum == nullptr) {
+        if (teams == 1) {
+            if (cin == 64) go(pool_wgrad_sparse_centre_kernel<64, 1, false>, 64);
+            else go(pool_wgrad_sparse_centre_kernel<128, 1, false>, 128);
+        } else if (cin == 64) go(pool_wgrad_sparse_centre_kernel<64, 2, false>, 64);
+        else go(pool_wgrad_sparse_centre_kernel<128, 2, false>, 128);
+    } else if (teams == 1) {
         if (cin == 64) go(pool_wgrad_sparse_centre_kernel<64, 1>, 64);
         else go(pool_wgrad_sparse_centre_kernel<128, 1>, 128);
     } else if (cin == 64) go(pool_wgrad_sparse_centre_kernel<64, 2>, 64);
@@ -1389,7 +1183,13 @@
         hipLaunchKernelGGL(kern, dim3(grid), dim3(256 * teams), smem, st, groups, cout, xz, in_scale, in_shift, in_relu, gout, argmax, zsel, coef,
                            relu, dw, colsum, scratch, hc, wh, G, nh_dev);
     };
-    if (hc && g_sparse_teams == 2 && !scratch) {
+    if (hc && colsum == nullptr) {
+        if (g_sparse_teams == 2) {
+            if (cin == 64) go(pool_wgrad_sparse_kernel<64, kPiece, 2, false>, 64, kPiece, 2, g_sparse_wgs2);
+            else go(pool_wgrad_sparse_kernel<128, kPiece, 2, false>, 128, kPiece, 2, g_sparse_wgs2);
+        } else if (cin == 64) go(pool_wgrad_sparse_kernel<64, kPiece, 1, false>, 64, kPiece, 1, g_sparse_wgs);
+        else go(pool_wgrad_sparse_kernel<128, kPiece, 1, false>, 128, kPiece, 1, g_sparse_wgs);
+    } else if (hc && g_sparse_teams == 2 && !scratch) {
         if (cin == 64) go(pool_wgrad_sparse_kernel<64, kPiece, 2>, 64, kPiece, 2, g_sparse_wgs2);
         else go(pool_wgrad_sparse_kernel<128, kPiece, 2>, 128, kPiece, 2, g_sparse_wgs2);
     } else if (hc) {
@@ -1418,7 +1218,7 @@
                                          const float *coef, float *dw, void *stream)
 {
     VN_REQUIRE(cin > 0 && cout > 0 && gram && colsum && w && coef && dw, "pool_wgrad_finish: bad arguments");
-    hipLaunchKernelGGL(pool_wgrad_finish_kernel, dim3((cout + 15) / 16, (cin + 15) / 16), dim3(256), 0, as_stream(stream), cin, cout,
-                       gram, colsum, w, bias, coef, dw);
+    hipLaunchKernelGGL(pool_wgrad_finish_kernel<false>, dim3((cout + 15) / 16, (cin + 15) / 16), dim3(256), 0, as_stream(stream), cin, cout,
+                       const_cast<float *>(gram), colsum, w, bias, coef, dw);
     return check_launch("pool_wgrad_finish");
 }
diff --git a/votenet_amd/csrc/poolonce/pool_once.hip b/votenet_amd/csrc/poolonce/pool_once.hip
--- /dev/null
+++ b/votenet_amd/csrc/poolonce/pool_once.hip
@@ -0,0 +1,48 @@
+#include "../gram_bf3.h"
+#include "../error_text.h"
+
+#include <cstdint>
+#pragma GCC visibility push(default)
+#include "../../../include/votenet_pool_once.h"
+#pragma GCC visibility pop
+
+namespace votenet {
+
+static thread_local ErrorText g_po_err;
+#define PO_REQUIRE(cond, ...) VN_REQUIRE_IN(::votenet::g_po_err, cond, __VA_ARGS__)
+
+static int g_po_pieces = 2;
+constexpr int kPoWorkgroups = 384;
+
+}
+
+using namespace votenet;
+
+extern "C" const char *votenet_pool_once_last_error(void) { return g_po_err.text; }
+
+extern "C" int votenet_pool_once_pieces(int pieces)
+{
+    PO_REQUIRE(pieces == 2 || pieces == 3, "pool_once_pieces expects 2 (fp16 x 2) or 3 (bf16 x 3), got %d", pieces);
+    g_po_pieces = pieces;
+    return VOTENET_OK;
+}
+
+extern "C" int votenet_mlp_gram_colsum_half(long rows, int c, const float *z, const float *scale_shift, int relu, const float *wh, float *gram,
+                                            float *colsum, const int *nh_dev, void *stream)
+{
+    PO_REQUIRE((c == 128 || c == 64) && rows > 0 && rows % kPiece == 0 && rows < (1L << 31) / c,
+               "mlp_gram_colsum_half expects rows %% 16 == 0 and c in {64, 128}");
+    PO_REQUIRE(z && scale_shift && wh && gram && colsum && (uintptr_t)z % 16 == 0, "mlp_gram_colsum_half: null / unaligned buffer");
+    if (c == 128) gram_bf3_launch<128, true>(g_po_pieces, kPoWorkgroups, rows, z, scale_shift, relu, gram, as_stream(stream), wh, nh_dev, colsum);
+    else gram_bf3_launch<64, true>(g_po_pieces, kPoWorkgroups, rows, z, scale_shift, relu, gram, as_stream(stream), wh, nh_dev, colsum);
+    return g_po_err.check_launch("mlp_gram_colsum_half");
+}
+
+extern "C" int votenet_pool_wgrad_finish_upper(int cin, int cout, float *gram, const float *colsum, const float *w, const float *bias,
+                                               const float *coef, float *dw, void *stream)
+{
+    PO_REQUIRE(cin > 0 && cout > 0 && gram && colsum && w && coef && dw, "pool_wgrad_finish_upper: bad arguments");
+    hipLaunchKernelGGL(pool_wgrad_finish_kernel<true>, dim3((cout + 15) / 16, (cin + 15) / 16), dim3(256), 0, as_stream(stream), cin, cout,
+                       gram, colsum, w, bias, coef, dw);
+    return g_po_err.check_launch("pool_wgrad_finish_upper");
+}
diff --git a/votenet_amd/mlp.py b/votenet_amd/mlp.py
--- a/votenet_amd/mlp.py
+++ b/votenet_amd/mlp.py
@@ -1038,8 +1038,8 @@
     g = _zeros_f32((c + 1, c), xz.device)
     if half is not None:
         with L.device_guard(xz.device), _Timed("wgrad_dense", 2.0 * rows * c * c, (rows, c, c, "gram half"), limit=half):
-            L.check(L.lib().votenet_mlp_gram_half(rows, c, L.ptr(xz), L.ptr(scale_shift), 1 if relu else 0, L.ptr(half.wh), L.ptr(g),
-                                                  L.ptr(half.nh_limit), L.stream_ptr()))
+            L.check(L.side_lib("poolonce").votenet_mlp_gram_colsum_half(rows, c, L.ptr(xz), L.ptr(scale_shift), 1 if relu else 0, L.ptr(half.wh),
+                                                                        L.ptr(g), L.ptr(g[c]), L.ptr(half.nh_limit), L.stream_ptr()), side="poolonce")
         return g
     scr = _wgrad_scratch(None, rows, c, c, xz.device)
     with L.device_guard(xz.device), _Timed("wgrad_dense", 2.0 * rows * c * c, (rows, c, c, "gram")):
@@ -1057,19 +1057,19 @@
         with L.device_guard(xz.device):
             L.check(L.lib().votenet_pool_wgrad_sparse_half_centres(half.nh, half.G, cin, cout, L.ptr(xz), L.ptr(in_scale), L.ptr(in_shift),
                                                                    1 if in_relu else 0, L.ptr(gout), L.ptr(argmax), L.ptr(zsel), L.ptr(coef),
-                                                                   1 if relu else 0, L.ptr(dw), L.ptr(gram_buf[cin]), L.ptr(half.pos), L.ptr(half.wh),
+                                                                   1 if relu else 0, L.ptr(dw), None, L.ptr(half.pos), L.ptr(half.wh),
                                                                    L.ptr(half.nh_limit), L.stream_ptr()))
-            L.check(L.lib().votenet_pool_wgrad_finish(cin, cout, L.ptr(gram_buf), L.ptr(gram_buf[cin]), L.ptr(w), L.ptr(bias), L.ptr(coef),
-                                                      L.ptr(dw), L.stream_ptr()))
+            L.check(L.side_lib("poolonce").votenet_pool_wgrad_finish_upper(cin, cout, L.ptr(gram_buf), L.ptr(gram_buf[cin]), L.ptr(w), L.ptr(bias),
+                                                                           L.ptr(coef), L.ptr(dw), L.stream_ptr()), side="poolonce")
         return
     if half is not None:
         with L.device_guard(xz.device):
             L.check(L.lib().votenet_pool_wgrad_sparse_half(half.nh, half.G, cin, cout, L.ptr(xz), L.ptr(in_scale), L.ptr(in_shift),
                                                            1 if in_relu else 0, L.ptr(gout), L.ptr(argmax), L.ptr(zsel), L.ptr(coef),
-                                                           1 if relu else 0, L.ptr(dw), L.ptr(gram_buf[cin]), L.ptr(half.hc), L.ptr(half.wh),
+                                                           1 if relu else 0, L.ptr(dw), None, L.ptr(half.hc), L.ptr(half.wh),
                                                            L.ptr(half.nh_limit), L.stream_ptr()))
-            L.check(L.lib().votenet_pool_wgrad_finish(cin, cout, L.ptr(gram_buf), L.ptr(gram_buf[cin]), L.ptr(w), L.ptr(bias), L.ptr(coef),
-                                                      L.ptr(dw), L.stream_ptr()))
+            L.check(L.side_lib("poolonce").votenet_pool_wgrad_finish_upper(cin, cout, L.ptr(gram_buf), L.ptr(gram_buf[cin]), L.ptr(w), L.ptr(bias),
+                                                                           L.ptr(coef), L.ptr(dw), L.stream_ptr()), side="poolonce")
         return
     scr = None
     if DETERMINISTIC:
```

After: 2281. No clear change (-0.7%).
